# Patryk27/strolle

Measured on NVIDIA H100. Metric: Mrays/s (+ frames/s) at 1080p-per-GPU Cornell, ReSTIR DI+GI + SVGF; H100 vs CPU restatement of the reference, higher is better.
Workload: dtype f32

## Files before the change

include/strolle_b200.h:

```cpp
#ifndef STROLLE_B200_H
#define STROLLE_B200_H

#include <stddef.h>
#include <stdint.h>

#ifdef __cplusplus
extern "C" {
#endif

typedef struct st_engine st_engine;
typedef uint64_t st_handle;
typedef int32_t st_camera_handle;

enum { ST_OK = 0, ST_ERR_CUDA = -1, ST_ERR_INVALID = -2, ST_ERR_NOT_FOUND = -3, ST_ERR_LIMIT = -4 };

typedef struct st_mesh_triangle {
    float positions[3][3];
    float normals[3][3];
    float uvs[3][2];
    float tangents[3][4];
} st_mesh_triangle;

typedef struct st_material {
    float base_color[4];
// ... 52 lines not shown
int st_update_sun(st_engine* e, float azimuth, float altitude);
int st_set_environment_map(st_engine* e, const float* rgba32f, uint32_t width, uint32_t height, float intensity, float rotation);
typedef struct st_exposure { float ev, compensation, ev_min, ev_max, low, high, speed_up, speed_down; } st_exposure;
int st_set_exposure(st_engine* e, const st_exposure* exposure);
typedef struct st_bloom { float intensity, scatter, threshold, softness; int32_t levels, mode; } st_bloom;
int st_set_bloom(st_engine* e, const st_bloom* bloom);
typedef struct st_depth_of_field { float focal_distance, aperture_f_stops, sensor_height, max_radius; } st_depth_of_field;
int st_set_depth_of_field(st_engine* e, const st_depth_of_field* dof);

int st_create_camera(st_engine* e, const st_camera* camera, st_camera_handle* out);
int st_update_camera(st_engine* e, st_camera_handle camera, const st_camera* desc);
int st_delete_camera(st_engine* e, st_camera_handle camera);

int st_tick(st_engine* e);

int st_render_camera(st_engine* e, st_camera_handle camera, void* host_out, int format);
int st_copy_output(st_engine* e, st_camera_handle camera, void* host_out, int format);
int st_synchronize(st_engine* e);

int st_set_seed_base(st_engine* e, uint32_t base);
int st_set_blue_noise(st_engine* e, const uint8_t* rgba8_256x256);
int st_read_buffer(st_engine* e, st_camera_handle camera, const char* name, float* dst, size_t cap_floats, size_t* count);
int st_read_scene(st_engine* e, const char* name, float* dst, size_t cap_floats, size_t* count);
int st_bvh_depth(st_engine* e, int* depth);
uint32_t st_frame(st_engine* e);
int st_set_frame(st_engine* e, uint32_t frame);
int st_trace_closest(st_engine* e, const float* rays, size_t n, float* out, float* device_ms);
int st_trace_any(st_engine* e, const float* rays, size_t n, uint32_t* out, float* device_ms);
int st_device_math(st_engine* e, int op, const float* a, const float* b, float* out, size_t n);
#define ST_PASS_COUNT 27
int st_enable_timing(st_engine* e, int enabled);
int st_pass_times(st_engine* e, float* ms, uint32_t* launches, int reset);
const char* st_pass_name(int pass);
int st_wavelet_times(st_engine* e, float* ms5, uint32_t* launches5, int reset);
enum { ST_OPT_SVGF_FAST_MATH = 1, ST_OPT_ASYNC_OUTPUT = 2, ST_OPT_HALO_NCCL = 3, ST_OPT_WAVELET_TILED = 4, ST_OPT_WAVELET_TILE_CFG = 5, ST_OPT_FUSE_REPROJECT = 6, ST_OPT_BVH_REUSE = 7, ST_OPT_VARIANCE_TILED = 8, ST_OPT_SHADING_FAST_MATH = 9, ST_OPT_STRIP_FUSED = 10, ST_OPT_FUSED_PASSES = 11, ST_OPT_STRIP_DMA = 12, ST_OPT_WAVELET_PAIRED = 13, ST_OPT_NORMAL_MAPS = 14, ST_OPT_BVH_REFIT = 15, ST_OPT_LIGHT_GRID = 16, ST_OPT_TEXTURE_FILTER = 17, ST_OPT_TEMPORAL_AA = 18, ST_OPT_ENVIRONMENT_MAP_SAMPLING = 19, ST_OPT_TONEMAPPING = 20, ST_OPT_AUTO_EXPOSURE = 21, ST_OPT_BLOOM = 22, ST_OPT_DEPTH_OF_FIELD = 23 };
#define ST_WAVELET_PAIRED_DEFAULT 1
#define ST_STRIP_DMA_DEFAULT (-1)
#define ST_FUSED_PASSES_DEFAULT 1
#define ST_SHADING_FAST_DEFAULT 1
#define ST_VARIANCE_TILED_DEFAULT 1
#define ST_WAVELET_TILED_DEFAULT 15
#define ST_WAVELET_CFG_DEFAULT 0x01000
#define ST_FUSE_REPROJECT_DEFAULT 1
int st_set_option(st_engine* e, int option, int value);
enum { ST_STAT_WAVELET_TILED_LAUNCHES = 1, ST_STAT_WAVELET_TILED_ERRORS = 2, ST_STAT_BVH_GRAFTED_SUBTREES = 3, ST_STAT_VARIANCE_TILED_LAUNCHES = 4,
       ST_STAT_STRIP_PULLED_ROWS = 5 , ST_STAT_LAST_FRAME_FUSED_STRIPS = 6 ,
       ST_STAT_STRIP_FIRST_TIMEOUT = 7 ,
       ST_STAT_NORMAL_MAP_LAUNCHES = 8 ,
       ST_STAT_BVH_REFITS = 9 ,
       ST_STAT_LIGHT_GRID_BUILDS = 10 ,
       ST_STAT_TEXTURE_MIP_BUILDS = 11 ,
       ST_STAT_TAA_RESOLVES = 12 ,
       ST_STAT_ENVIRONMENT_MAP_LAUNCHES = 13 ,
       ST_STAT_ENVIRONMENT_MAP_DISTRIBUTION_BUILDS = 14 ,
       ST_STAT_EXPOSURE_METERINGS = 15 ,
       ST_STAT_BLOOM_PYRAMIDS = 16 ,
       ST_STAT_DEPTH_OF_FIELD_GATHERS = 17  };
int st_get_stat(st_engine* e, int stat, uint64_t* value);
typedef struct st_bvh_builder st_bvh_builder;
int st_bvh_builder_create(st_bvh_builder** out);
void st_bvh_builder_destroy(st_bvh_builder* b);
int st_bvh_builder_build(st_bvh_builder* b, const float* prims11, size_t n, int reuse, float* out, size_t cap_floats, size_t* n_floats,
                         uint32_t* grafted_subtrees, int* depth);
int st_bvh_builder_read(st_bvh_builder* b, float* out, size_t cap_floats);
int st_set_stream(st_engine* e, void* cuda_stream, int external);
int st_count_rays(st_engine* e, int enabled);
// ... 61 lines not shown
```

rust/strolle-b200-sys/src/lib.rs:

```rust
#![allow(non_camel_case_types, clippy::too_many_arguments)]

use std::os::raw::{c_char, c_int, c_void};

#[repr(C)] pub struct st_engine { _private: [u8; 0] }
#[repr(C)] pub struct st_multi { _private: [u8; 0] }
#[repr(C)] pub struct st_bvh_builder { _private: [u8; 0] }
pub type st_handle = u64;
pub type st_camera_handle = i32;

pub const ST_OK: c_int = 0;
pub const ST_ERR_CUDA: c_int = -1;
pub const ST_ERR_INVALID: c_int = -2;
pub const ST_ERR_NOT_FOUND: c_int = -3;
pub const ST_ERR_LIMIT: c_int = -4;

#[repr(C)] #[derive(Clone, Copy, Debug, Default)]
pub struct st_mesh_triangle { pub positions: [[f32; 3]; 3], pub normals: [[f32; 3]; 3], pub uvs: [[f32; 2]; 3], pub tangents: [[f32; 4]; 3] }
#[repr(C)] #[derive(Clone, Copy, Debug, Default)]
pub struct st_material { pub base_color: [f32; 4], pub emissive: [f32; 4], pub perceptual_roughness: f32, pub metallic: f32, pub reflectance: f32, pub ior: f32, pub alpha_blend: i32 }
#[repr(C)] #[derive(Clone, Copy, Debug, Default)]
pub struct st_material_textures { pub base_color: st_handle, pub emissive: st_handle, pub metallic_roughness: st_handle, pub normal_map: st_handle, pub mask: u32 }
pub const ST_LIGHT_POINT: i32 = 1;
pub const ST_LIGHT_SPOT: i32 = 2;
#[repr(C)] #[derive(Clone, Copy, Debug, Default)]
// ... 79 lines not shown
    pub fn st_remove_material(e: *mut st_engine, material: st_handle) -> c_int;
    pub fn st_insert_image(e: *mut st_engine, image: st_handle, rgba8: *const u8, width: u32, height: u32) -> c_int;
    pub fn st_remove_image(e: *mut st_engine, image: st_handle) -> c_int;
    pub fn st_set_material_textures(e: *mut st_engine, material: st_handle, textures: *const st_material_textures) -> c_int;
    pub fn st_insert_instance(e: *mut st_engine, instance: st_handle, mesh: st_handle, material: st_handle, affine: *const f32) -> c_int;
    pub fn st_remove_instance(e: *mut st_engine, instance: st_handle) -> c_int;
    pub fn st_insert_light(e: *mut st_engine, light: st_handle, l: *const st_light) -> c_int;
    pub fn st_remove_light(e: *mut st_engine, light: st_handle) -> c_int;
    pub fn st_update_sun(e: *mut st_engine, azimuth: f32, altitude: f32) -> c_int;
    pub fn st_set_environment_map(e: *mut st_engine, rgba32f: *const f32, width: u32, height: u32, intensity: f32, rotation: f32) -> c_int;
    pub fn st_set_exposure(e: *mut st_engine, exposure: *const st_exposure) -> c_int;
    pub fn st_set_bloom(e: *mut st_engine, bloom: *const st_bloom) -> c_int;
    pub fn st_set_depth_of_field(e: *mut st_engine, dof: *const st_depth_of_field) -> c_int;
    pub fn st_create_camera(e: *mut st_engine, camera: *const st_camera, out: *mut st_camera_handle) -> c_int;
    pub fn st_update_camera(e: *mut st_engine, camera: st_camera_handle, desc: *const st_camera) -> c_int;
    pub fn st_delete_camera(e: *mut st_engine, camera: st_camera_handle) -> c_int;
    pub fn st_tick(e: *mut st_engine) -> c_int;
    pub fn st_render_camera(e: *mut st_engine, camera: st_camera_handle, host_out: *mut c_void, format: c_int) -> c_int;
    pub fn st_copy_output(e: *mut st_engine, camera: st_camera_handle, host_out: *mut c_void, format: c_int) -> c_int;
    pub fn st_synchronize(e: *mut st_engine) -> c_int;
    pub fn st_set_seed_base(e: *mut st_engine, base: u32) -> c_int;
    pub fn st_set_blue_noise(e: *mut st_engine, rgba8_256x256: *const u8) -> c_int;
    pub fn st_read_buffer(e: *mut st_engine, camera: st_camera_handle, name: *const c_char, dst: *mut f32, cap_floats: usize, count: *mut usize) -> c_int;
    pub fn st_read_scene(e: *mut st_engine, name: *const c_char, dst: *mut f32, cap_floats: usize, count: *mut usize) -> c_int;
    pub fn st_bvh_depth(e: *mut st_engine, depth: *mut c_int) -> c_int;
    pub fn st_frame(e: *mut st_engine) -> u32;
    pub fn st_set_frame(e: *mut st_engine, frame: u32) -> c_int;
    pub fn st_trace_closest(e: *mut st_engine, rays: *const f32, n: usize, out: *mut f32, device_ms: *mut f32) -> c_int;
    pub fn st_trace_any(e: *mut st_engine, rays: *const f32, n: usize, out: *mut u32, device_ms: *mut f32) -> c_int;
    pub fn st_device_math(e: *mut st_engine, op: c_int, a: *const f32, b: *const f32, out: *mut f32, n: usize) -> c_int;
    pub fn st_enable_timing(e: *mut st_engine, enabled: c_int) -> c_int;
    pub fn st_pass_times(e: *mut st_engine, ms: *mut f32, launches: *mut u32, reset: c_int) -> c_int;
    pub fn st_pass_name(pass: c_int) -> *const c_char;
    pub fn st_wavelet_times(e: *mut st_engine, ms5: *mut f32, launches5: *mut u32, reset: c_int) -> c_int;
    pub fn st_set_option(e: *mut st_engine, option: c_int, value: c_int) -> c_int;
    pub fn st_get_stat(e: *mut st_engine, stat: c_int, value: *mut u64) -> c_int;
    pub fn st_bvh_builder_create(out: *mut *mut st_bvh_builder) -> c_int;
    pub fn st_bvh_builder_destroy(b: *mut st_bvh_builder);
    pub fn st_bvh_builder_build(b: *mut st_bvh_builder, prims11: *const f32, n: usize, reuse: c_int, out: *mut f32, cap_floats: usize, n_floats: *mut usize, grafted_subtrees: *mut u32, depth: *mut c_int) -> c_int;
    pub fn st_bvh_builder_read(b: *mut st_bvh_builder, out: *mut f32, cap_floats: usize) -> c_int;
    pub fn st_set_stream(e: *mut st_engine, cuda_stream: *mut c_void, external: c_int) -> c_int;
    pub fn st_count_rays(e: *mut st_engine, enabled: c_int) -> c_int;
    pub fn st_ray_count(e: *mut st_engine, rays: *mut u64, reset: c_int) -> c_int;
    pub fn st_nccl_unique_id(out128: *mut u8) -> c_int;
    pub fn st_nccl_init(e: *mut st_engine, id128: *const u8, rank: c_int, world: c_int) -> c_int;
    pub fn st_plan_frame(schedule: *const c_int, n: c_int, frame: u32, temporal_reach: c_int, out: *mut c_char, cap: usize) -> c_int;
    pub fn st_render_strips(e: *mut st_engine, camera: st_camera_handle, host_out: *mut c_void, format: c_int, temporal_reach: c_int, gather: c_int) -> c_int;
    pub fn st_plan_strip_order(schedule: *const c_int, n: c_int, dma: c_int, out: *mut c_char, cap: usize) -> c_int;
    pub fn st_strip_bounds(height: c_int, world: c_int, rows_out: *mut c_int) -> c_int;
    pub fn st_halo_bytes(e: *mut st_engine, bytes: *mut u64) -> c_int;
    pub fn st_peer_export(e: *mut st_engine, camera: st_camera_handle, out192: *mut u8) -> c_int;
    pub fn st_peer_import(e: *mut st_engine, camera: st_camera_handle, all_handles: *const u8, rank: c_int, world: c_int) -> c_int;
    pub fn st_peer_errors(e: *mut st_engine, camera: st_camera_handle, count: *mut u32) -> c_int;
    pub fn st_mark_begin(e: *mut st_engine) -> c_int;
    pub fn st_mark_end(e: *mut st_engine, ms: *mut f32) -> c_int;
    pub fn st_camera_set_strip(e: *mut st_engine, camera: st_camera_handle, y0: c_int, y1: c_int) -> c_int;
    pub fn st_buffer_device_ptr(e: *mut st_engine, camera: st_camera_handle, name: *const c_char, ptr: *mut *mut c_void, bytes: *mut usize) -> c_int;
    pub fn st_frame_schedule(e: *mut st_engine, camera: st_camera_handle, pass_ids: *mut c_int, cap: c_int, count: *mut c_int) -> c_int;
    pub fn st_render_range(e: *mut st_engine, camera: st_camera_handle, first: c_int, last: c_int) -> c_int;
    pub fn st_link_local(engines: *const *mut st_engine, cameras: *const st_camera_handle, n: c_int) -> c_int;
    pub fn st_multi_create(device_ordinals: *const c_int, n: c_int, out: *mut *mut st_multi) -> c_int;
    pub fn st_multi_destroy(m: *mut st_multi);
    pub fn st_multi_size(m: *mut st_multi) -> c_int;
    pub fn st_multi_engine(m: *mut st_multi, rank: c_int) -> *mut st_engine;
    pub fn st_multi_member_camera(m: *mut st_multi, camera: st_camera_handle, rank: c_int) -> st_camera_handle;
    pub fn st_multi_insert_mesh(m: *mut st_multi, mesh: st_handle, triangles: *const st_mesh_triangle, count: usize) -> c_int;
// ... 29 lines not shown
```

strolle_b200/csrc/engine.cu:

```cuda
#include <algorithm>
#include <cmath>
#include <cstdio>
#include <cstring>
#include <deque>
#include <functional>
#include <limits>
#include <string>
#include <unordered_map>
#include <vector>

#include <nccl.h>

#include "../../include/strolle_b200.h"
#include "kernels.h"

#include <dlfcn.h>
namespace {
struct NcclApi {
    void* lib = nullptr;
    ncclResult_t (*GetUniqueId)(ncclUniqueId*) = nullptr;
    ncclResult_t (*CommInitRank)(ncclComm_t*, int, ncclUniqueId, int) = nullptr;
    ncclResult_t (*CommDestroy)(ncclComm_t) = nullptr;
    ncclResult_t (*GroupStart)() = nullptr;
    ncclResult_t (*GroupEnd)() = nullptr;
    ncclResult_t (*Send)(const void*, size_t, ncclDataType_t, int, ncclComm_t, cudaStream_t) = nullptr;
    ncclResult_t (*Recv)(void*, size_t, ncclDataType_t, int, ncclComm_t, cudaStream_t) = nullptr;
    const char* (*GetErrorString)(ncclResult_t) = nullptr;
    bool load(std::string* err) {
        if (lib) return true;
        void* h = dlopen("libnccl.so.2", RTLD_NOW | RTLD_NOLOAD);
        if (!h) h = dlopen("libnccl.so.2", RTLD_NOW | RTLD_LOCAL);
        if (!h) { *err = std::string("cannot load libnccl.so.2: ") + dlerror(); return false; }
        auto sym = [&](const char* n) { void* p = dlsym(h, n); if (!p) *err = std::string("libnccl.so.2 lacks ") + n; return p; };
        GetUniqueId = (decltype(GetUniqueId))sym("ncclGetUniqueId"); CommInitRank = (decltype(CommInitRank))sym("ncclCommInitRank");
        CommDestroy = (decltype(CommDestroy))sym("ncclCommDestroy"); GroupStart = (decltype(GroupStart))sym("ncclGroupStart");
        GroupEnd = (decltype(GroupEnd))sym("ncclGroupEnd"); Send = (decltype(Send))sym("ncclSend"); Recv = (decltype(Recv))sym("ncclRecv");
        GetErrorString = (decltype(GetErrorString))sym("ncclGetErrorString");
        if (!GetUniqueId || !CommInitRank || !CommDestroy || !GroupStart || !GroupEnd || !Send || !Recv || !GetErrorString) return false;
        lib = h; return true;
    }
};
NcclApi g_nccl;
}


namespace st {

static thread_local std::string g_err;
static int fail(int code, const std::string& msg) { g_err = msg; return code; }
#define CK(call)                                                                                   \
    do { cudaError_t e_ = (call); if (e_ != cudaSuccess) return fail(ST_ERR_CUDA, std::string(#call) + ": " + cudaGetErrorString(e_)); } while (0)

struct H3 { float x, y, z; };
static inline H3 h3(float x, float y, float z) { H3 r = {x, y, z}; return r; }
static inline H3 operator+(H3 a, H3 b) { return h3(a.x + b.x, a.y + b.y, a.z + b.z); }
static inline H3 operator-(H3 a, H3 b) { return h3(a.x - b.x, a.y - b.y, a.z - b.z); }
static inline H3 operator*(H3 a, float s) { return h3(a.x * s, a.y * s, a.z * s); }
static inline H3 operator*(H3 a, H3 b) { return h3(a.x * b.x, a.y * b.y, a.z * b.z); }
static inline H3 operator/(H3 a, float s) { return h3(a.x / s, a.y / s, a.z / s); }
static inline float hdot(H3 a, H3 b) { return (a.x * b.x) + (a.y * b.y) + (a.z * b.z); }
static inline H3 hcross(H3 a, H3 b) { return h3(a.y * b.z - b.y * a.z, a.z * b.x - b.z * a.x, a.x * b.y - b.x * a.y); }
static inline H3 hnorm(H3 a) { return a * (1.0f / std::sqrt(hdot(a, a))); }
static inline float hmin(float a, float b) { return (a != a) ? b : ((b != b) ? a : (a < b ? a : b)); }
static inline float hmax(float a, float b) { return (a != a) ? b : ((b != b) ? a : (a > b ? a : b)); }
static inline uint32_t to_u32(float f) { if (!(f == f) || f <= 0.0f) return 0u; if (f >= 4294967296.0f) return 0xffffffffu; return (uint32_t)f; }
static inline float bits2f(uint32_t u) { float f; std::memcpy(&f, &u, 4); return f; }
static inline uint32_t f2bits(float f) { uint32_t u; std::memcpy(&u, &f, 4); return u; }
static const float FMAX = std::numeric_limits<float>::max();

struct Affine3 { H3 x, y, z, t; };
static inline H3 aff_mat(const Affine3& a, H3 v) { return (a.x * v.x + a.y * v.y) + a.z * v.z; }
static inline H3 aff_point(const Affine3& a, H3 p) { return aff_mat(a, p) + a.t; }
static Affine3 aff_inverse(const Affine3& a) {
    H3 t0 = hcross(a.y, a.z), t1 = hcross(a.z, a.x), t2 = hcross(a.x, a.y);
    float det = hdot(a.z, t2);
    float inv = 1.0f / det;
    H3 c0 = t0 * inv, c1 = t1 * inv, c2 = t2 * inv;
// ... 282 lines not shown
static const BloomDev kBloomDefaults = {0.15f, 0.7f, 0.0f, 0.0f, 7, 0};
static const st_depth_of_field kDofDefaults = {10.0f, 1.0f, 0.01866f, 16.0f};

struct CameraSlot {
    bool alive = false;
    st_camera desc;
    st_camera prev_desc;
    uint32_t frame = 0;
    CameraDev dev;
    std::vector<std::pair<std::string, float4**>> named;
    std::vector<std::pair<std::string, size_t>> sizes;
    DevMem arena;
    DevMem svgf_pairs; float4* pair[2] = {nullptr, nullptr};
    DevMem rgba8; int rgba8_slot = 0;
    DevMem taa; float4* taa_hist[2] = {nullptr, nullptr};
    DevMem expo;
    DevMem bloom;
    DevMem dof;
    cudaEvent_t ev_ready[2] = {nullptr, nullptr}, ev_copied[2] = {nullptr, nullptr};
    cudaStream_t side[2] = {nullptr, nullptr}; cudaEvent_t ev_produced = nullptr, ev_pushed[2] = {nullptr, nullptr}; bool pushed_pending[2] = {false, false};
    struct PeerLink { bool ready = false; bool ipc = false; std::vector<char*> arena, rgba8; std::vector<uint32_t*> flags; DevMem sync; uint32_t seq = 0, fseq = 0; } peer;
};

struct Step { int pass; std::function<void(cudaStream_t)> run; int sub = -1; };

}

using namespace st;

struct st_engine {
    int device = 0;
    cudaStream_t stream = nullptr; bool own_stream = true;
    cudaStream_t copy_stream = nullptr;
    std::unordered_map<st_handle, std::vector<st_mesh_triangle>> meshes;
    std::vector<st_material> materials; std::vector<st_handle> material_handles; bool materials_dirty = false;
    struct MatTex { st_handle tex[4]; uint32_t mask; };
    std::vector<MatTex> material_textures;
    struct ImageRect { st_handle handle; uint32_t x, y, w, h; };
    std::vector<ImageRect> images; uint32_t shelf_x = 0, shelf_y = 0, shelf_h = 0; bool images_dirty = false;
    DevMem d_atlas, d_srgb, d_tri_instance, d_instance_xforms;
    bool motion_dirty = true;
    bool moved_last_tick = false;
    struct Inst {
        st_handle handle, mesh, material; Affine3 xf, xf_inv, prev_xf; bool dirty;
        st_handle baked_mesh = ~(st_handle)0, baked_material = ~(st_handle)0; bool host_stale = false; Affine3 dev_xf, dev_xf_inv;
    };
    std::vector<Inst> instances; bool instances_dirty = false;
    struct Range { st_handle handle; size_t b, e; };
    std::vector<Range> tri_ranges; SlotAllocator tri_alloc;
    std::vector<float4> h_triangles; std::vector<Prim> prims; bool triangles_dirty = false;
    BvhBuild bvh; BvhOut bvh_out; bool bvh_dirty = false;
    std::vector<GpuMaterial> h_materials;
    static const st_handle kSun = ~(st_handle)0;
    std::vector<GpuLight> h_lights; std::vector<std::pair<st_handle, uint32_t>> light_slots;
    std::vector<st_handle> lights_created, lights_updated; std::vector<std::pair<st_handle, uint32_t>> lights_remapped; std::vector<uint32_t> lights_killed;
    uint32_t next_light = 1; bool lights_dirty = true;
    float sun_azimuth = 0.0f, sun_altitude = 0.35f; bool sun_dirty = true;
    GpuWorld world;
    uint32_t frame = 1, seed_base = 0xC0FFEEu;
    DevMem d_triangles, d_bvh, d_materials, d_matpacked, d_unpacklut, d_lights, d_noise, d_tlut, d_slut, d_skylut, d_scratch, d_raycount;
    bool count_rays = false;
    bool svgf_fast = true;
    bool shading_fast = ST_SHADING_FAST_DEFAULT != 0;
    bool fused_passes = ST_FUSED_PASSES_DEFAULT != 0;
    bool async_output = false;
    bool halo_nccl = false;
// ... 539 lines not shown
    const bool active = F > f;
    const double k = active ? A * f / (F - f) * (double)c.height / (double)l.sensor_height / 2.0 : 0.0;
    const double fx = -(double)c.transform[8], fy = -(double)c.transform[9], fz = -(double)c.transform[10];
    const double n = std::sqrt(fx * fx + fy * fy + fz * fz);
    DofDev p = {};
    p.active = active ? 1 : 0; p.k = (float)k; p.F = l.focal_distance; p.R = l.max_radius;
    p.fwd_x = (float)(fx / n); p.fwd_y = (float)(fy / n); p.fwd_z = (float)(fz / n);
    p.reach = (int)std::ceil((double)l.max_radius / kDofTile);
    const DofBufs b = dof_bufs(cs);
    const float fl[8] = {(float)f, (float)A, p.k, p.F, p.R, p.fwd_x, p.fwd_y, p.fwd_z};
    p.head[0] = c.width; p.head[1] = c.height; p.head[2] = (uint32_t)b.tx; p.head[3] = (uint32_t)b.ty; p.head[4] = (uint32_t)p.active;
    std::memcpy(p.head + 5, fl, sizeof fl);
    return p;
}
static bool lens_params(const st_engine* e, const CameraSlot* cs, uint32_t seed, LensDev* out) {
    const st_depth_of_field& l = e->dof_cfg;
    const st_camera& c = cs->desc;
    const double f = 0.5 * (double)l.sensor_height * (double)c.projection[5], A = f / (double)l.aperture_f_stops;
    if (!(e->dof_frame && c.mode == ST_MODE_REFERENCE && (double)l.focal_distance > f)) return false;
    double ax[3][3];
    for (int k = 0; k < 3; k++) {
        const double sg = k == 2 ? -1.0 : 1.0;
        const double x = sg * c.transform[4 * k], y = sg * c.transform[4 * k + 1], z = sg * c.transform[4 * k + 2], n = std::sqrt(x * x + y * y + z * z);
        ax[k][0] = x / n; ax[k][1] = y / n; ax[k][2] = z / n;
    }
    *out = LensDev{seed, (float)(A / 2.0), l.focal_distance, (float)ax[0][0], (float)ax[0][1], (float)ax[0][2], (float)ax[1][0], (float)ax[1][1],
                   (float)ax[1][2], (float)ax[2][0], (float)ax[2][1], (float)ax[2][2]};
    return true;
}
static CameraDev frame_source(const st_engine* e, const CameraSlot* cs, CameraDev c) {
    if (defocuses(e, cs) && cs->dof.p) c.output = dof_bufs(cs).frame;
    return c;
}
static void build_schedule(st_engine* e, CameraSlot* cs, std::vector<Step>* steps, const StripExt* ext = nullptr) {
    GpuCamera jc, jp; float4 jit;
    const bool taa = taa_cameras(e, cs, &jc, &jp, &jit);
    const CameraDev cam = [&] { CameraDev c = cs->dev; if (taa) { c.curr = jc; c.prev = jp; } return c; }();
    const StripExt no_ext; const StripExt& x = ext ? *ext : no_ext;
    const CameraDev camG = grown(cam, x.gbuffer), camV = grown(cam, x.variance);
    const int pm0 = x.preview_mirror[0], pm1 = x.preview_mirror[1];
    const SceneDev sc = e->scene();
    const uint32_t f = cs->frame;
    const int cur = (f % 2u) == 1u ? 1 : 0;
    const st_camera& d = cs->desc;
    const bool fs = e->shading_fast;
    const bool nm = e->nmap_frame;
    const bool lgon = e->lgrid_frame;
    const LightGridDev lgd = e->lgrid;
    const bool tfon = e->texf_frame;
    const TexFilterDev tfd = e->texf;
    const bool emon = e->envm_frame;
    EnvMapDev emd = e->envm;
    if (!e->envs_frame) emd.cdf = nullptr;
    const bool eson = emon && e->envs_frame;
    auto seed = [&](uint32_t k) { return dispatch_seed(e->seed_base, f, k); };
    auto add = [&](int pass, std::function<void(cudaStream_t)> fn) { steps->push_back(Step{pass, std::move(fn)}); };
    const CameraDev camO = frame_source(e, cs, cam);
    auto defocus = [&]() {
        if (!defocuses(e, cs)) return;
        const DofDev dp = dof_params(e, cs); const DofBufs db = dof_bufs(cs);
        add(P_COMPOSITION, [=](cudaStream_t s) { e->dof_gathers++; launch_depth_of_field(cam, dp, db, s); });
    };
    auto meter = [&]() {
        if (!meters(e, cs)) return;
        uint32_t* state = (uint32_t*)cs->expo.p; const ExposureDev ep = e->expo_frame; const int sms = e->sm_count;
        add(P_COMPOSITION, [=](cudaStream_t s) { e->exposure_meterings++; launch_exposure_histogram(camO, state, ep, sms, s); });
// ... 412 lines not shown
            StripPull pl; std::memset(&pl, 0, sizeof pl);
            for (int r = 0; r < N; r++) { pl.arena[r] = cs->peer.arena[r]; pl.bounds[r] = bounds[r].first; }
            pl.bounds[N] = H; pl.n_ranks = N; pl.rank = R; pl.w = (int)cs->desc.width; pl.h = H; pl.own_y0 = d.own_y0; pl.own_y1 = d.own_y1;
            pl.need_rows = (const int*)(sync + kNeedRowsWord); pl.pulled_rows = (unsigned long long*)(sync + kPulledRowsWord);
            struct { std::string name; int local; } items[] = {
                {std::string("prim_surface_map_") + prv, kSpatialReach}, {std::string("prim_gbuffer_d0_") + prv, kSpatialReach}, {std::string("prim_gbuffer_d1_") + prv, kSpatialReach},
                {"di_reservoirs_0", 0}, {"gi_reservoirs_0", 0}, {"di_diff_prev_colors", 0}, {"gi_diff_prev_colors", 0},
                {std::string("di_diff_moments_") + prv, 0}, {std::string("gi_diff_moments_") + prv, 0}};
            for (auto& it : items) {
                size_t kk = 0; float4* base = camera_buffer(cs, it.name, &kk);
                if (!base) return fail(ST_ERR_NOT_FOUND, "pull list names unknown buffer " + it.name);
                pl.items[pl.nitems++] = StripPullItem{(size_t)((char*)base - (char*)cs->arena.p), (int)kk, it.local};
            }
            e->run_timed(P_HALO_EXCHANGE, [=](cudaStream_t s) { launch_strip_pull(pl, s); });
            break;
        }
        }
    }
    d.y0 = d.own_y0; d.y1 = d.own_y1;
    if (push_rc) return push_rc;
    CK(cudaGetLastError());
    return ST_OK;
}

static CameraSlot* get_camera(st_engine* e, st_camera_handle h) { return (h >= 0 && (size_t)h < e->cameras.size() && e->cameras[h]->alive) ? e->cameras[h] : nullptr; }

}

extern "C" {

int st_copy_output(st_engine* e, st_camera_handle h, void* host_out, int format);
const char* st_last_error(void) { return g_err.c_str(); }
const char* st_pass_name(int pass) { return (pass >= 0 && pass < P_COUNT) ? kPassNames[pass] : ""; }

int st_engine_create(int device, st_engine** out) {
    if (!out) return fail(ST_ERR_INVALID, "out is null");
    int count = 0;
    cudaError_t ce = cudaGetDeviceCount(&count);
    if (ce != cudaSuccess || count == 0) return fail(ST_ERR_CUDA, "no CUDA device available: this library has no CPU fallback");
    if (device < 0 || device >= count) return fail(ST_ERR_INVALID, "bad device ordinal");
    CK(cudaSetDevice(device));
    st_engine* e = new st_engine();
    e->device = device;
    CK(cudaDeviceGetAttribute(&e->sm_count, cudaDevAttrMultiProcessorCount, device));
    CK(cudaStreamCreateWithFlags(&e->stream, cudaStreamNonBlocking));
    std::memset(&e->world, 0, sizeof e->world);
    e->h_lights.push_back(make_sun(make_float4(0, 0, 0, 25.0f), make_float4(0, 0, 0, std::numeric_limits<float>::infinity())));
    e->light_slots.push_back({st_engine::kSun, 0u});
    int rc = e->d_noise.ensure(256 * 256 * 4); if (rc) { delete e; return rc; }
    rc = e->d_unpacklut.ensure(512 * 4); if (rc) { delete e; return rc; }
    rc = e->d_tile_errors.ensure(4); if (rc) { delete e; return rc; }
    launch_unpack_lut((float*)e->d_unpacklut.p, e->stream);
    *out = e;
    return ST_OK;
}
void st_engine_destroy(st_engine* e) {
    if (!e) return;
    cudaSetDevice(e->device);
    cudaStreamSynchronize(e->stream);
    if (e->copy_stream) cudaStreamSynchronize(e->copy_stream);
    for (CameraSlot* c : e->cameras) { for (int k = 0; k < 2; k++) { if (c->side[k]) { cudaStreamSynchronize(c->side[k]); cudaStreamDestroy(c->side[k]); } if (c->ev_pushed[k]) cudaEventDestroy(c->ev_pushed[k]); } if (c->ev_produced) cudaEventDestroy(c->ev_produced);
        c->arena.release(); c->svgf_pairs.release(); c->rgba8.release(); for (int k = 0; k < 2; k++) { if (c->ev_ready[k]) cudaEventDestroy(c->ev_ready[k]); if (c->ev_copied[k]) cudaEventDestroy(c->ev_copied[k]); } delete c; }
    DevMem* all[] = {&e->d_triangles, &e->d_bvh, &e->d_materials, &e->d_lights, &e->d_noise, &e->d_tlut, &e->d_slut, &e->d_skylut, &e->d_scratch, &e->d_raycount, &e->d_matpacked, &e->d_unpacklut, &e->d_atlas, &e->d_srgb, &e->d_tri_instance, &e->d_instance_xforms, &e->d_tile_errors, &e->d_plan, &e->d_bake, &e->d_lgrid, &e->d_texf_pool, &e->d_texf_table, &e->d_texf_jobs, &e->d_envm, &e->d_envs};
    for (DevMem* d : all) d->release();
    for (auto& m : e->d_meshes) m.second.release();
    for (int k = 0; k < 2; k++) { if (e->staging[k]) cudaFreeHost(e->staging[k]); if (e->staging_ev[k]) cudaEventDestroy(e->staging_ev[k]); }
    for (auto& t : e->pending) { cudaEventDestroy(t.a); cudaEventDestroy(t.b); }
    for (cudaEvent_t ev : e->event_pool) cudaEventDestroy(ev);
    if (e->comm) g_nccl.CommDestroy(e->comm);
    if (e->own_stream) cudaStreamDestroy(e->stream);
    if (e->copy_stream) cudaStreamDestroy(e->copy_stream);
    delete e;
}

int st_insert_mesh(st_engine* e, st_handle mesh, const st_mesh_triangle* tris, size_t count) {
    if (!e || (!tris && count)) return fail(ST_ERR_INVALID, "null argument");
    rebake_host_mesh(e, mesh);
    auto dm = e->d_meshes.find(mesh);
    if (dm != e->d_meshes.end()) { cudaSetDevice(e->device); dm->second.release(); e->d_meshes.erase(dm); }
    e->meshes[mesh].assign(tris, tris + count);
    return ST_OK;
}
int st_remove_mesh(st_engine* e, st_handle mesh) {
    if (!e) return fail(ST_ERR_INVALID, "null engine");
    rebake_host_mesh(e, mesh);
    auto dm = e->d_meshes.find(mesh);
    if (dm != e->d_meshes.end()) { cudaSetDevice(e->device); dm->second.release(); e->d_meshes.erase(dm); }
    e->meshes.erase(mesh);
    return ST_OK;
}

int st_insert_material(st_engine* e, st_handle h, const st_material* m) {
    if (!e || !m) return fail(ST_ERR_INVALID, "null argument");
    auto it = std::find(e->material_handles.begin(), e->material_handles.end(), h);
    if (it != e->material_handles.end()) e->materials[it - e->material_handles.begin()] = *m;
    else { e->material_handles.push_back(h); e->materials.push_back(*m); st_engine::MatTex mt; std::memset(&mt, 0, sizeof mt); e->material_textures.push_back(mt); }
    e->materials_dirty = true;
    return ST_OK;
}
int st_has_material(st_engine* e, st_handle h) { return e && std::find(e->material_handles.begin(), e->material_handles.end(), h) != e->material_handles.end() ? 1 : 0; }
int st_remove_material(st_engine* e, st_handle h) {
    if (!e) return fail(ST_ERR_INVALID, "null engine");
    auto it = std::find(e->material_handles.begin(), e->material_handles.end(), h);
    if (it != e->material_handles.end()) *it = ~(st_handle)0 - 1;
// ... 284 lines not shown
    e->envm_frame = e->envm_set;
    if (!(e->envm_sampling && e->envm_set)) { e->d_envs.release(); e->envs_built = false; e->envm.cdf = nullptr; e->envm.total = 0.0f; }
    else if (!e->envs_built) { if ((rc = build_env_distribution(e))) return rc; }
    e->envs_frame = e->envs_built && e->envm.total > 0.0f && e->envm.total < INFINITY;
    if (e->temporal_aa != e->taa_frame) for (CameraSlot* c : e->cameras) { c->taa.release(); c->taa_hist[0] = c->taa_hist[1] = nullptr; }
    e->taa_frame = e->temporal_aa;
    if ((e->tonemapping != 0 && e->auto_exposure) != (e->tm_frame != 0 && e->ae_frame)) for (CameraSlot* c : e->cameras) c->expo.release();
    e->tm_frame = e->tonemapping; e->ae_frame = e->auto_exposure; e->expo_frame = e->exposure;
    if (e->bloom != e->bloom_frame || e->bloom_set.levels != e->bloom_cfg.levels) for (CameraSlot* c : e->cameras) c->bloom.release();
    e->bloom_frame = e->bloom; e->bloom_cfg = e->bloom_set;
    if (e->dof != e->dof_frame) for (CameraSlot* c : e->cameras) c->dof.release();
    e->dof_frame = e->dof; e->dof_cfg = e->dof_set;
    e->frame += 1;
    if (too_deep) return fail(ST_ERR_LIMIT, "BVH deeper than the 24-entry traversal stack (strolle-gpu/src/lib.rs:72-76): the scene is not drawn until it changes");
    return ST_OK;
}

int st_frame_schedule(st_engine* e, st_camera_handle h, int* pass_ids, int cap, int* count) {
    CameraSlot* cs = e ? get_camera(e, h) : nullptr;
    if (!cs || !count) return fail(ST_ERR_NOT_FOUND, "unknown camera");
    std::vector<Step> steps; build_schedule(e, cs, &steps);
    *count = (int)steps.size();
    for (int i = 0; i < cap && i < *count; i++) pass_ids[i] = steps[i].pass;
    return ST_OK;
}
static int ensure_taa_history(st_engine* e, CameraSlot* cs) {
    GpuCamera a, b; float4 j;
    if (cs->taa.p || !taa_cameras(e, cs, &a, &b, &j)) return ST_OK;
    const size_t bytes = ((size_t)cs->desc.width * cs->desc.height * 16 + 255) / 256 * 256;
    int rc = cs->taa.ensure(2 * bytes); if (rc) return rc;
    cs->taa_hist[0] = (float4*)cs->taa.p; cs->taa_hist[1] = (float4*)((char*)cs->taa.p + bytes);
    return ST_OK;
}
int st_render_range(st_engine* e, st_camera_handle h, int first, int last) {
    CameraSlot* cs = e ? get_camera(e, h) : nullptr;
    if (!cs) return fail(ST_ERR_NOT_FOUND, "unknown camera");
    if (cs->frame == 0) return fail(ST_ERR_INVALID, "st_tick must precede st_render_camera");
    CK(cudaSetDevice(e->device));
    int rc = ensure_luts(e); if (rc) return rc;
    if ((rc = ensure_taa_history(e, cs))) return rc;
    if ((rc = ensure_exposure_state(e, cs))) return rc;
    if ((rc = ensure_bloom_state(e, cs))) return rc;
    if ((rc = ensure_dof_state(e, cs))) return rc;
    std::vector<Step> steps; build_schedule(e, cs, &steps);
    if (last < 0 || last >= (int)steps.size()) last = (int)steps.size() - 1;
    for (int i = std::max(first, 0); i <= last; i++) e->run_timed(steps[i].pass, steps[i].run, steps[i].sub);
    CK(cudaGetLastError());
    return ST_OK;
}
int st_render_camera(st_engine* e, st_camera_handle h, void* host_out, int format) {
    int rc = st_render_range(e, h, 0, -1); if (rc) return rc;
    if (host_out) return st_copy_output(e, h, host_out, format);
    return ST_OK;
}
static int store_rgba8(st_engine* e, CameraSlot* cs, const CameraDev& cd, uchar4* dst8) {
    const SceneDev sc = e->scene();
    const int op = cs->desc.mode == ST_MODE_BVH_HEATMAP ? 0 : e->tm_frame;
    if (blooms(e, cs)) {
        int rc = ensure_exposure_state(e, cs); if (rc) return rc;
        if ((rc = ensure_bloom_state(e, cs))) return rc;
        const uint32_t* state = meters(e, cs) ? (const uint32_t*)cs->expo.p : nullptr; const ExposureDev ep = e->expo_frame;
        const BloomDev bp = e->bloom_cfg; const BloomLevels lv = bloom_levels(e, cs);
        e->run_timed(P_COMPOSITION, [=](cudaStream_t s) { launch_output_bloom(cd, sc, op, state, ep, bp, lv.up[0], lv.w[0], lv.h[0], dst8, s); });
        return ST_OK;
    }
    if (op == 0) { e->run_timed(P_COMPOSITION, [=](cudaStream_t s) { launch_output_rgba8(cd, sc, dst8, s); }); return ST_OK; }
    int rc = ensure_exposure_state(e, cs); if (rc) return rc;
    const uint32_t* state = meters(e, cs) ? (const uint32_t*)cs->expo.p : nullptr; const ExposureDev ep = e->expo_frame;
    e->run_timed(P_COMPOSITION, [=](cudaStream_t s) { launch_output_display(cd, sc, op, state, ep, dst8, s); });
    return ST_OK;
}
static int copy_rows_out(st_engine* e, CameraSlot* cs, void* host_out, int format, int y0, int y1) {
    const size_t W = cs->desc.width, n = W * cs->desc.height;
    const size_t first = (size_t)y0 * W, count = (size_t)(y1 - y0) * W;
    int rc2 = ensure_dof_state(e, cs); if (rc2) return rc2;
    const CameraDev src = frame_source(e, cs, cs->dev);
    if (format == ST_FORMAT_RGBA32F) CK(cudaMemcpyAsync((char*)host_out + first * 16, src.output + first, count * 16, cudaMemcpyDeviceToHost, e->stream));
    else if (format == ST_FORMAT_RGBA8_SRGB) {
        if ((rc2 = cs->rgba8.ensure(2 * n * 4))) return rc2;
        cs->rgba8_slot ^= 1;
        uchar4* dst8 = (uchar4*)cs->rgba8.p + (cs->rgba8_slot ? n : 0); CameraDev cd = src; cd.y0 = y0; cd.y1 = y1;
        const int k = cs->rgba8_slot;
        if (e->async_output) {
            if (!e->copy_stream) CK(cudaStreamCreateWithFlags(&e->copy_stream, cudaStreamNonBlocking));
            if (!cs->ev_ready[k]) { CK(cudaEventCreateWithFlags(&cs->ev_ready[k], cudaEventDisableTiming)); CK(cudaEventCreateWithFlags(&cs->ev_copied[k], cudaEventDisableTiming)); }
            else CK(cudaStreamWaitEvent(e->stream, cs->ev_copied[k], 0));
        }
        if ((rc2 = store_rgba8(e, cs, cd, dst8))) return rc2;
        if (e->async_output) {
            CK(cudaEventRecord(cs->ev_ready[k], e->stream));
            CK(cudaStreamWaitEvent(e->copy_stream, cs->ev_ready[k], 0));
            CK(cudaMemcpyAsync((char*)host_out + first * 4, dst8 + first, count * 4, cudaMemcpyDeviceToHost, e->copy_stream));
            CK(cudaEventRecord(cs->ev_copied[k], e->copy_stream));
        } else CK(cudaMemcpyAsync((char*)host_out + first * 4, dst8 + first, count * 4, cudaMemcpyDeviceToHost, e->stream));
    } else return fail(ST_ERR_INVALID, "unsupported output format");
    return ST_OK;
}
int st_copy_output(st_engine* e, st_camera_handle h, void* host_out, int format) {
    CameraSlot* cs = e ? get_camera(e, h) : nullptr;
    if (!cs || !host_out) return fail(ST_ERR_NOT_FOUND, "unknown camera");
    CK(cudaSetDevice(e->device));
    int rc = copy_rows_out(e, cs, host_out, format, 0, (int)cs->desc.height); if (rc) return rc;
    if (!e->async_output) CK(cudaStreamSynchronize(e->stream));
    return ST_OK;
}
int st_synchronize(st_engine* e) {
    if (!e) return fail(ST_ERR_INVALID, "null engine");
    CK(cudaSetDevice(e->device)); CK(cudaStreamSynchronize(e->stream));
    if (e->copy_stream) CK(cudaStreamSynchronize(e->copy_stream));
    for (CameraSlot* c : e->cameras) for (int k = 0; k < 2; k++) if (c->side[k]) CK(cudaStreamSynchronize(c->side[k]));
    return ST_OK;
}

int st_read_buffer(st_engine* e, st_camera_handle h, const char* name, float* dst, size_t cap, size_t* count) {
    CameraSlot* cs = e ? get_camera(e, h) : nullptr;
    if (!cs || !name || !count) return fail(ST_ERR_NOT_FOUND, "unknown camera");
    CK(cudaSetDevice(e->device));
    if (!std::strcmp(name, "curr_camera") || !std::strcmp(name, "prev_camera")) {
        GpuCamera jc, jp; float4 jit;
        const bool taa = taa_cameras(e, cs, &jc, &jp, &jit);
        const GpuCamera& c = !std::strcmp(name, "curr_camera") ? (taa ? jc : cs->dev.curr) : (taa ? jp : cs->dev.prev);
        *count = 40; if (dst) std::memcpy(dst, &c, 4 * std::min<size_t>(cap, 40)); return ST_OK;
    }
    if (!std::strcmp(name, "exposure")) {
        if (!cs->expo.p) return fail(ST_ERR_NOT_FOUND, "no exposure state: the camera does not meter (ST_OPT_TONEMAPPING and ST_OPT_AUTO_EXPOSURE)");
        *count = 5 + kExposureBins;
        if (dst) { CK(cudaStreamSynchronize(e->stream)); CK(cudaMemcpy(dst, cs->expo.p, 4 * std::min(cap, *count), cudaMemcpyDeviceToHost)); }
        return ST_OK;
    }
    if (!std::strcmp(name, "bloom")) {
        if (!blooms(e, cs) || !cs->bloom.p) return fail(ST_ERR_NOT_FOUND, "no bloom pyramid: ST_OPT_BLOOM is off or the camera does not bloom");
        BloomLevels lv; *count = bloom_layout((int)cs->desc.width, (int)cs->desc.height, e->bloom_cfg.levels, nullptr, &lv) / 4;
        if (dst) { CK(cudaStreamSynchronize(e->stream)); CK(cudaMemcpy(dst, cs->bloom.p, 4 * std::min(cap, *count), cudaMemcpyDeviceToHost)); }
        return ST_OK;
    }
    if (!std::strcmp(name, "depth_of_field")) {
        if (!defocuses(e, cs) || !cs->dof.p) return fail(ST_ERR_NOT_FOUND, "no depth of field: ST_OPT_DEPTH_OF_FIELD is off or the camera is not defocused");
        const DofBufs b = dof_bufs(cs); *count = b.words_count;
        if (dst) { CK(cudaStreamSynchronize(e->stream)); CK(cudaMemcpy(dst, b.words, 4 * std::min(cap, *count), cudaMemcpyDeviceToHost)); }
        return ST_OK;
    }
    if (!std::strcmp(name, "taa_history_a") || !std::strcmp(name, "taa_history_b")) {
// ... 779 lines not shown
```

strolle_b200/csrc/kernels.cu:

```cuda
#include <algorithm>
#include <cstdio>
#include <cuda_fp16.h>
#include <cuda.h>
#include <map>
#include <mutex>
#include <tuple>
#include <vector>
#include "st_device.cuh"
#include "kernels.h"
#if ST_BLOOM_TAIL_KIND == 2
#include <cooperative_groups.h>
#endif

#if defined(ST_FAST) && ST_FAST
#define ST_EXACT_ONLY 0
#else
#define ST_EXACT_ONLY 1
#endif

namespace ST_NS {

#define TILE_W 16
#define TILE_H 8

struct Px { u32 x, y; bool in; };
ST_DEV u32 row_tile(const CameraDev& cam) {
    if (cam.mirror_dn == 0) return blockIdx.y;
    const u32 lead = (u32)(ST_REACH_SPATIAL / TILE_H);
    return gridDim.y > lead ? (blockIdx.y + gridDim.y - lead) % gridDim.y : blockIdx.y;
}
ST_DEV Px pixel_full(const CameraDev& cam) {
    Px p; p.x = blockIdx.x * TILE_W + (threadIdx.x % TILE_W); p.y = (u32)cam.y0 + row_tile(cam) * TILE_H + (threadIdx.x / TILE_W);
    p.in = p.x < (u32)cam.w && p.y < (u32)cam.y1;
    return p;
}
ST_DEV int half_grid_w(int w) { return 8 * (((w + 7) / 8) / 2); }
ST_DEV Px pixel_half(const CameraDev& cam) {
    Px p; p.x = blockIdx.x * TILE_W + (threadIdx.x % TILE_W); p.y = (u32)cam.y0 + row_tile(cam) * TILE_H + (threadIdx.x / TILE_W);
    p.in = p.x < (u32)half_grid_w(cam.w) && p.y < (u32)cam.y1;
    return p;
}
ST_DEV size_t pix(const CameraDev& cam, u32 x, u32 y) { return (size_t)y * (size_t)cam.w + x; }
ST_DEV size_t screen_idx(const CameraDev& cam, u32 x, u32 y) { return (size_t)(y * to_u32_sat(cam.curr.screen.x) + x); }
ST_DEV bool in_tex(const CameraDev& cam, u32 x, u32 y) { return x < (u32)cam.w && y < (u32)cam.h; }
ST_DEV float4 tex_or_zero(const float4* __restrict__ t, const CameraDev& cam, u32 x, u32 y) { return in_tex(cam, x, y) ? t[pix(cam, x, y)] : f4zero(); }
ST_DEV void tex_store(float4* __restrict__ t, const CameraDev& cam, u32 x, u32 y, float4 v) { if (in_tex(cam, x, y)) t[pix(cam, x, y)] = v; }
ST_DEV Hit load_hit(const GpuCamera& c, const float4* __restrict__ d0, const float4* __restrict__ d1, const CameraDev& cam, u32 x, u32 y) {
    return hit_make(cam_ray(c, x, y), gbuf_unpack(tex_or_zero(d0, cam, x, y), tex_or_zero(d1, cam, x, y)));
}
ST_DEV Hit load_hit_lut(const SceneDev& sc, const GpuCamera& c, const float4* __restrict__ d0, const float4* __restrict__ d1, const CameraDev& cam, u32 x, u32 y) {
    return hit_make(cam_ray(c, x, y), gbuf_unpack(sc, tex_or_zero(d0, cam, x, y), tex_or_zero(d1, cam, x, y)));
}
#define ST_TRACE_STACK()                                          \
// ... 45 lines not shown
#ifndef ST_MINB_GI_SAMPLING_A
#define ST_MINB_GI_SAMPLING_A 0
#endif
#define ST_LB_GI_SAMPLING_A ST_LB_PICK(ST_MINB_GI_SAMPLING_A)
#ifndef ST_MINB_GI_SAMPLING_B
#define ST_MINB_GI_SAMPLING_B 0
#endif
#define ST_LB_GI_SAMPLING_B ST_LB_PICK(ST_MINB_GI_SAMPLING_B)
#ifndef ST_MINB_GI_TEMPORAL
#define ST_MINB_GI_TEMPORAL 0
#endif
#define ST_LB_GI_TEMPORAL ST_LB_PICK(ST_MINB_GI_TEMPORAL)
#ifndef ST_MINB_GI_SPATIAL_PICK
#define ST_MINB_GI_SPATIAL_PICK 0
#endif
#define ST_LB_GI_SPATIAL_PICK ST_LB_PICK(ST_MINB_GI_SPATIAL_PICK)
#ifndef ST_MINB_GI_SPATIAL_SAMPLE
#define ST_MINB_GI_SPATIAL_SAMPLE 0
#endif
#define ST_LB_GI_SPATIAL_SAMPLE ST_LB_PICK(ST_MINB_GI_SPATIAL_SAMPLE)
#ifndef ST_MINB_GI_PREVIEW
#define ST_MINB_GI_PREVIEW 0
#endif
#define ST_LB_GI_PREVIEW ST_LB_PICK(ST_MINB_GI_PREVIEW)
#ifndef ST_MINB_GI_RESOLVING
#define ST_MINB_GI_RESOLVING 0
#endif
#define ST_LB_GI_RESOLVING ST_LB_PICK(ST_MINB_GI_RESOLVING)

#if ST_EXACT_ONLY
ST_DEV float4 frame_reprojection_px(const CameraDev& cam, int cur, Px p, float4 surface_texel, float4 vel);
template <bool NMAP, bool TEXF>
__global__ void ST_LB_PRIM_GBUFFER k_prim_gbuffer(KPARAMS, int cur, int with_reprojection, const __grid_constant__ TexFilterDev tf) {
    ST_TRACE_STACK();
    Px p = pixel_full(cam);
    if (!p.in) return;
    Ray ray = cam_ray(cam.curr, p.x, p.y);
    TriHit th = trace_closest(ray, sc, stk);
    if ((int)p.y < cam.own_y0 || (int)p.y >= cam.own_y1) uncount_ray(sc);
    float4 g0 = f4zero(), g1 = f4zero(), surf = f4zero(), vel = f4zero(), tid = f4(bitsf(0xffffffffu), 0.f, 0.f, 0.f), nd = f4zero();
    if (trihit_some(th)) {
        const GpuMaterial m = sc.materials[th.material_id];
        if (NMAP) th.normal = nmap_normal(sc, th, m.normal_map_texture);
        GBuf g;
        float2 mr;
        if (TEXF) {
            TexFoot ft; ft.tri = th.triangle_id; ft.dir = ray.d; ft.w = texf_cone_width(cam.curr, p.x, p.y, th.t, true);
            const float4 t = texf_sample(sc, tf, th.material_id, 2u, m.metallic_roughness_texture, f4(1.0f, m.roughness, m.metallic, 1.0f), th.uv, ft);
            mr = f2(t.z, t.y);
            g.base_color = texf_sample(sc, tf, th.material_id, 0u, m.base_color_texture, m.base_color, th.uv, ft);
            g.emissive = xyz(texf_sample(sc, tf, th.material_id, 1u, m.emissive_texture, m.emissive, th.uv, ft));
        } else {
            mr = mat_metallic_roughness(sc, m, th.uv);
            g.base_color = mat_base_color(sc, m, th.uv); g.emissive = mat_emissive(sc, m, th.uv);
        }
        g.normal = th.normal; g.metallic = mr.x;
        g.roughness = mr.y; g.reflectance = m.reflectance; g.depth = dist(ray.o, th.point);
        gbuf_pack_pre(g, all_zero(m.base_color_texture) ? __ldg(sc.material_packed + th.material_id) : gbuf_pack_color(g.base_color), &g0, &g1);
        float2 n = oct_encode(th.normal);
        surf = f4(n.x, n.y, g.depth, m.roughness);
        nd = f4(oct_decode(n), g.depth);
        const float4* xf = sc.instance_xforms + 6u * (size_t)__ldg(sc.tri_instance + th.triangle_id);
        float4 c0 = ldg4(xf), c1 = ldg4(xf + 1), c2 = ldg4(xf + 2), q0 = ldg4(xf + 3), q1 = ldg4(xf + 4), q2 = ldg4(xf + 5);
        float3 local = ((xyz(c0) * th.point.x + xyz(c1) * th.point.y) + xyz(c2) * th.point.z) + f3(c0.w, c1.w, c2.w);
        float3 prev_point = ((xyz(q0) * local.x + xyz(q1) * local.y) + xyz(q2) * local.z) + f3(q0.w, q1.w, q2.w);
        float2 v = cam_world_to_screen(cam.curr, th.point) - cam_world_to_screen(cam.prev, prev_point);
// ... 6 lines not shown
            if (hi >= cam.own_y1) atomicMax(cam.need_rows + 1, hi);
        }
    }
    size_t i = pix(cam, p.x, p.y);
    cam.prim_gbuffer_d0[cur][i] = g0; cam.prim_gbuffer_d1[cur][i] = g1; cam.prim_surface_map[cur][i] = surf;
    cam.velocity_map[i] = vel; cam.prim_triangle_ids[i] = tid; cam.surface_nd[i] = nd;
    if (with_reprojection && (int)p.y >= cam.own_y0 && (int)p.y < cam.own_y1) cam.reprojection_map[i] = frame_reprojection_px(cam, cur, p, surf, vel);
}

ST_DEV float4 frame_reprojection_px(const CameraDev& cam, int cur, Px p, float4 surface_texel, float4 vel) {
    const float4* sp_ = cam.prim_surface_map[cur ^ 1];
    Reproj rp; rp.px = 0.f; rp.py = 0.f; rp.confidence = 0.f; rp.validity = 0u;
    Surf surface = surf_decode(surface_texel);
    if (surface.depth == 0.0f) return reproj_encode(rp);
    float2 prev = f2((float)p.x, (float)p.y) - f2(vel.x, vel.y);
    float2 pr = f2(roundf(prev.x), roundf(prev.y));
    if (cam_contains_f(cam.prev, pr)) {
        Surf ps = surf_decode(tex_or_zero(sp_, cam, to_u32_sat(pr.x), to_u32_sat(pr.y)));
        float conf = surf_similarity(ps, surface);
        if (conf > 0.0f) { rp.px = prev.x; rp.py = prev.y; rp.confidence = conf; rp.validity = 0u; }
    }
    if (reproj_some(rp)) {
        int x0 = to_i32_sat(floorf(rp.px)), x1 = to_i32_sat(ceilf(rp.px)), y0 = to_i32_sat(floorf(rp.py)), y1 = to_i32_sat(ceilf(rp.py));
        int xs[4] = {x0, x1, x0, x1}, ys[4] = {y0, y0, y1, y1};
#pragma unroll
        for (int k = 0; k < 4; k++) {
            if (!cam_contains_i(cam.curr, xs[k], ys[k])) continue;
            if (surf_similarity(surf_decode(sp_[pix(cam, (u32)xs[k], (u32)ys[k])]), surface) >= 0.25f) rp.validity |= (1u << k);
        }
    }
    return reproj_encode(rp);
}
__global__ void __launch_bounds__(ST_BLOCK) k_frame_reprojection(KPARAMS, int cur) {
    Px p = pixel_full(cam);
    if (!p.in) return;
    size_t i = pix(cam, p.x, p.y);
    cam.reprojection_map[i] = frame_reprojection_px(cam, cur, p, cam.prim_surface_map[cur][i], cam.velocity_map[i]);
}
#endif

template <bool LGRID>
ST_DEV DiRes di_sampling_px(const CameraDev& cam, const SceneDev& sc, const TraceStack& stk, const Hit& hit, u32 seed, u32 frame, Px p, const LightGridDev& lg) {
    Rng rng = rng_make(seed, p.x, p.y);
    EphRes res = LGRID ? ephemeral_build_list(rng, sc, hit, lgrid_list(lg, hit.point)) : ephemeral_build(rng, sc, hit);
    DiRes out = di_zero();
    if (res.m > 0.0f) {
        float4 bn = blue_noise(sc, p.x, p.y, frame);
        Ray ray = light_ray_bnoise(light_load(sc, res.light_id), f2(bn.x, bn.y), hit.point);
        bool occ = trace_any(ray, sc, stk);
        if (occ) res.w = 0.0f;
        out.pdf = 0.f; out.confidence = 0.f; out.light_id = res.light_id; out.light_point = ray.o; out.occluded = occ; out.m = 1.0f; out.w = res.w;
    }
    return out;
}
template <bool LGRID>
__global__ void ST_LB_DI_SAMPLING k_di_sampling(KPARAMS, int cur, u32 seed, u32 frame, const __grid_constant__ LightGridDev lg) {
    ST_TRACE_STACK();
    Px p = pixel_full(cam);
    if (!p.in) return;
    Hit hit = load_hit_lut(sc, cam.curr, cam.prim_gbuffer_d0[cur], cam.prim_gbuffer_d1[cur], cam, p.x, p.y);
    if (!hit_some(hit)) return;
    di_store(di_sampling_px<LGRID>(cam, sc, stk, hit, seed, frame, p, lg), cam.di_reservoirs[1], screen_idx(cam, p.x, p.y));
}

ST_DEV DiRes di_temporal_px(const CameraDev& cam, const SceneDev& sc, int cur, u32 seed, Px p, const Hit& lhs_hit, DiRes lhs) {
    size_t npx = (size_t)cam.w * cam.h;
    Rng rng = rng_make(seed, p.x, p.y);
    if (lhs.m != 0.0f) lhs.pdf = di_pdf_with(lhs, light_load(sc, lhs.light_id), lhs_hit);
    DiRes rhs = di_zero();
    Hit rhs_hit = hit_zero();
    bool killed = false;
    Reproj rp = reproj_decode(cam.reprojection_map[pix(cam, p.x, p.y)]);
    if (reproj_some(rp)) {
        uint2 rpos = reproj_round(rp);
        size_t ridx = screen_idx(cam, rpos.x, rpos.y);
        if (ridx < npx) rhs = di_load(cam.di_reservoirs[0], ridx);
        rhs.m = rmin(rhs.m, 64.0f);
        if (rhs.m != 0.0f) {
            GpuLight rl = light_load(sc, rhs.light_id);
            u32 slot = fbits(rl.d3.x);
            if (slot == 0xcafebabeu) { rhs.w = 0.0f; killed = true; }
            else if (slot > 0u) rhs.light_id = slot - 1u;
            rhs_hit = load_hit_lut(sc, cam.prev, cam.prim_gbuffer_d0[cur ^ 1], cam.prim_gbuffer_d1[cur ^ 1], cam, rpos.x, rpos.y);
        }
    }
    MisIn mi;
    mi.lhs_m = lhs.m; mi.rhs_m = rhs.m; mi.rhs_jacobian = 1.0f; mi.lhs_lhs_pdf = lhs.pdf; mi.rhs_rhs_pdf = rhs.pdf;
    mi.lhs_rhs_pdf = ((lhs.m > 0.0f) & hit_some(rhs_hit)) ? di_pdf_with(lhs, light_prev(light_load(sc, lhs.light_id)), rhs_hit) : 0.0f;
    mi.rhs_lhs_pdf = ((rhs.m > 0.0f) & !killed) ? di_pdf_with(rhs, light_load(sc, rhs.light_id), lhs_hit) : 0.0f;
    MisOut mo = mis_eval(mi);
    DiRes main_ = di_zero();
    float main_pdf = 0.0f;
    if (di_update(main_, rng, lhs, mo.lhs_mis * mo.lhs_pdf * lhs.w)) main_pdf = mo.lhs_pdf;
    if (di_update(main_, rng, rhs, mo.rhs_mis * mo.rhs_pdf * rhs.w)) main_pdf = mo.rhs_pdf;
    main_.m = lhs.m + mo.m;
    main_.pdf = main_pdf;
    main_.confidence = killed ? 0.0f : 1.0f;
    main_.w = res_norm(main_.w, main_pdf, 1.0f, 1.0f);
    return main_;
}
__global__ void ST_LB_DI_TEMPORAL k_di_temporal(KPARAMS, int cur, u32 seed) {
    Px p = pixel_full(cam);
    if (!p.in) return;
    size_t lhs_idx = screen_idx(cam, p.x, p.y);
    Hit lhs_hit = load_hit_lut(sc, cam.curr, cam.prim_gbuffer_d0[cur], cam.prim_gbuffer_d1[cur], cam, p.x, p.y);
    if (!hit_some(lhs_hit)) return;
    di_store_m(cam, di_temporal_px(cam, sc, cur, seed, p, lhs_hit, di_load(cam.di_reservoirs[1], lhs_idx)), cam.di_reservoirs[1], lhs_idx, p.y, cam.di_mirror_reach);
}
template <bool LGRID>
__global__ void ST_LB_DI_SAMPLING k_di_sample_temporal(KPARAMS, int cur, u32 seed_sampling, u32 seed_temporal, u32 frame, const __grid_constant__ LightGridDev lg) {
    ST_TRACE_STACK();
    Px p = pixel_full(cam);
    if (!p.in) return;
    Hit hit = load_hit_lut(sc, cam.curr, cam.prim_gbuffer_d0[cur], cam.prim_gbuffer_d1[cur], cam, p.x, p.y);
    if (!hit_some(hit)) return;
    DiRes fresh = di_sampling_px<LGRID>(cam, sc, stk, hit, seed_sampling, frame, p, lg);
    di_store_m(cam, di_temporal_px(cam, sc, cur, seed_temporal, p, hit, fresh), cam.di_reservoirs[1], screen_idx(cam, p.x, p.y), p.y, cam.di_mirror_reach);
}

struct PairTexels { float4 a0, a1, b0, b1; int state; };

ST_DEV PairTexels di_spatial_pick_pair(const CameraDev& cam, const SceneDev& sc, int cur, u32 seed, u32 frame, Px g) {
    PairTexels o; o.a0 = o.a1 = o.b0 = o.b1 = f4zero(); o.state = 0;
    uint2 lp = checker(g.x, g.y, frame / 2u + 1u);
    if (!cam_contains_u(cam.curr, lp.x, lp.y)) return o;
    o.state = 1;
    size_t lhs_idx = screen_idx(cam, lp.x, lp.y);
    Rng rng = rng_make(seed, lp.x, lp.y);
    const float4* gd0 = cam.prim_gbuffer_d0[cur]; const float4* gd1 = cam.prim_gbuffer_d1[cur];
    Hit lhs_hit = load_hit_lut(sc, cam.curr, gd0, gd1, cam, lp.x, lp.y);
    if (!hit_some(lhs_hit)) return o;
    DiRes lhs = di_load(cam.di_reservoirs[1], lhs_idx);
    DiRes rhs = di_zero();
    size_t rhs_idx = 0;
    Hit rhs_hit = hit_zero();
    float max_radius = 128.0f;
    for (u32 nth = 0u; nth < 8u; nth++) {
        float2 off = rng_disk(rng) * max_radius;
        float2 fp = f2((float)lp.x, (float)lp.y) + off;
        uint2 rpos = cam_contain(cam.curr, to_i32_sat(fp.x), to_i32_sat(fp.y));
        if (rpos.x == lp.x && rpos.y == lp.y) continue;
        float4 nd = tex_or_zero(cam.surface_nd, cam, rpos.x, rpos.y);
        if (nd.w == 0.0f) { max_radius = rmax(max_radius * 0.5f, 5.0f); continue; }
        if (fabs_(nd.w - lhs_hit.g.depth) > 0.33f * lhs_hit.g.depth) { max_radius = rmax(max_radius * 0.5f, 5.0f); continue; }
        if (dot(xyz(nd), lhs_hit.g.normal) < 0.33f) { max_radius = rmax(max_radius * 0.5f, 5.0f); continue; }
        rhs_idx = screen_idx(cam, rpos.x, rpos.y);
        rhs = di_load(cam.di_reservoirs[1], rhs_idx);
        if (rhs.m != 0.0f) { rhs_hit = load_hit_lut(sc, cam.curr, gd0, gd1, cam, rpos.x, rpos.y); break; }
    }
    if (rhs.m == 0.0f) return o;
    float lhs_rhs_pdf = di_pdf_with(lhs, light_load(sc, lhs.light_id), rhs_hit);
    float rhs_lhs_pdf = di_pdf_with(rhs, light_load(sc, rhs.light_id), lhs_hit);
    Ray ra = (lhs_rhs_pdf > 0.0f) ? di_ray(lhs, rhs_hit.point) : ray_zero();
    Ray rb = (rhs_lhs_pdf > 0.0f) ? di_ray(rhs, lhs_hit.point) : ray_zero();
    float2 na = oct_encode(ra.d), nb = oct_encode(rb.d);
    o.a0 = f4(ra.o, ra.len); o.a1 = f4(na.x, na.y, bitsf((u32)rhs_idx + 1u), 0.0f);
    o.b0 = f4(rb.o, rb.len); o.b1 = f4(nb.x, nb.y, lhs_rhs_pdf, rhs_lhs_pdf);
    o.state = 2;
    return o;
}
ST_DEV void store_pair_texels(const CameraDev& cam, const PairTexels& o, float4* buf_d0, float4* buf_d1, Px g) {
    if (o.state == 0) return;
    u32 ax = g.x * 2u, bx = g.x * 2u + 1u;
    if (o.state == 2) { tex_store(buf_d0, cam, ax, g.y, o.a0); tex_store(buf_d0, cam, bx, g.y, o.b0); }
    tex_store(buf_d1, cam, ax, g.y, o.a1); tex_store(buf_d1, cam, bx, g.y, o.b1);
}
__global__ void ST_LB_DI_SPATIAL_PICK k_di_spatial_pick(KPARAMS, int cur, u32 seed, u32 frame) {
    Px g = pixel_half(cam);
    if (!g.in) return;
    store_pair_texels(cam, di_spatial_pick_pair(cam, sc, cur, seed, frame, g), cam.di_diff_samples, cam.di_diff_curr_colors, g);
}

ST_DEV float4 spatial_trace_texel(const SceneDev& sc, const TraceStack& stk, float4 d0, float4 d1) {
    if (all_zero(d1)) return f4zero();
    Ray ray = ray_make(xyz(d0), oct_decode(f2(d1.x, d1.y)), d0.w);
    bool occ = trace_any(ray, sc, stk);
    return f4(occ ? 0.0f : 1.0f, d1.z, d1.w, 0.0f);
}
__global__ void ST_LB_SPATIAL_TRACE k_spatial_trace(KPARAMS, const float4* __restrict__ buf_d0, const float4* __restrict__ buf_d1, float4* __restrict__ buf_d2) {
    ST_TRACE_STACK();
    Px p = pixel_full(cam);
    if (!p.in) return;
    size_t i = pix(cam, p.x, p.y);
    buf_d2[i] = spatial_trace_texel(sc, stk, buf_d0[i], buf_d1[i]);
}
ST_DEV void trace_pair_texels(const CameraDev& cam, const SceneDev& sc, const TraceStack& stk, const PairTexels& o, Px g, float4* d2a, float4* d2b) {
    u32 ax = g.x * 2u, bx = g.x * 2u + 1u;
    *d2a = (o.state == 2 && in_tex(cam, ax, g.y)) ? spatial_trace_texel(sc, stk, o.a0, o.a1) : f4zero();
    *d2b = (o.state == 2 && in_tex(cam, bx, g.y)) ? spatial_trace_texel(sc, stk, o.b0, o.b1) : f4zero();
}

ST_DEV void di_spatial_sample_pair(const CameraDev& cam, u32 seed, u32 frame, Px g, float4 d0, float4 d1) {
    uint2 lp = checker(g.x, g.y, frame / 2u + 1u);
    if (!cam_contains_u(cam.curr, lp.x, lp.y)) return;
    size_t npx = (size_t)cam.w * cam.h;
    size_t lhs_idx = screen_idx(cam, lp.x, lp.y);
    Rng rng = rng_make(seed, lp.x, lp.y);
    const float4* in = cam.di_reservoirs[1]; float4* out = cam.di_reservoirs[2];
    float lhs_rhs_vis = d0.x; u32 rhs_idx = fbits(d0.y);
    float rhs_lhs_vis = d1.x, lhs_rhs_pdf = d1.y, rhs_lhs_pdf = d1.z;
    DiRes lhs = di_load(in, lhs_idx);
    if (rhs_idx > 0u && (size_t)rhs_idx - 1 < npx) {
        DiRes rhs = di_load(in, (size_t)rhs_idx - 1);
        MisIn mi;
        mi.lhs_m = lhs.m; mi.rhs_m = rhs.m; mi.rhs_jacobian = 1.0f; mi.lhs_lhs_pdf = lhs.pdf;
        mi.lhs_rhs_pdf = lhs_rhs_pdf * lhs_rhs_vis; mi.rhs_lhs_pdf = rhs_lhs_pdf * rhs_lhs_vis; mi.rhs_rhs_pdf = rhs.pdf;
        MisOut mo = mis_eval(mi);
        DiRes main_ = di_zero();
        float main_pdf = 0.0f;
        if (di_update(main_, rng, lhs, mo.lhs_mis * mo.lhs_pdf * lhs.w)) main_pdf = mo.lhs_pdf;
        if (di_update(main_, rng, rhs, mo.rhs_mis * mo.rhs_pdf * rhs.w)) { main_pdf = mo.rhs_pdf; main_.occluded = lhs_rhs_vis == 0.0f; }
        main_.m = lhs.m + mo.m;
        main_.pdf = main_pdf;
        main_.w = res_norm(main_.w, main_pdf, 1.0f, 1.0f);
        di_store(main_, out, lhs_idx);
    } else di_store(lhs, out, lhs_idx);
    uint2 op = checker(g.x, g.y, frame / 2u);
    if (cam_contains_u(cam.curr, op.x, op.y)) { size_t oi = screen_idx(cam, op.x, op.y); di_store(di_load(in, oi), out, oi); }
}
__global__ void __launch_bounds__(ST_BLOCK) k_di_spatial_sample(KPARAMS, u32 seed, u32 frame) {
    Px g = pixel_half(cam);
    if (!g.in) return;
    di_spatial_sample_pair(cam, seed, frame, g, tex_or_zero(cam.di_diff_stash, cam, g.x * 2u, g.y), tex_or_zero(cam.di_diff_stash, cam, g.x * 2u + 1u, g.y));
}
__global__ void ST_LB_DI_SPATIAL_PICK k_di_spatial_fused(KPARAMS, int cur, u32 seed_pick, u32 seed_sample, u32 frame) {
    ST_TRACE_STACK();
    Px g = pixel_half(cam);
    if (!g.in) return;
    PairTexels o = di_spatial_pick_pair(cam, sc, cur, seed_pick, frame, g);
    if (o.state == 0) return;
    float4 d2a, d2b; trace_pair_texels(cam, sc, stk, o, g, &d2a, &d2b);
    di_spatial_sample_pair(cam, seed_sample, frame, g, d2a, d2b);
}

template <bool ENVM>
__global__ void ST_LB_DI_RESOLVING k_di_resolving(KPARAMS, int cur, const __grid_constant__ EnvMapDev em) {
    ST_TRACE_STACK();
    Px p = pixel_full(cam);
    if (!p.in) return;
    size_t idx = screen_idx(cam, p.x, p.y);
    Hit hit = load_hit_lut(sc, cam.curr, cam.prim_gbuffer_d0[cur], cam.prim_gbuffer_d1[cur], cam, p.x, p.y);
    DiRes res = di_load(cam.di_reservoirs[2], idx);
    float confidence;
    LightRad rad;
    if (hit_some(hit)) {
        bool occ = trace_any(di_ray(res, hit.point), sc, stk);
        confidence = (res.occluded == occ) ? res.confidence : 0.0f;
        res.confidence = 1.0f;
        res.occluded = occ;
        if (occ) rad = lightrad_zero();
        else { rad = light_radiance(light_load(sc, res.light_id), hit); rad.radiance = rad.radiance * res.w; }
    } else {
        confidence = 1.0f;
        rad.radiance = sky_radiance<ENVM>(sc, em, world_sun_dir(sc.world), hit.dir);
        rad.diff = f3s(1.0f); rad.spec = f3s(0.0f);
    }
    float diff_brdf = (1.0f - hit.g.metallic) / kPi;
    size_t i = pix(cam, p.x, p.y);
    cam.di_diff_samples[i] = f4(rad.radiance * diff_brdf, confidence);
    cam.di_spec_samples[i] = f4(rad.radiance * rad.spec, confidence);
    di_store(res, cam.di_reservoirs[0], idx);
}

ST_DEV GiRes gi_reprojection_px(const CameraDev& cam, const Hit& hit, const Reproj& rp) {
    size_t npx = (size_t)cam.w * cam.h;
    GiRes res = gi_zero();
    if (reproj_some(rp)) {
        uint2 rpos = reproj_round(rp);
        size_t ridx = screen_idx(cam, rpos.x, rpos.y);
        if (ridx < npx) res = gi_load(cam.gi_reservoirs[0], ridx);
    }
    res.confidence = 1.0f;
    res.v1 = hit.point;
    return res;
}
__global__ void __launch_bounds__(ST_BLOCK) k_gi_reprojection(KPARAMS, int cur) {
    Px p = pixel_full(cam);
    if (!p.in) return;
    Hit hit = load_hit_lut(sc, cam.curr, cam.prim_gbuffer_d0[cur], cam.prim_gbuffer_d1[cur], cam, p.x, p.y);
    if (!hit_some(hit)) return;
    gi_store_m(cam, gi_reprojection_px(cam, hit, reproj_decode(cam.reprojection_map[pix(cam, p.x, p.y)])), cam.gi_reservoirs[2], screen_idx(cam, p.x, p.y), p.y,
               (int)p.x >= 2 * half_grid_w(cam.w) ? cam.gi_mirror_reach : 0);
}

template <bool NMAP, bool TEXF, int ENVM>
ST_DEV bool gi_sampling_a_pair(const CameraDev& cam, const SceneDev& sc, const TraceStack& stk, int cur, u32 seed, u32 frame, Px g, float4* t0, float4* t1, float4* t2,
                               const TexFilterDev& tf, const EnvMapDev& em) {
    bool tracing = gi_tracing_frame(frame);
    uint2 sp = tracing ? checker(g.x, g.y, frame / 2u) : checker(g.x, g.y, frame);
    if (!cam_contains_u(cam.curr, sp.x, sp.y)) return false;
    size_t idx = screen_idx(cam, sp.x, sp.y);
    Ray gi_r; float gi_pdf_;
    if (tracing) {
        Rng rng = rng_make(seed, sp.x, sp.y);
        Hit hit = load_hit_lut(sc, cam.curr, cam.prim_gbuffer_d0[cur], cam.prim_gbuffer_d1[cur], cam, sp.x, sp.y);
        if (!hit_some(hit)) return false;
        if (ENVM == ENV_SAMPLED) {
            float3 dir;
            if (rng_f(rng) < 0.5f) { const float xi1 = rng_f(rng), xi2 = rng_f(rng); dir = env_draw(em, xi1, xi2); }
            else dir = brdf_layered_sample(hit.g, rng, -hit.dir).dir;
            gi_r = ray_make(hit.point, dir);
            gi_pdf_ = env_mixture_pdf(em, hit.g, -hit.dir, dir);
        } else {
            BrdfS s = brdf_layered_sample(hit.g, rng, -hit.dir);
            gi_r = ray_make(hit.point, s.dir);
            gi_pdf_ = s.pdf;
        }
    } else {
        GiRes res = gi_load(cam.gi_reservoirs[2], idx);
        if (res.m == 0.0f) return false;
        gi_r = ray_make(res.v1, gi_dir(res, res.v1));
        gi_pdf_ = 1.0f;
    }
    TriHit gh = trace_closest(gi_r, sc, stk);
    GBuf gg = gbuf_zero();
    u32 gi_color_bits = 0u;
    if (trihit_some(gh)) {
        GpuMaterial m = sc.materials[gh.material_id];
        m.roughness = rmax(m.roughness, 0.75f * 0.75f);
        if (TEXF) {
            TexFoot ft; ft.tri = gh.triangle_id; ft.dir = gi_r.d; ft.w = texf_cone_width(cam.curr, sp.x, sp.y, gh.t, false);
            gg.base_color = texf_sample(sc, tf, gh.material_id, 0u, m.base_color_texture, m.base_color, gh.uv, ft);
            gg.emissive = xyz(texf_sample(sc, tf, gh.material_id, 1u, m.emissive_texture, m.emissive, gh.uv, ft));
            gg.normal = NMAP ? nmap_normal(sc, gh, m.normal_map_texture) : gh.normal; gg.metallic = m.metallic;
        } else {
            gg.base_color = mat_base_color(sc, m, gh.uv); gg.normal = NMAP ? nmap_normal(sc, gh, m.normal_map_texture) : gh.normal; gg.metallic = m.metallic; gg.emissive = mat_emissive(sc, m, gh.uv);
        }
        gi_color_bits = all_zero(m.base_color_texture) ? __ldg(sc.material_packed + gh.material_id) : gbuf_pack_color(gg.base_color);
        gg.roughness = m.roughness; gg.reflectance = m.reflectance; gg.depth = dist(gi_r.o, gh.point);
    }
    gbuf_pack_pre(gg, gi_color_bits, t1, t2);
    *t0 = f4(gi_r.d, gi_pdf_);
    return true;
}
template <bool NMAP, bool TEXF, int ENVM>
__global__ void ST_LB_GI_SAMPLING_A k_gi_sampling_a(KPARAMS, int cur, u32 seed, u32 frame, const __grid_constant__ TexFilterDev tf, const __grid_constant__ EnvMapDev em) {
    ST_TRACE_STACK();
    Px g = pixel_half(cam);
    if (!g.in) return;
    float4 t0, t1, t2;
    if (!gi_sampling_a_pair<NMAP, TEXF, ENVM>(cam, sc, stk, cur, seed, frame, g, &t0, &t1, &t2, tf, em)) return;
    size_t gi = pix(cam, g.x, g.y);
    cam.gi_d0[gi] = t0; cam.gi_d1[gi] = t1; cam.gi_d2[gi] = t2;
}

template <bool LGRID, int ENVM>
ST_DEV void gi_sampling_b_pair(const CameraDev& cam, const SceneDev& sc, const TraceStack& stk, int cur, u32 seed, u32 frame, Px g, float4 d0, float4 d1, float4 d2, const LightGridDev& lg,
                               const EnvMapDev& em) {
    bool tracing = gi_tracing_frame(frame);
    uint2 sp = tracing ? checker(g.x, g.y, frame / 2u) : checker(g.x, g.y, frame);
    if (!cam_contains_u(cam.curr, sp.x, sp.y)) return;
    size_t idx = screen_idx(cam, sp.x, sp.y);
    Hit prim = load_hit_lut(sc, cam.curr, cam.prim_gbuffer_d0[cur], cam.prim_gbuffer_d1[cur], cam, sp.x, sp.y);
    if (!hit_some(prim)) return;
    Rng rng; Hit gh; float gi_pdf_;
    if (tracing) {
        rng = rng_make(seed, sp.x, sp.y);
        gh = hit_make(ray_make(prim.point, xyz(d0)), gbuf_unpack(sc, d1, d2));
        gi_pdf_ = d0.w;
    } else {
        GiRes res = gi_load(cam.gi_reservoirs[2], idx);
        if (res.m == 0.0f) return;
        rng.s = res.rng;
        gh = hit_make(ray_make(res.v1, xyz(d0)), gbuf_unpack(sc, d1, d2));
        gi_pdf_ = 1.0f;
    }
    u32 rng_state = rng.s;
    const u32 SKY = 0xffffffffu;
    float3 sun_dir = world_sun_dir(sc.world);
// ... 17 lines not shown
            }
        } else {
            EphRes er = LGRID ? ephemeral_build_list(rng, sc, gh, lgrid_list(lg, gh.point)) : ephemeral_build(rng, sc, gh);
            if (er.w > 0.0f) { light_id = er.light_id; light_pdf = (1.0f / er.w) * (1.0f - atm_pdf); light_rad = er.rad.radiance * (f3s(1.0f) + er.rad.spec); }
            else { light_id = 0u; light_pdf = 1.0f; light_rad = f3s(0.f); }
        }
    }
    float3 radiance;
    if (light_pdf > 0.0f) {
        float vis;
        if (hit_some(gh)) {
            if (ENVM == ENV_SAMPLED && sky_below) vis = 0.0f;
            else {
                Ray r = (light_id == SKY) ? ray_make(gh.point, light_dir) : light_ray_wnoise(light_load(sc, light_id), rng, gh.point);
                vis = trace_any(r, sc, stk) ? 0.0f : 1.0f;
            }
        } else vis = 1.0f;
        radiance = light_rad * vis / light_pdf;
    } else radiance = f3s(0.f);
    if (hit_some(gh)) { radiance = radiance * (xyz(gh.g.base_color) / kPi); radiance = radiance + gh.g.emissive; }
    GiRes res = gi_zero();
    if (gi_pdf_ > 0.0f) {
        res.rng = rng_state; res.radiance = radiance; res.v1 = prim.point;
        if (hit_some(gh)) { res.v2 = gh.point; res.v2n = gh.g.normal; }
        else { res.v2 = prim.point + gh.dir * 1000.0f; res.v2n = -gh.dir; }
        res.m = 1.0f; res.w = 1.0f / gi_pdf_;
        res.pdf = 0.0f;
        res.pdf = gi_pdf(res, prim);
    }
    gi_store(res, cam.gi_reservoirs[1], idx);
}
template <bool LGRID, int ENVM>
__global__ void ST_LB_GI_SAMPLING_B k_gi_sampling_b(KPARAMS, int cur, u32 seed, u32 frame, const __grid_constant__ LightGridDev lg, const __grid_constant__ EnvMapDev em) {
    ST_TRACE_STACK();
    Px g = pixel_half(cam);
    if (!g.in) return;
    size_t gi = pix(cam, g.x, g.y);
    gi_sampling_b_pair<LGRID, ENVM>(cam, sc, stk, cur, seed, frame, g, cam.gi_d0[gi], cam.gi_d1[gi], cam.gi_d2[gi], lg, em);
}
template <bool NMAP, bool LGRID, bool TEXF, int ENVM>
__global__ void ST_LB_GI_SAMPLING_B k_gi_sampling_fused(KPARAMS, int cur, u32 seed_a, u32 seed_b, u32 frame, const __grid_constant__ LightGridDev lg,
                                                        const __grid_constant__ TexFilterDev tf, const __grid_constant__ EnvMapDev em) {
    ST_TRACE_STACK();
    Px g = pixel_half(cam);
    if (!g.in) return;
    float4 t0, t1, t2;
    if (!gi_sampling_a_pair<NMAP, TEXF, ENVM == ENV_SAMPLED ? ENV_SAMPLED : ENV_NONE>(cam, sc, stk, cur, seed_a, frame, g, &t0, &t1, &t2, tf, em)) return;
    gi_sampling_b_pair<LGRID, ENVM>(cam, sc, stk, cur, seed_b, frame, g, t0, t1, t2, lg, em);
}

__global__ void ST_LB_GI_TEMPORAL k_gi_temporal(KPARAMS, int cur, u32 seed, u32 frame, int inline_reprojection) {
    Px p = pixel_full(cam);
    if (!p.in) return;
    bool tracing = gi_tracing_frame(frame);
    size_t lhs_idx = screen_idx(cam, p.x, p.y);
    Rng rng = rng_make(seed, p.x, p.y);
    Hit lhs_hit = load_hit_lut(sc, cam.curr, cam.prim_gbuffer_d0[cur], cam.prim_gbuffer_d1[cur], cam, p.x, p.y);
    float4* curr = cam.gi_reservoirs[1];
    if (!hit_some(lhs_hit)) { gi_store_m(cam, gi_zero(), curr, lhs_idx, p.y, cam.gi_mirror_reach); return; }
    bool got = tracing ? (frame % 2u == 0u && checker_at(p.x, p.y, frame / 2u)) : checker_at(p.x, p.y, frame);
    GiRes lhs = got ? gi_load(curr, lhs_idx) : gi_zero();
    GiRes rhs = gi_zero();
    Hit rhs_hit = hit_zero();
    Reproj rp = reproj_decode(cam.reprojection_map[pix(cam, p.x, p.y)]);
    if (inline_reprojection) {
        GiRes r11 = gi_reprojection_px(cam, lhs_hit, rp);
        if ((int)p.x >= 2 * half_grid_w(cam.w)) gi_store_m(cam, r11, cam.gi_reservoirs[2], lhs_idx, p.y, cam.gi_mirror_reach);
        if (reproj_some(rp)) { rhs = r11; rhs.v2n = oct_decode(oct_encode(r11.v2n)); }
    } else if (reproj_some(rp)) rhs = gi_load(cam.gi_reservoirs[2], lhs_idx);
    if (reproj_some(rp)) {
        rhs.confidence = 1.0f;
        rhs.m = rmin(rhs.m, 128.0f);
        if (!tracing && lhs.m != 0.0f && rhs.m != 0.0f && gi_exists(rhs)) {
            if (dist(lhs.radiance, rhs.radiance) > 0.33f) rhs.confidence = 0.0f;
            rhs.radiance = lhs.radiance; rhs.v2 = lhs.v2; rhs.v2n = lhs.v2n;
        }
        if (rhs.m != 0.0f) {
            uint2 rpos = reproj_round(rp);
            rhs_hit = load_hit_lut(sc, cam.prev, cam.prim_gbuffer_d0[cur ^ 1], cam.prim_gbuffer_d1[cur ^ 1], cam, rpos.x, rpos.y);
        }
    }
    GiRes main_ = gi_zero();
    float main_pdf = 0.0f;
    if (tracing) {
// ... 35 lines not shown
    Hit rhs_hit = hit_zero();
    float rhs_jac = 0.0f;
    float max_radius = 128.0f;
    for (u32 nth = 0u; nth < 8u; nth++) {
        float2 off = rng_disk(rng) * max_radius;
        float2 fp = f2((float)lp.x, (float)lp.y) + off;
        uint2 rpos = cam_contain(cam.curr, to_i32_sat(fp.x), to_i32_sat(fp.y));
        if (rpos.x == lp.x && rpos.y == lp.y) continue;
        float4 nd = tex_or_zero(cam.surface_nd, cam, rpos.x, rpos.y);
        if (nd.w == 0.0f) { max_radius = rmax(max_radius * 0.5f, 5.0f); continue; }
        if (fabs_(nd.w - lhs_hit.g.depth) > 0.33f * lhs_hit.g.depth) { max_radius = rmax(max_radius * 0.5f, 5.0f); continue; }
        if (dot(xyz(nd), lhs_hit.g.normal) < 0.33f) { max_radius = rmax(max_radius * 0.5f, 5.0f); continue; }
        rhs_idx = screen_idx(cam, rpos.x, rpos.y);
        rhs = gi_load(reservoirs, rhs_idx);
        if (rhs.m == 0.0f) continue;
        rhs_jac = gi_jacobian(rhs, lhs_hit.point);
        if (rhs_jac < 1.0f / 10.0f || rhs_jac > 10.0f) { rhs.m = 0.0f; continue; }
        rhs_jac = rclamp(rhs_jac, 1.0f / 3.0f, 3.0f);
        rhs_hit = load_hit_lut(sc, cam.curr, gd0, gd1, cam, rpos.x, rpos.y);
        break;
    }
    if (rhs.m == 0.0f || !hit_some(rhs_hit)) return o;
    float lhs_rhs_pdf = gi_pdf(lhs, rhs_hit);
    float rhs_lhs_pdf = gi_pdf(rhs, lhs_hit);
    Ray ra = (lhs_rhs_pdf > 0.0f) ? gi_ray(lhs, rhs_hit.point) : ray_zero();
    Ray rb = (rhs_lhs_pdf > 0.0f) ? gi_ray(rhs, lhs_hit.point) : ray_zero();
    float2 na = oct_encode(ra.d), nb = oct_encode(rb.d);
    o.a0 = f4(ra.o, ra.len); o.a1 = f4(na.x, na.y, bitsf((u32)rhs_idx + 1u), rhs_jac);
    o.b0 = f4(rb.o, rb.len); o.b1 = f4(nb.x, nb.y, lhs_rhs_pdf, rhs_lhs_pdf);
    o.state = 2;
    return o;
}
__global__ void ST_LB_GI_SPATIAL_PICK k_gi_spatial_pick(KPARAMS, int cur, u32 seed, u32 frame) {
    Px g = pixel_half(cam);
    if (!g.in) return;
    store_pair_texels(cam, gi_spatial_pick_pair(cam, sc, cur, seed, frame, g), cam.gi_d0, cam.gi_d1, g);
}

ST_DEV void gi_spatial_sample_pair(const CameraDev& cam, u32 seed, u32 frame, Px g, float4 d0, float4 d1) {
    uint2 sp = checker(g.x, g.y, frame / 2u + 1u);
    if (!cam_contains_u(cam.curr, sp.x, sp.y)) return;
    size_t npx = (size_t)cam.w * cam.h;
    size_t idx = screen_idx(cam, sp.x, sp.y);
    Rng rng = rng_make(seed, sp.x, sp.y);
    const float4* in = cam.gi_reservoirs[1]; float4* out = cam.gi_reservoirs[2];
    float lhs_rhs_vis = d0.x; u32 rhs_idx = fbits(d0.y); float rhs_jac = d0.z;
    float rhs_lhs_vis = d1.x, lhs_rhs_pdf = d1.y, rhs_lhs_pdf = d1.z;
    GiRes lhs = gi_load(in, idx);
    if (rhs_idx > 0u && (size_t)rhs_idx - 1 < npx) {
        GiRes rhs = gi_load(in, (size_t)rhs_idx - 1);
        MisIn mi;
        mi.lhs_m = lhs.m; mi.rhs_m = rhs.m; mi.rhs_jacobian = rhs_jac; mi.lhs_lhs_pdf = lhs.pdf;
        mi.lhs_rhs_pdf = lhs_rhs_pdf * lhs_rhs_vis; mi.rhs_lhs_pdf = rhs_lhs_pdf * rhs_lhs_vis; mi.rhs_rhs_pdf = rhs.pdf;
        MisOut mo = mis_eval(mi);
        GiRes main_ = gi_zero();
        float main_pdf = 0.0f;
        if (gi_update(main_, rng, lhs, mo.lhs_mis * mo.lhs_pdf * lhs.w)) main_pdf = mo.lhs_pdf;
        if (gi_update(main_, rng, rhs, mo.rhs_mis * mo.rhs_pdf * rhs.w * rhs_jac)) main_pdf = mo.rhs_pdf;
        main_.m = lhs.m + mo.m;
        main_.confidence = 1.0f;
        main_.pdf = main_pdf;
        main_.v1 = lhs.v1;
        main_.w = res_norm(main_.w, main_pdf, 1.0f, 1.0f);
        main_.w = rmin(main_.w, 5.0f);
        gi_store_m(cam, main_, out, idx, sp.y, cam.gi_mirror_reach);
    } else gi_store_m(cam, lhs, out, idx, sp.y, cam.gi_mirror_reach);
    uint2 op = checker(g.x, g.y, frame / 2u);
    if (cam_contains_u(cam.curr, op.x, op.y)) { size_t oi = screen_idx(cam, op.x, op.y); gi_store_m(cam, gi_load(in, oi), out, oi, op.y, cam.gi_mirror_reach); }
}
__global__ void ST_LB_GI_SPATIAL_SAMPLE k_gi_spatial_sample(KPARAMS, u32 seed, u32 frame) {
    Px g = pixel_half(cam);
    if (!g.in) return;
    gi_spatial_sample_pair(cam, seed, frame, g, tex_or_zero(cam.gi_d2, cam, g.x * 2u, g.y), tex_or_zero(cam.gi_d2, cam, g.x * 2u + 1u, g.y));
}
__global__ void ST_LB_GI_SPATIAL_PICK k_gi_spatial_fused(KPARAMS, int cur, u32 seed_pick, u32 seed_sample, u32 frame) {
    ST_TRACE_STACK();
    Px g = pixel_half(cam);
    if (!g.in) return;
    PairTexels o = gi_spatial_pick_pair(cam, sc, cur, seed_pick, frame, g);
    if (o.state == 0) return;
    float4 d2a, d2b; trace_pair_texels(cam, sc, stk, o, g, &d2a, &d2b);
    gi_spatial_sample_pair(cam, seed_sample, frame, g, d2a, d2b);
}

ST_DEV bool gi_preview_px(const CameraDev& cam, const SceneDev& sc, const Hit& chit, u32 seed, u32 nth, const float4* __restrict__ in, Px p, GiRes* result) {
    size_t cidx = screen_idx(cam, p.x, p.y);
    Rng rng = rng_make(seed, p.x, p.y);
    if (!hit_some(chit)) { *result = gi_zero(); return true; }
    GiRes main_ = gi_zero();
    float main_pdf = 0.0f;
    GiRes center = gi_load(in, cidx);
    if (gi_merge(main_, rng, center, center.pdf)) main_pdf = center.pdf;
    u32 max_samples = to_u32_sat(lerpc(8.0f, 0.0f, main_.m / 8.0f));
    float max_radius = (nth == 0u) ? 128.0f : 64.0f;
    const float4* __restrict__ surf = cam.surface_nd;
    for (u32 k = 0u; k < max_samples; k++) {
        float2 off = rng_disk(rng) * max_radius;
        float2 fp = f2((float)p.x, (float)p.y) + off;
        uint2 sp = cam_contain(cam.curr, to_i32_sat(fp.x), to_i32_sat(fp.y));
        if (sp.x == p.x && sp.y == p.y) return false;
        if (!cam_contains_u(cam.curr, sp.x, sp.y)) continue;
        float4 nd = surf[pix(cam, sp.x, sp.y)];
        if (nd.w == 0.0f) continue;
        if (fabs_(nd.w - chit.g.depth) > 0.25f * chit.g.depth) continue;
        if (dot(xyz(nd), chit.g.normal) < 0.5f) continue;
        GiRes s = gi_load(in, screen_idx(cam, sp.x, sp.y));
        if (s.m == 0.0f) continue;
        float s_pdf = gi_pdf(s, chit);
        float s_jac = gi_jacobian(s, chit.point);
        if (s_jac < 1.0f / 10.0f || s_jac > 10.0f) continue;
        s_jac = rclamp(s_jac, 1.0f / 3.0f, 3.0f);
        if (gi_merge(main_, rng, s, s_pdf * s_jac)) main_pdf = s_pdf;
    }
    main_.confidence = center.confidence;
    main_.pdf = main_pdf;
    main_.v1 = center.v1;
    main_.w = res_norm(main_.w, main_pdf, 1.0f, main_.m);
    main_.w = rmin(main_.w, 5.0f);
    *result = main_;
    return true;
}
__global__ void ST_LB_GI_PREVIEW k_gi_preview(KPARAMS, int cur, u32 seed, u32 nth, const float4* __restrict__ in, float4* __restrict__ out, int reach) {
    Px p = pixel_full(cam);
    if (!p.in) return;
    Hit chit = load_hit_lut(sc, cam.curr, cam.prim_gbuffer_d0[cur], cam.prim_gbuffer_d1[cur], cam, p.x, p.y);
    GiRes r;
    if (gi_preview_px(cam, sc, chit, seed, nth, in, p, &r)) gi_store_m(cam, r, out, screen_idx(cam, p.x, p.y), p.y, reach);
}

ST_DEV void gi_resolving_px(const CameraDev& cam, const Hit& hit, const GiRes& res, const float4* __restrict__ in, Px p) {
    size_t idx = screen_idx(cam, p.x, p.y);
    float confidence; float3 radiance;
    if (hit_some(hit)) { confidence = res.confidence; radiance = res.w * gi_cosine(res, hit) * res.radiance; }
    else { confidence = 1.0f; radiance = f3s(0.f); }
    float diff_brdf = (1.0f - hit.g.metallic) / kPi;
    float3 spec = gi_spec(res, hit);
    size_t i = pix(cam, p.x, p.y);
    cam.gi_diff_samples[i] = f4(radiance * diff_brdf, confidence);
    cam.gi_spec_samples[i] = f4(radiance * spec, confidence);
    gi_store(gi_load(in, idx), cam.gi_reservoirs[0], idx);
}
__global__ void ST_LB_GI_RESOLVING k_gi_resolving(KPARAMS, int cur, const float4* __restrict__ in) {
    Px p = pixel_full(cam);
    if (!p.in) return;
    Hit hit = load_hit_lut(sc, cam.curr, cam.prim_gbuffer_d0[cur], cam.prim_gbuffer_d1[cur], cam, p.x, p.y);
    gi_resolving_px(cam, hit, gi_load(cam.gi_reservoirs[0], screen_idx(cam, p.x, p.y)), in, p);
}
__global__ void ST_LB_GI_PREVIEW k_gi_preview_resolve(KPARAMS, int cur, u32 seed, const float4* __restrict__ in, const float4* __restrict__ source) {
    Px p = pixel_full(cam);
    if (!p.in) return;
    Hit chit = load_hit_lut(sc, cam.curr, cam.prim_gbuffer_d0[cur], cam.prim_gbuffer_d1[cur], cam, p.x, p.y);
    GiRes r;
    if (!gi_preview_px(cam, sc, chit, seed, 1u, in, p, &r)) r = gi_load(cam.gi_reservoirs[0], screen_idx(cam, p.x, p.y));
    gi_resolving_px(cam, chit, r, source, p);
}

#if ST_EXACT_ONLY
__global__ void __launch_bounds__(ST_BLOCK) k_denoise_reproject(KPARAMS, int cur, const float4* __restrict__ prev_colors, const float4* __restrict__ prev_moments,
                                                                const float4* __restrict__ samples, float4* __restrict__ colors, float4* __restrict__ moments) {
    Px p = pixel_full(cam);
    if (!p.in) return;
    size_t i = pix(cam, p.x, p.y);
    float4 sample = samples[i];
    if (cam.prim_surface_map[cur][i].z == 0.0f) { store4m(cam, colors + i, sample, p.y, ST_REACH_SVGF); return; }
    float sl = luma(xyz(sample));
    Reproj rp = reproj_decode(cam.reprojection_map[i]);
    float3 color, moment;
    if (reproj_some(rp) && sample.w > 0.0f) {
        float4 pc = history_fetch(rp, prev_colors, cam.w, cam.h);
        float4 pm = history_fetch(rp, prev_moments, cam.w, cam.h);
        float hist = rmin(pm.x + 1.0f, 16.0f);
        float alpha = 1.0f / hist;
        color = lerpc(xyz(pc), xyz(sample), alpha);
        moment = f3(hist, lerpc(pm.y, sl, alpha), lerpc(pm.z, sl * sl, alpha));
    } else { color = xyz(sample); moment = f3(1.0f, sl, sl * sl); }
    store4m(cam, colors + i, f4(color, 0.0f), p.y, ST_REACH_SVGF);
    store4m(cam, moments + i, f4(moment, 0.0f), p.y, ST_REACH_SVGF);
}

struct ReprojectSignal { const float4* prev_colors; const float4* prev_moments; const float4* samples; float4* colors; float4* moments; };
ST_DEV void denoise_reproject_signal(const CameraDev& cam, size_t i, u32 y, float4 sample, const Reproj& rp, bool has_rp, const ReprojectSignal& g) {
    float sl = luma(xyz(sample));
    float3 color, moment;
    if (has_rp && sample.w > 0.0f) {
        float4 pc = history_fetch(rp, g.prev_colors, cam.w, cam.h);
        float4 pm = history_fetch(rp, g.prev_moments, cam.w, cam.h);
        float hist = rmin(pm.x + 1.0f, 16.0f);
        float alpha = 1.0f / hist;
        color = lerpc(xyz(pc), xyz(sample), alpha);
        moment = f3(hist, lerpc(pm.y, sl, alpha), lerpc(pm.z, sl * sl, alpha));
    } else { color = xyz(sample); moment = f3(1.0f, sl, sl * sl); }
    store4m(cam, g.colors + i, f4(color, 0.0f), y, ST_REACH_SVGF);
    store4m(cam, g.moments + i, f4(moment, 0.0f), y, ST_REACH_SVGF);
}
__global__ void __launch_bounds__(ST_BLOCK) k_denoise_reproject_pair(KPARAMS, int cur, const __grid_constant__ ReprojectSignal di, const __grid_constant__ ReprojectSignal gi) {
    Px p = pixel_full(cam);
    if (!p.in) return;
    size_t i = pix(cam, p.x, p.y);
    float4 sd = di.samples[i], sg = gi.samples[i];
    if (cam.prim_surface_map[cur][i].z == 0.0f) { store4m(cam, di.colors + i, sd, p.y, ST_REACH_SVGF); store4m(cam, gi.colors + i, sg, p.y, ST_REACH_SVGF); return; }
    Reproj rp = reproj_decode(cam.reprojection_map[i]);
    bool has_rp = reproj_some(rp);
    denoise_reproject_signal(cam, i, p.y, sd, rp, has_rp, di);
    denoise_reproject_signal(cam, i, p.y, sg, rp, has_rp, gi);
}

ST_DEV float sfu_ex2(float x) { float r; asm("ex2.approx.ftz.f32 %0, %1;" : "=f"(r) : "f"(x)); return r; }
ST_DEV float sfu_sqrt(float x) { float r; asm("sqrt.approx.ftz.f32 %0, %1;" : "=f"(r) : "f"(x)); return r; }
ST_DEV float sfu_rcp(float x) { float r; asm("rcp.approx.ftz.f32 %0, %1;" : "=f"(r) : "f"(x)); return r; }
template <bool FAST> ST_DEV float sv_sqrt(float x) { return FAST ? sfu_sqrt(x) : sqrtf(x); }
template <bool FAST> ST_DEV float sv_luma(float3 c) { return FAST ? __fmaf_rn(c.z, 0.0722f, __fmaf_rn(c.y, 0.7152f, c.x * 0.2126f)) : luma(c); }
template <bool FAST> ST_DEV float svgf_depth_weight(float c_depth, float s_depth, float depth_sigma) {
    float leeway = c_depth * depth_sigma;
    float diff = fabs_(s_depth - c_depth);
    if (diff >= leeway) return 0.0f;
    return FAST ? __fmaf_rn(-diff, sfu_rcp(leeway), 1.0f) : 1.0f - diff / leeway;
}
template <bool FAST> ST_DEV float svgf_normal_weight(float3 c_normal, float3 s_normal) {
    float d = FAST ? __fmaf_rn(s_normal.z, c_normal.z, __fmaf_rn(s_normal.y, c_normal.y, s_normal.x * c_normal.x)) : dot(s_normal, c_normal);
    return pow_det(rmax(d, 0.0f), 64.0f);
}
template <bool FAST> ST_DEV float svgf_luma_weight(float sqrt_center_luma, float sample_luma, float luma_sigma) {
    float lw = fabs_(sqrt_center_luma - sv_sqrt<FAST>(sample_luma)) * luma_sigma;
    return FAST ? sfu_ex2(lw * -1.44269504088896341f) : exp_det(-lw);
}

template <bool FAST>
__global__ void __launch_bounds__(ST_BLOCK) k_denoise_variance(KPARAMS, int cur) {
    Px p = pixel_full(cam);
    if (!p.in) return;
    size_t i = pix(cam, p.x, p.y);
    const float4* __restrict__ snd = cam.surface_nd;
    const float4* __restrict__ di_colors = cam.di_diff_curr_colors; const float4* __restrict__ gi_colors = cam.gi_diff_curr_colors;
    float4 cnd = snd[i];
    float4 cdi = di_colors[i], cgi = gi_colors[i];
    if (cnd.w == 0.0f) { cam.di_diff_stash[i] = cdi; cam.gi_diff_stash[i] = cgi; return; }
    float4 mdi = cam.di_diff_moments[cur][i], mgi = cam.gi_diff_moments[cur][i];
    float di_var, gi_var;
    if (mdi.x >= 4.0f) { di_var = mdi.z - sq(mdi.y); gi_var = mgi.z - sq(mgi.y); }
    else {
        float3 cn = xyz(cnd);
        float scdl = sv_sqrt<FAST>(sv_luma<FAST>(xyz(cdi))), scgl = sv_sqrt<FAST>(sv_luma<FAST>(xyz(cgi)));
        float3 sdi = f3s(0.f), sgi = f3s(0.f);
        int ox = -2, oy = -2;
        for (;;) {
            int sx = (int)p.x + ox, sy = (int)p.y + oy;
            if (cam_contains_i(cam.curr, sx, sy)) {
                size_t si = pix(cam, (u32)sx, (u32)sy);
                float4 nds = snd[si];
                if (nds.w != 0.0f) {
                    float common = svgf_depth_weight<FAST>(cnd.w, nds.w, 0.2f);
                    float nw = svgf_normal_weight<FAST>(cn, xyz(nds));
                    float sl = sv_luma<FAST>(xyz(di_colors[si]));
                    float w = svgf_luma_weight<FAST>(scdl, sl, 1.0f) * common * nw;
                    sdi = sdi + f3(sl, sl * sl, 1.0f) * f3s(w);
                    float gl = sv_luma<FAST>(xyz(gi_colors[si]));
                    float wg = svgf_luma_weight<FAST>(scgl, gl, 1.0f) * common * nw;
                    sgi = sgi + f3(gl, gl * gl, 1.0f) * f3s(wg);
                }
            }
            ox += 1;
            if (ox == 3) { ox = -3; oy += 1; if (oy == 3) break; }
        }
        { float m1 = sdi.x / sdi.z, m2 = sdi.y / sdi.z; di_var = fabs_(m2 - m1 * m1) * 4.0f; }
        { float m1 = sgi.x / sgi.z, m2 = sgi.y / sgi.z; gi_var = fabs_(m2 - m1 * m1) * 4.0f; }
    }
    di_var = rmax(di_var, 0.0f); gi_var = rmax(gi_var, 0.0f);
    cam.di_diff_stash[i] = f4(xyz(cdi), di_var);
    cam.gi_diff_stash[i] = f4(xyz(cgi), gi_var);
}

#ifndef ST_WAVELET_MIN_BLOCKS
#define ST_WAVELET_MIN_BLOCKS 10
#endif
template <bool FAST, bool PAIR_IN>
__global__ void __launch_bounds__(ST_BLOCK, ST_WAVELET_MIN_BLOCKS) k_denoise_wavelet(KPARAMS, int cur, u32 frame, u32 stride, float strength,
                                                              const float4* __restrict__ di_in, float4* __restrict__ di_out,
                                                              const float4* __restrict__ gi_in, float4* __restrict__ gi_out,
                                                              const float4* __restrict__ pair_in, float4* __restrict__ pair_out) {
    Px p = pixel_full(cam);
    if (!p.in) return;
    size_t i = pix(cam, p.x, p.y);
    const float4* __restrict__ snd = cam.surface_nd;
    float4 cnd = snd[i];
    float4 cdi, cgi;
    if (PAIR_IN) { F8 c = ld8(pair_in + 2 * i); cdi = c.a; cgi = c.b; } else cdi = di_in[i];
    float3 cdc = xyz(cdi); float cdv = cdi.w;
    if (cnd.w == 0.0f) { if (pair_out) pair_out[2 * i] = f4(cdc, cdv); else di_out[i] = f4(cdc, cdv); return; }
    float4 bn = blue_noise(sc, p.x, p.y, frame);
    if (!PAIR_IN) cgi = gi_in[i];
    float3 cgc = xyz(cgi); float cgv = cgi.w;
    float3 cn = xyz(cnd);
    float scdl = sv_sqrt<FAST>(sv_luma<FAST>(cdc)), scgl = sv_sqrt<FAST>(sv_luma<FAST>(cgc));
    float ls_di = lerpc(2.5f, 0.5f, sv_sqrt<FAST>(cdv));
    float ls_gi = lerpc(1.0f, 0.0f, sv_sqrt<FAST>(cgv));
    float depth_sigma = 0.33f / strength;
    float2 jf = (f2(bn.z, bn.w) - f2(0.5f, 0.5f)) * ((float)stride - 1.0f) * 0.5f;
    int jx = to_i32_sat(jf.x), jy = to_i32_sat(jf.y);
    float sdw = 1.0f; float3 sdc = cdc; float sdv = cdv;
    float sgw = 1.0f; float3 sgc = cgc; float sgv = cgv;
#pragma unroll
    for (int oy = -1; oy <= 1; oy++) {
#pragma unroll
        for (int ox = -1; ox <= 1; ox++) {
            if (ox == 0 && oy == 0) continue;
            int sx = (int)p.x + jx + ox * (int)stride, sy = (int)p.y + jy + oy * (int)stride;
            if (!cam_contains_i(cam.curr, sx, sy)) continue;
            size_t si = pix(cam, (u32)sx, (u32)sy);
            float4 nds = snd[si];
            if (nds.w == 0.0f) continue;
            float dw = svgf_depth_weight<FAST>(cnd.w, nds.w, depth_sigma);
            float nw = svgf_normal_weight<FAST>(cn, xyz(nds));
// ... 73 lines not shown
        }
    }
    ST_DEV void store(float4* __restrict__ di_out, float4* __restrict__ gi_out, float4* __restrict__ pair_out, size_t i) const {
        float4 odi, ogi;
        if (FAST) {
            float rd = sfu_rcp(sdw), rg = sfu_rcp(sgw);
            odi = f4(sdc * rd, sdv * (rd * rd));
            ogi = f4(sgc * rg, sgv * (rg * rg));
        } else {
            odi = f4(sdc / sdw, sdv / (sdw * sdw));
            ogi = f4(sgc / sgw, sgv / (sgw * sgw));
        }
        if (pair_out) st8(pair_out + 2 * i, odi, ogi);
        else { di_out[i] = odi; gi_out[i] = ogi; }
    }
};

template <int S, int J, int TW, int TH> struct WaveletTile {
    static constexpr int HL = S + J, BW = TW + 2 * HL, BH = TH + 2 * HL;
    static constexpr u32 BOX_BYTES = (u32)(BW * BH * 16);
    static constexpr u32 PLANE = (BOX_BYTES + 127u) & ~127u;
    static constexpr u32 SMEM = 3u * PLANE + 128u;
};

#ifndef ST_WAVELET_TILED_MINB
#define ST_WAVELET_TILED_MINB 1
#endif
template <bool FAST, int S, int J, int TW, int TH>
__global__ void __launch_bounds__(TW * TH, (TW * TH <= 256 && S <= 8) ? ST_WAVELET_TILED_MINB : 1) k_denoise_wavelet_tiled(KPARAMS, u32 frame, float strength,
                                                                   const __grid_constant__ CUtensorMap tm_nd, const __grid_constant__ CUtensorMap tm_di,
                                                                   const __grid_constant__ CUtensorMap tm_gi,
                                                                   float4* __restrict__ di_out, float4* __restrict__ gi_out, float4* __restrict__ pair_out,
                                                                   u32* __restrict__ errors) {
    typedef WaveletTile<S, J, TW, TH> T;
    extern __shared__ unsigned char s_raw[];
    __shared__ __align__(8) unsigned long long s_bar;
    const int tx = (int)threadIdx.x % TW, ty = (int)threadIdx.x / TW;
    const int x0 = (int)blockIdx.x * TW, y0 = cam.y0 + (int)blockIdx.y * TH;
    const u32 bar = smem_addr(&s_bar);
    const u32 raw = smem_addr(s_raw);
    const u32 base = (raw + 127u) & ~127u;
    if (threadIdx.x == 0) { mbar_init(bar, 1u); mbar_fence_init(); }
    __syncthreads();
    if (threadIdx.x == 0) {
        mbar_expect_tx(bar, 3u * T::BOX_BYTES);
        tma_load_2d(base, &tm_nd, (x0 - T::HL) * 2, y0 - T::HL, bar);
        tma_load_2d(base + T::PLANE, &tm_di, (x0 - T::HL) * 2, y0 - T::HL, bar);
        tma_load_2d(base + 2u * T::PLANE, &tm_gi, (x0 - T::HL) * 2, y0 - T::HL, bar);
    }
    const u32 px = (u32)(x0 + tx), py = (u32)(y0 + ty);
    const bool in = px < (u32)cam.w && py < (u32)cam.y1;
    int jo = 0;
    if (J > 0 && in) {
        float4 bn = blue_noise(sc, px, py, frame);
        float2 jf = (f2(bn.z, bn.w) - f2(0.5f, 0.5f)) * ((float)S - 1.0f) * 0.5f;
        jo = to_i32_sat(jf.y) * T::BW + to_i32_sat(jf.x);
    }
    {
        bool done = false;
        for (u32 spin = 0; spin < (1u << 20) && !done; spin++) done = mbar_try_wait(bar, 0u);
        if (!done) { if (threadIdx.x == 0) atomicAdd(errors, 1u); return; }
    }
    if (!in) return;
    const float4* __restrict__ t_nd = reinterpret_cast<const float4*>(s_raw + (base - raw));
    const float4* __restrict__ t_di = reinterpret_cast<const float4*>(s_raw + (base - raw) + T::PLANE);
    const float4* __restrict__ t_gi = reinterpret_cast<const float4*>(s_raw + (base - raw) + 2u * T::PLANE);
// ... 8 lines not shown
#pragma unroll
    for (int oy = -1; oy <= 1; oy++) {
#pragma unroll
        for (int ox = -1; ox <= 1; ox++) {
            if (ox == 0 && oy == 0) continue;
            const int k = cj + oy * S * T::BW + ox * S;
            float4 nds = t_nd[k];
            if (nds.w == 0.0f) continue;
            float dw, nw;
            if (!ctr.geometry(nds, &dw, &nw)) continue;
            ctr.add(dw, nw, t_di[k], t_gi[k]);
        }
    }
    ctr.store(di_out, gi_out, pair_out, i);
}

ST_DEV float3 compose_px(const CameraDev& cam, const SceneDev& sc, int cur, u32 mode, const float4* __restrict__ di_diff, const float4* __restrict__ gi_diff, size_t i) {
    float3 color;
    if (mode == 0u) {
        GBuf g = gbuf_unpack(sc, cam.prim_gbuffer_d0[cur][i], cam.prim_gbuffer_d1[cur][i]);
        float3 dd = xyz(di_diff[i]), ds = xyz(cam.di_spec_samples[i]), gd = xyz(gi_diff[i]), gs = xyz(cam.gi_spec_samples[i]);
        if (g.depth != 0.0f) color = g.emissive + (dd + gd) * xyz(g.base_color) + ds + gs;
        else color = dd;
    } else if (mode == 1u) color = xyz(di_diff[i]);
    else if (mode == 2u) color = xyz(cam.di_spec_samples[i]);
    else if (mode == 3u) color = xyz(gi_diff[i]);
    else if (mode == 4u) color = xyz(cam.gi_spec_samples[i]);
    else if (mode == 5u) color = xyz(cam.ref_colors[i]);
    else if (mode == 6u) { float4 c = cam.ref_colors[i]; color = xyz(c) / c.w; }
    else color = f3s(0.f);
    return color;
}
__global__ void __launch_bounds__(ST_BLOCK) k_composition(KPARAMS, int cur, u32 mode, const float4* __restrict__ di_diff, const float4* __restrict__ gi_diff) {
    Px p = pixel_full(cam);
    if (!p.in) return;
    size_t i = pix(cam, p.x, p.y);
    cam.output[i] = f4(compose_px(cam, sc, cur, mode, di_diff, gi_diff, i), 1.0f);
}

#define TAA_TW 32
#define TAA_TH 8
static const float kTaaClipEps = 1e-8f;
ST_DEV float taa_max(float a, float b) { return a > b ? a : b; }
ST_DEV float taa_min(float a, float b) { return a < b ? a : b; }
ST_DEV float3 taa_tonemap(float3 c) { const float d = 1.0f + taa_max(taa_max(c.x, c.y), c.z); return f3(c.x / d, c.y / d, c.z / d); }
ST_DEV float3 taa_untonemap(float3 t) { const float d = 1.0f - taa_max(taa_max(t.x, t.y), t.z); return f3(t.x / d, t.y / d, t.z / d); }
ST_DEV float3 taa_ycocg(float3 c) { return f3((0.25f * c.x + 0.5f * c.y) + 0.25f * c.z, 0.5f * c.x - 0.5f * c.z, (-0.25f * c.x + 0.5f * c.y) - 0.25f * c.z); }
ST_DEV float3 taa_rgb(float3 v) { const float t = v.x - v.z; return f3(t + v.y, v.x + v.z, t - v.y); }
ST_DEV void taa_cr_weights(float f, float w[4]) {
    w[0] = f * (-0.5f + f * (1.0f - 0.5f * f));
    w[1] = 1.0f + (f * f) * (-2.5f + 1.5f * f);
    w[2] = f * (0.5f + f * (2.0f - 1.5f * f));
    w[3] = (f * f) * (-0.5f + 0.5f * f);
}
__global__ void __launch_bounds__(TAA_TW * TAA_TH) k_taa_resolve(KPARAMS, int cur, u32 mode, const float4* __restrict__ di_diff, const float4* __restrict__ gi_diff,
                                                                 const float4* __restrict__ hist_in, float4* __restrict__ hist_out, float4 jit) {
    const int HW = TAA_TW + 2, HH = TAA_TH + 2;
    __shared__ float4 s_t[HW * HH];
    const int bx = (int)blockIdx.x * TAA_TW - 1, by = (int)blockIdx.y * TAA_TH - 1;
    for (int k = threadIdx.x; k < HW * HH; k += TAA_TW * TAA_TH) {
        const int x = min(max(bx + k % HW, 0), cam.w - 1), y = min(max(by + k / HW, 0), cam.h - 1);
        s_t[k] = f4(taa_tonemap(compose_px(cam, sc, cur, mode, di_diff, gi_diff, pix(cam, (u32)x, (u32)y))), 0.0f);
    }
    __syncthreads();
    const int tx = threadIdx.x % TAA_TW, ty = threadIdx.x / TAA_TW;
    const u32 px = blockIdx.x * TAA_TW + tx, py = blockIdx.y * TAA_TH + ty;
// ... 926 lines not shown
        float nt = ((i + 0.3f) / 32.0f) * t_max;
        float dt = nt - t; t = nt;
        float3 np = vp + t * rd;
        float3 rs, ext; float ms; atm_scattering(np, &rs, &ms, &ext);
        float3 st_ = exp3(-dt * ext);
        float3 sun_t = atm_lut(tl, 256, 64, np, sun_dir);
        float3 psi = atm_lut(sl, 32, 32, np, sun_dir);
        float3 ri = rs * (rp * sun_t + psi);
        float3 mi = ms * (mp * sun_t + psi);
        float3 ins = ri + mi;
        float3 si = (ins - ins * st_) / ext;
        lum = lum + si * tr;
        tr = tr * st_;
    }
    out[y * 256 + x] = f4(round_f16(lum.x), round_f16(lum.y), round_f16(lum.z), 1.0f);
}

#endif

__global__ void k_math_shading(int op, const float* __restrict__ a, const float* __restrict__ b, float* __restrict__ out, long n) {
    long i = (long)blockIdx.x * blockDim.x + threadIdx.x;
    if (i >= n) return;
    float r = 0.f, x = a[i], y = b[i];
    switch (op) {
        case 0: r = sin_det(x); break; case 1: r = cos_det(x); break; case 2: r = exp_det(x); break;
        case 3: r = pow_det(x, y); break; case 4: r = sqrtf(x); break; case 5: r = x / y; break;
        case 6: r = acos_det(x); break; case 7: r = atan2_det(x, y); break;
    }
    out[i] = r;
}

static dim3 grid_full(const CameraDev& cam) { return dim3((cam.w + TILE_W - 1) / TILE_W, (cam.y1 - cam.y0 + TILE_H - 1) / TILE_H); }
static dim3 grid_half(const CameraDev& cam) { int hw = 8 * (((cam.w + 7) / 8) / 2); return dim3((hw + TILE_W - 1) / TILE_W, (cam.y1 - cam.y0 + TILE_H - 1) / TILE_H); }
#define HALF_LAUNCH(kernel, c, st, ...) do { dim3 g_ = grid_half(c); if (g_.x > 0 && g_.y > 0) kernel<<<g_, ST_BLOCK, 0, st>>>(__VA_ARGS__); } while (0)

void launch_di_sampling(const CameraDev& c, const SceneDev& s, int cur, u32 seed, u32 frame, const LightGridDev* lg, cudaStream_t st) {
    if (lg) k_di_sampling<true><<<grid_full(c), ST_BLOCK, 0, st>>>(c, s, cur, seed, frame, *lg); else k_di_sampling<false><<<grid_full(c), ST_BLOCK, 0, st>>>(c, s, cur, seed, frame, LightGridDev{});
}
void launch_di_temporal(const CameraDev& c, const SceneDev& s, int cur, u32 seed, cudaStream_t st) { k_di_temporal<<<grid_full(c), ST_BLOCK, 0, st>>>(c, s, cur, seed); }
void launch_di_spatial_pick(const CameraDev& c, const SceneDev& s, int cur, u32 seed, u32 frame, cudaStream_t st) { HALF_LAUNCH(k_di_spatial_pick, c, st, c, s, cur, seed, frame); }
void launch_spatial_trace(const CameraDev& c, const SceneDev& s, const float4* d0, const float4* d1, float4* d2, cudaStream_t st) { k_spatial_trace<<<grid_full(c), ST_BLOCK, 0, st>>>(c, s, d0, d1, d2); }
void launch_di_spatial_sample(const CameraDev& c, const SceneDev& s, u32 seed, u32 frame, cudaStream_t st) { HALF_LAUNCH(k_di_spatial_sample, c, st, c, s, seed, frame); }
void launch_di_resolving(const CameraDev& c, const SceneDev& s, int cur, const EnvMapDev* em, cudaStream_t st) {
    if (em) k_di_resolving<true><<<grid_full(c), ST_BLOCK, 0, st>>>(c, s, cur, *em); else k_di_resolving<false><<<grid_full(c), ST_BLOCK, 0, st>>>(c, s, cur, EnvMapDev{});
}
void launch_gi_reprojection(const CameraDev& c, const SceneDev& s, int cur, cudaStream_t st) { k_gi_reprojection<<<grid_full(c), ST_BLOCK, 0, st>>>(c, s, cur); }
void launch_gi_sampling_a(const CameraDev& c, const SceneDev& s, int cur, u32 seed, u32 frame, bool nmap, const TexFilterDev* tf, const EnvMapDev* em,
                          cudaStream_t st) {
    const TexFilterDev tnone{};
    const TexFilterDev& t = tf ? *tf : tnone;
    const EnvMapDev enone{};
    const EnvMapDev& m = em ? *em : enone;
#define ST_GSA(N_, T_, E_) HALF_LAUNCH((k_gi_sampling_a<N_, T_, E_>), c, st, c, s, cur, seed, frame, t, m)
#define ST_GSA_E(N_, T_) do { if (em && em->cdf) ST_GSA(N_, T_, ENV_SAMPLED); else ST_GSA(N_, T_, ENV_NONE); } while (0)
    if (tf) { if (nmap) ST_GSA_E(true, true); else ST_GSA_E(false, true); }
    else { if (nmap) ST_GSA_E(true, false); else ST_GSA_E(false, false); }
#undef ST_GSA_E
#undef ST_GSA
}
void launch_gi_sampling_b(const CameraDev& c, const SceneDev& s, int cur, u32 seed, u32 frame, const LightGridDev* lg, const EnvMapDev* em, cudaStream_t st) {
    const LightGridDev none{};
    const LightGridDev& g = lg ? *lg : none;
    const EnvMapDev enone{};
    const EnvMapDev& m = em ? *em : enone;
#define ST_GSB(L_, E_) HALF_LAUNCH((k_gi_sampling_b<L_, E_>), c, st, c, s, cur, seed, frame, g, m)
#define ST_GSB_E(L_) do { if (!em) ST_GSB(L_, ENV_NONE); else if (em->cdf) ST_GSB(L_, ENV_SAMPLED); else ST_GSB(L_, ENV_MAP); } while (0)
    if (lg) ST_GSB_E(true); else ST_GSB_E(false);
#undef ST_GSB_E
#undef ST_GSB
}
void launch_gi_temporal(const CameraDev& c, const SceneDev& s, int cur, u32 seed, u32 frame, int inline_reprojection, cudaStream_t st) { k_gi_temporal<<<grid_full(c), ST_BLOCK, 0, st>>>(c, s, cur, seed, frame, inline_reprojection); }
void launch_gi_spatial_pick(const CameraDev& c, const SceneDev& s, int cur, u32 seed, u32 frame, cudaStream_t st) { HALF_LAUNCH(k_gi_spatial_pick, c, st, c, s, cur, seed, frame); }
void launch_gi_spatial_sample(const CameraDev& c, const SceneDev& s, u32 seed, u32 frame, cudaStream_t st) { HALF_LAUNCH(k_gi_spatial_sample, c, st, c, s, seed, frame); }
void launch_gi_preview(const CameraDev& c, const SceneDev& s, int cur, u32 seed, u32 nth, const float4* in, float4* out, int mirror_reach, cudaStream_t st) { k_gi_preview<<<grid_full(c), ST_BLOCK, 0, st>>>(c, s, cur, seed, nth, in, out, mirror_reach); }
void launch_gi_resolving(const CameraDev& c, const SceneDev& s, int cur, const float4* in, cudaStream_t st) { k_gi_resolving<<<grid_full(c), ST_BLOCK, 0, st>>>(c, s, cur, in); }
void launch_di_sample_temporal(const CameraDev& c, const SceneDev& s, int cur, u32 seed_sampling, u32 seed_temporal, u32 frame, const LightGridDev* lg, cudaStream_t st) {
    if (lg) k_di_sample_temporal<true><<<grid_full(c), ST_BLOCK, 0, st>>>(c, s, cur, seed_sampling, seed_temporal, frame, *lg);
    else k_di_sample_temporal<false><<<grid_full(c), ST_BLOCK, 0, st>>>(c, s, cur, seed_sampling, seed_temporal, frame, LightGridDev{});
}
void launch_di_spatial_fused(const CameraDev& c, const SceneDev& s, int cur, u32 seed_pick, u32 seed_sample, u32 frame, cudaStream_t st) { HALF_LAUNCH(k_di_spatial_fused, c, st, c, s, cur, seed_pick, seed_sample, frame); }
void launch_gi_sampling_fused(const CameraDev& c, const SceneDev& s, int cur, u32 seed_a, u32 seed_b, u32 frame, bool nmap, const LightGridDev* lg, const TexFilterDev* tf,
                              const EnvMapDev* em, cudaStream_t st) {
    const LightGridDev none{};
    const LightGridDev& g = lg ? *lg : none;
    const TexFilterDev tnone{};
    const TexFilterDev& t = tf ? *tf : tnone;
    const EnvMapDev enone{};
    const EnvMapDev& m = em ? *em : enone;
#define ST_GSF(N_, L_, T_, E_) HALF_LAUNCH((k_gi_sampling_fused<N_, L_, T_, E_>), c, st, c, s, cur, seed_a, seed_b, frame, g, t, m)
#define ST_GSF_E(N_, L_, T_) do { if (!em) ST_GSF(N_, L_, T_, ENV_NONE); else if (em->cdf) ST_GSF(N_, L_, T_, ENV_SAMPLED); else ST_GSF(N_, L_, T_, ENV_MAP); } while (0)
    if (tf) {
        if (lg) { if (nmap) ST_GSF_E(true, true, true); else ST_GSF_E(false, true, true); }
        else { if (nmap) ST_GSF_E(true, false, true); else ST_GSF_E(false, false, true); }
    } else {
        if (lg) { if (nmap) ST_GSF_E(true, true, false); else ST_GSF_E(false, true, false); }
        else { if (nmap) ST_GSF_E(true, false, false); else ST_GSF_E(false, false, false); }
    }
#undef ST_GSF_E
#undef ST_GSF
}
void launch_gi_spatial_fused(const CameraDev& c, const SceneDev& s, int cur, u32 seed_pick, u32 seed_sample, u32 frame, cudaStream_t st) { HALF_LAUNCH(k_gi_spatial_fused, c, st, c, s, cur, seed_pick, seed_sample, frame); }
void launch_gi_preview_resolve(const CameraDev& c, const SceneDev& s, int cur, u32 seed, const float4* in, const float4* source, cudaStream_t st) { k_gi_preview_resolve<<<grid_full(c), ST_BLOCK, 0, st>>>(c, s, cur, seed, in, source); }
void launch_math_shading(int op, const float* a, const float* b, float* out, long n, cudaStream_t st) { k_math_shading<<<(unsigned)((n + 255) / 256), 256, 0, st>>>(op, a, b, out, n); }
#if ST_EXACT_ONLY
void launch_prim_gbuffer(const CameraDev& c, const SceneDev& s, int cur, int with_reprojection, bool nmap, const TexFilterDev* tf, cudaStream_t st) {
    const TexFilterDev none{};
    const TexFilterDev& t = tf ? *tf : none;
#define ST_PG(N_, T_) k_prim_gbuffer<N_, T_><<<grid_full(c), ST_BLOCK, 0, st>>>(c, s, cur, with_reprojection, t)
    if (tf) { if (nmap) ST_PG(true, true); else ST_PG(false, true); }
    else { if (nmap) ST_PG(true, false); else ST_PG(false, false); }
#undef ST_PG
}
void launch_frame_reprojection(const CameraDev& c, const SceneDev& s, int cur, cudaStream_t st) { k_frame_reprojection<<<grid_full(c), ST_BLOCK, 0, st>>>(c, s, cur); }
void launch_denoise_reproject(const CameraDev& c, const SceneDev& s, int cur, const float4* pc, const float4* pm, const float4* smp, float4* col, float4* mom, cudaStream_t st) { k_denoise_reproject<<<grid_full(c), ST_BLOCK, 0, st>>>(c, s, cur, pc, pm, smp, col, mom); }
void launch_denoise_reproject_pair(const CameraDev& c, const SceneDev& s, int cur, cudaStream_t st) {
    ReprojectSignal di{c.di_diff_prev_colors, c.di_diff_moments[cur ^ 1], c.di_diff_samples, c.di_diff_curr_colors, c.di_diff_moments[cur]};
    ReprojectSignal gi{c.gi_diff_prev_colors, c.gi_diff_moments[cur ^ 1], c.gi_diff_samples, c.gi_diff_curr_colors, c.gi_diff_moments[cur]};
    k_denoise_reproject_pair<<<grid_full(c), ST_BLOCK, 0, st>>>(c, s, cur, di, gi);
}
void launch_denoise_variance(const CameraDev& c, const SceneDev& s, int cur, bool fast, cudaStream_t st) {
    if (fast) k_denoise_variance<true><<<grid_full(c), ST_BLOCK, 0, st>>>(c, s, cur); else k_denoise_variance<false><<<grid_full(c), ST_BLOCK, 0, st>>>(c, s, cur);
}
void launch_denoise_wavelet(const CameraDev& c, const SceneDev& s, int cur, u32 frame, u32 stride, float strength, const float4* di_in, float4* di_out, const float4* gi_in, float4* gi_out,
                            const float4* pair_in, float4* pair_out, bool fast, cudaStream_t st) {
#define ST_WG(F_, P_) k_denoise_wavelet<F_, P_><<<grid_full(c), ST_BLOCK, 0, st>>>(c, s, cur, frame, stride, strength, di_in, di_out, gi_in, gi_out, pair_in, pair_out)
    if (pair_in) { if (fast) ST_WG(true, true); else ST_WG(false, true); }
    else { if (fast) ST_WG(true, false); else ST_WG(false, false); }
#undef ST_WG
}
template <int TW, int TH> struct VarianceTile {
    static constexpr int HX = 3, HY = 2, BW = TW + 2 * HX, BH = TH + 2 * HY;
    static constexpr u32 BOX_BYTES = (u32)(BW * BH * 16);
    static constexpr u32 PLANE = (BOX_BYTES + 127u) & ~127u;
    static constexpr u32 SMEM = 3u * PLANE + 128u;
};
template <bool FAST, int TW, int TH>
__global__ void __launch_bounds__(TW * TH) k_denoise_variance_tiled(KPARAMS, int cur, const __grid_constant__ CUtensorMap tm_nd, const __grid_constant__ CUtensorMap tm_di,
                                                                    const __grid_constant__ CUtensorMap tm_gi, u32* __restrict__ errors) {
    typedef VarianceTile<TW, TH> T;
    extern __shared__ unsigned char s_raw[];
    __shared__ __align__(8) unsigned long long s_bar;
    const int tx = (int)threadIdx.x % TW, ty = (int)threadIdx.x / TW;
    const int x0 = (int)blockIdx.x * TW, y0 = cam.y0 + (int)blockIdx.y * TH;
    const u32 bar = smem_addr(&s_bar);
    const u32 raw = smem_addr(s_raw);
    const u32 base = (raw + 127u) & ~127u;
    if (threadIdx.x == 0) { mbar_init(bar, 1u); mbar_fence_init(); }
    __syncthreads();
    if (threadIdx.x == 0) {
        mbar_expect_tx(bar, 3u * T::BOX_BYTES);
        tma_load_2d(base, &tm_nd, (x0 - T::HX) * 2, y0 - T::HY, bar);
        tma_load_2d(base + T::PLANE, &tm_di, (x0 - T::HX) * 2, y0 - T::HY, bar);
        tma_load_2d(base + 2u * T::PLANE, &tm_gi, (x0 - T::HX) * 2, y0 - T::HY, bar);
    }
    const u32 px = (u32)(x0 + tx), py = (u32)(y0 + ty);
    const bool in = px < (u32)cam.w && py < (u32)cam.y1;
    const size_t i = in ? pix(cam, px, py) : 0;
    float4 mdi = f4zero(), mgi = f4zero();
    if (in) { mdi = cam.di_diff_moments[cur][i]; mgi = cam.gi_diff_moments[cur][i]; }
    {
        bool done = false;
        for (u32 spin = 0; spin < (1u << 20) && !done; spin++) done = mbar_try_wait(bar, 0u);
        if (!done) { if (threadIdx.x == 0) atomicAdd(errors, 1u); return; }
    }
    if (!in) return;
    const float4* __restrict__ t_nd = reinterpret_cast<const float4*>(s_raw + (base - raw));
    const float4* __restrict__ t_di = reinterpret_cast<const float4*>(s_raw + (base - raw) + T::PLANE);
    const float4* __restrict__ t_gi = reinterpret_cast<const float4*>(s_raw + (base - raw) + 2u * T::PLANE);
    const int c = (ty + T::HY) * T::BW + (tx + T::HX);
    float4 cnd = t_nd[c];
    float4 cdi = t_di[c], cgi = t_gi[c];
// ... 48 lines not shown
    Key key(plane, w, h, bw, bh);
    auto it = cache.find(key);
    if (it != cache.end()) { *out = it->second; return true; }
    TensorMapEncodeFn enc = tensor_map_encoder();
    if (!enc) {
        static bool warned = false;
        if (!warned) { warned = true; std::fprintf(stderr, "strolle_b200: cuTensorMapEncodeTiled is not available from this driver; the tile-staged SVGF kernels are off\n"); }
        return false;
    }
    cuuint64_t dims[2] = {(cuuint64_t)w * 2u, (cuuint64_t)h};
    cuuint64_t strides[1] = {(cuuint64_t)w * 16u};
    cuuint32_t box[2] = {(cuuint32_t)bw * 2u, (cuuint32_t)bh};
    cuuint32_t estr[2] = {1u, 1u};
    CUtensorMap tm;
    if (enc(&tm, CU_TENSOR_MAP_DATA_TYPE_UINT64, 2, const_cast<float4*>(plane), dims, strides, box, estr, CU_TENSOR_MAP_INTERLEAVE_NONE,
            CU_TENSOR_MAP_SWIZZLE_NONE, CU_TENSOR_MAP_L2_PROMOTION_L2_256B, CU_TENSOR_MAP_FLOAT_OOB_FILL_NONE) != CUDA_SUCCESS) return false;
    if (cache.size() > 4096) cache.clear();
    cache[key] = tm; *out = tm;
    return true;
}
template <bool FAST, int S, int J, int TW, int TH>
static bool wavelet_tiled_go(const CameraDev& c, const SceneDev& s, u32 frame, float strength, const float4* di_in, float4* di_out, const float4* gi_in, float4* gi_out,
                             float4* pair_out, u32* errors, cudaStream_t st) {
    typedef WaveletTile<S, J, TW, TH> T;
    if (T::BW * 2 > 256 || T::BH > 256) return false;
    CUtensorMap tn, td, tg;
    if (!wavelet_tensor_map(c.surface_nd, c.w, c.h, T::BW, T::BH, &tn) || !wavelet_tensor_map(di_in, c.w, c.h, T::BW, T::BH, &td) ||
        !wavelet_tensor_map(gi_in, c.w, c.h, T::BW, T::BH, &tg)) return false;
    auto kern = k_denoise_wavelet_tiled<FAST, S, J, TW, TH>;
    static bool attr_set[64] = {};
    int dev = 0; cudaGetDevice(&dev); dev &= 63;
    if (!attr_set[dev]) { if (cudaFuncSetAttribute(kern, cudaFuncAttributeMaxDynamicSharedMemorySize, (int)T::SMEM) != cudaSuccess) { cudaGetLastError(); return false; } attr_set[dev] = true; }
    dim3 grid((c.w + TW - 1) / TW, (c.y1 - c.y0 + TH - 1) / TH);
    kern<<<grid, TW * TH, T::SMEM, st>>>(c, s, frame, strength, tn, td, tg, di_out, gi_out, pair_out, errors);
    return true;
}
template <bool FAST, int S, int J>
static bool wavelet_tiled_cfg(int cfg, const CameraDev& c, const SceneDev& s, u32 frame, float strength, const float4* di_in, float4* di_out, const float4* gi_in, float4* gi_out,
                              float4* pair_out, u32* errors, cudaStream_t st) {
    switch (cfg) {
    case 0: return wavelet_tiled_go<FAST, S, J, 32, 8>(c, s, frame, strength, di_in, di_out, gi_in, gi_out, pair_out, errors, st);
    case 1: return wavelet_tiled_go<FAST, S, J, 32, 16>(c, s, frame, strength, di_in, di_out, gi_in, gi_out, pair_out, errors, st);
    case 2: return wavelet_tiled_go<FAST, S, J, 64, 4>(c, s, frame, strength, di_in, di_out, gi_in, gi_out, pair_out, errors, st);
    case 3: return wavelet_tiled_go<FAST, S, J, 64, 8>(c, s, frame, strength, di_in, di_out, gi_in, gi_out, pair_out, errors, st);
    default: return false;
    }
}
bool launch_denoise_wavelet_tiled(const CameraDev& c, const SceneDev& s, u32 frame, u32 stride, float strength, const float4* di_in, float4* di_out, const float4* gi_in,
                                  float4* gi_out, float4* pair_out, bool fast, int cfg, u32* errors, cudaStream_t st) {
    if (c.curr.screen.x != (float)c.w || c.curr.screen.y != (float)c.h) return false;
#define ST_WT(S_, J_) (fast ? wavelet_tiled_cfg<true, S_, J_>(cfg, c, s, frame, strength, di_in, di_out, gi_in, gi_out, pair_out, errors, st) \
                            : wavelet_tiled_cfg<false, S_, J_>(cfg, c, s, frame, strength, di_in, di_out, gi_in, gi_out, pair_out, errors, st))
    switch (stride) {
    case 1: return ST_WT(1, 0);
    case 2: return ST_WT(2, 0);
    case 4: return ST_WT(4, 0);
    case 8: return ST_WT(8, 1);
    case 16: return ST_WT(16, 3);
    default: return false;
    }
#undef ST_WT
}
template <bool FAST>
static bool variance_tiled_go(const CameraDev& c, const SceneDev& s, int cur, u32* errors, cudaStream_t st) {
    typedef VarianceTile<32, 8> T;
    CUtensorMap tn, td, tg;
    if (!wavelet_tensor_map(c.surface_nd, c.w, c.h, T::BW, T::BH, &tn) || !wavelet_tensor_map(c.di_diff_curr_colors, c.w, c.h, T::BW, T::BH, &td) ||
        !wavelet_tensor_map(c.gi_diff_curr_colors, c.w, c.h, T::BW, T::BH, &tg)) return false;
    auto kern = k_denoise_variance_tiled<FAST, 32, 8>;
    static bool attr_set[64] = {};
    int dev = 0; cudaGetDevice(&dev); dev &= 63;
    if (!attr_set[dev]) { if (cudaFuncSetAttribute(kern, cudaFuncAttributeMaxDynamicSharedMemorySize, (int)T::SMEM) != cudaSuccess) { cudaGetLastError(); return false; } attr_set[dev] = true; }
    dim3 grid((c.w + 31) / 32, (c.y1 - c.y0 + 7) / 8);
    kern<<<grid, 256, T::SMEM, st>>>(c, s, cur, tn, td, tg, errors);
    return true;
}
bool launch_denoise_variance_tiled(const CameraDev& c, const SceneDev& s, int cur, bool fast, u32* errors, cudaStream_t st) {
    if (c.curr.screen.x != (float)c.w || c.curr.screen.y != (float)c.h) return false;
    return fast ? variance_tiled_go<true>(c, s, cur, errors, st) : variance_tiled_go<false>(c, s, cur, errors, st);
}
void launch_composition(const CameraDev& c, const SceneDev& s, int cur, u32 mode, const float4* di_diff, const float4* gi_diff, cudaStream_t st) { k_composition<<<grid_full(c), ST_BLOCK, 0, st>>>(c, s, cur, mode, di_diff, gi_diff); }
void launch_taa_resolve(const CameraDev& c, const SceneDev& s, int cur, u32 mode, const float4* di_diff, const float4* gi_diff, const float4* hist_in, float4* hist_out,
                        float4 jit, cudaStream_t st) {
    const dim3 grid((c.w + TAA_TW - 1) / TAA_TW, (c.h + TAA_TH - 1) / TAA_TH);
    k_taa_resolve<<<grid, TAA_TW * TAA_TH, 0, st>>>(c, s, cur, mode, di_diff, gi_diff, hist_in, hist_out, jit);
}
void launch_output_rgba8(const CameraDev& c, const SceneDev& s, uchar4* out, cudaStream_t st) { k_output_rgba8<<<grid_full(c), ST_BLOCK, 0, st>>>(c, s, out); }
void launch_exposure_histogram(const CameraDev& c, u32* state, ExposureDev p, int sms, cudaStream_t st) {
    const u32 n = (u32)c.w * (u32)c.h;
    const u32 ctas = std::max(1u, std::min((n + EXPO_THREADS - 1) / EXPO_THREADS, (u32)ST_EXPO_CTAS_PER_SM * (u32)sms));
    k_exposure_histogram<<<ctas, EXPO_THREADS, 0, st>>>(c.output, n, state, p);
#if ST_EXPO_METER_LAUNCH
    k_exposure_meter<<<1, kExposureBins, 0, st>>>(state, p);
#endif
}
void launch_output_display(const CameraDev& c, const SceneDev& s, int op, const u32* state, ExposureDev p, uchar4* out, cudaStream_t st) {
    switch (op) {
    case 1: k_output_display<1><<<grid_full(c), ST_BLOCK, 0, st>>>(c, s, out, state, p); break;
    case 2: k_output_display<2><<<grid_full(c), ST_BLOCK, 0, st>>>(c, s, out, state, p); break;
    case 3: k_output_display<3><<<grid_full(c), ST_BLOCK, 0, st>>>(c, s, out, state, p); break;
    default: k_output_display<4><<<grid_full(c), ST_BLOCK, 0, st>>>(c, s, out, state, p); break;
    }
}
static dim3 grid_of(int w, int h) { return dim3((w + TILE_W - 1) / TILE_W, (h + TILE_H - 1) / TILE_H); }
void launch_bloom_pyramid(const CameraDev& c, const BloomLevels& lv, const u32* state, ExposureDev p, int tm, BloomDev b, cudaStream_t st) {
    const int L = lv.levels;
    k_bloom_down0<<<dim3((lv.w[0] + BLOOM_TX - 1) / BLOOM_TX, (lv.h[0] + BLOOM_TY - 1) / BLOOM_TY), BLOOM_TX * BLOOM_TY, 0, st>>>(
        c.output, c.w, c.h, lv.down[0], lv.w[0], lv.h[0], state, p, tm, b);
    int tail = L;
    for (int k = 1; k < L && ST_BLOOM_TAIL_TEXELS > 0; k++) if (lv.w[k] * lv.h[k] <= ST_BLOOM_TAIL_TEXELS) { tail = k; break; }
    for (int k = 1; k < tail; k++) k_bloom_down<<<grid_of(lv.w[k], lv.h[k]), ST_BLOCK, 0, st>>>(lv.down[k - 1], lv.w[k - 1], lv.h[k - 1], lv.down[k], lv.w[k], lv.h[k]);
    if (tail < L) {
#if ST_BLOOM_TAIL_KIND == 0
        k_bloom_tail<<<1, BLOOM_TAIL_THREADS, 0, st>>>(lv, tail, b.scatter);
// ... 286 lines not shown
```

strolle_b200/csrc/kernels.h:

```cpp
#pragma once
#include <cuda_runtime.h>
#include "st_types.h"

namespace st {
typedef uint32_t u32;

void launch_prim_gbuffer(const CameraDev& c, const SceneDev& s, int cur, int with_reprojection, bool nmap, const TexFilterDev* tf, cudaStream_t st);
void launch_frame_reprojection(const CameraDev& c, const SceneDev& s, int cur, cudaStream_t st);
void launch_di_sampling(const CameraDev& c, const SceneDev& s, int cur, u32 seed, u32 frame, const LightGridDev* lg, cudaStream_t st);
void launch_di_temporal(const CameraDev& c, const SceneDev& s, int cur, u32 seed, cudaStream_t st);
void launch_di_spatial_pick(const CameraDev& c, const SceneDev& s, int cur, u32 seed, u32 frame, cudaStream_t st);
void launch_spatial_trace(const CameraDev& c, const SceneDev& s, const float4* d0, const float4* d1, float4* d2, cudaStream_t st);
void launch_di_spatial_sample(const CameraDev& c, const SceneDev& s, u32 seed, u32 frame, cudaStream_t st);
void launch_di_resolving(const CameraDev& c, const SceneDev& s, int cur, const EnvMapDev* em, cudaStream_t st);
void launch_gi_reprojection(const CameraDev& c, const SceneDev& s, int cur, cudaStream_t st);
void launch_gi_sampling_a(const CameraDev& c, const SceneDev& s, int cur, u32 seed, u32 frame, bool nmap, const TexFilterDev* tf, const EnvMapDev* em, cudaStream_t st);
void launch_gi_sampling_b(const CameraDev& c, const SceneDev& s, int cur, u32 seed, u32 frame, const LightGridDev* lg, const EnvMapDev* em, cudaStream_t st);
void launch_gi_temporal(const CameraDev& c, const SceneDev& s, int cur, u32 seed, u32 frame, int inline_reprojection, cudaStream_t st);
void launch_gi_spatial_pick(const CameraDev& c, const SceneDev& s, int cur, u32 seed, u32 frame, cudaStream_t st);
void launch_gi_spatial_sample(const CameraDev& c, const SceneDev& s, u32 seed, u32 frame, cudaStream_t st);
void launch_gi_preview(const CameraDev& c, const SceneDev& s, int cur, u32 seed, u32 nth, const float4* in, float4* out, int mirror_reach, cudaStream_t st);
void launch_gi_resolving(const CameraDev& c, const SceneDev& s, int cur, const float4* in, cudaStream_t st);
void launch_di_sample_temporal(const CameraDev& c, const SceneDev& s, int cur, u32 seed_sampling, u32 seed_temporal, u32 frame, const LightGridDev* lg, cudaStream_t st);
void launch_di_spatial_fused(const CameraDev& c, const SceneDev& s, int cur, u32 seed_pick, u32 seed_sample, u32 frame, cudaStream_t st);
void launch_gi_sampling_fused(const CameraDev& c, const SceneDev& s, int cur, u32 seed_a, u32 seed_b, u32 frame, bool nmap, const LightGridDev* lg, const TexFilterDev* tf,
                              const EnvMapDev* em, cudaStream_t st);
void launch_gi_spatial_fused(const CameraDev& c, const SceneDev& s, int cur, u32 seed_pick, u32 seed_sample, u32 frame, cudaStream_t st);
void launch_gi_preview_resolve(const CameraDev& c, const SceneDev& s, int cur, u32 seed, const float4* in, const float4* source, cudaStream_t st);
void launch_denoise_reproject(const CameraDev& c, const SceneDev& s, int cur, const float4* pc, const float4* pm, const float4* smp, float4* col, float4* mom, cudaStream_t st);
void launch_denoise_reproject_pair(const CameraDev& c, const SceneDev& s, int cur, cudaStream_t st);
void launch_denoise_variance(const CameraDev& c, const SceneDev& s, int cur, bool fast, cudaStream_t st);
void launch_denoise_wavelet(const CameraDev& c, const SceneDev& s, int cur, u32 frame, u32 stride, float strength, const float4* di_in, float4* di_out, const float4* gi_in, float4* gi_out, const float4* pair_in, float4* pair_out, bool fast, cudaStream_t st);
bool launch_denoise_wavelet_tiled(const CameraDev& c, const SceneDev& s, u32 frame, u32 stride, float strength, const float4* di_in, float4* di_out, const float4* gi_in, float4* gi_out, float4* pair_out, bool fast, int cfg, u32* errors, cudaStream_t st);
bool launch_denoise_variance_tiled(const CameraDev& c, const SceneDev& s, int cur, bool fast, u32* errors, cudaStream_t st);
void launch_composition(const CameraDev& c, const SceneDev& s, int cur, u32 mode, const float4* di_diff, const float4* gi_diff, cudaStream_t st);
// ... 132 lines not shown
```

strolle_b200/engine.py:

```python
import ctypes as C
import os

import numpy as np

_HERE = os.path.dirname(os.path.abspath(__file__))
PASS_COUNT = 27
FORMAT_RGBA32F, FORMAT_RGBA8_SRGB = 0, 1
OPT_SVGF_FAST_MATH = 1
OPT_ASYNC_OUTPUT = 2
OPT_HALO_NCCL = 3
OPT_WAVELET_TILED = 4
OPT_WAVELET_TILE_CFG = 5
OPT_FUSE_REPROJECT = 6
OPT_BVH_REUSE = 7
OPT_VARIANCE_TILED = 8
OPT_FUSED_PASSES = 11
OPT_WAVELET_PAIRED = 13
OPT_STRIP_DMA = 12
OPT_STRIP_FUSED = 10
OPT_SHADING_FAST_MATH = 9
OPT_NORMAL_MAPS = 14
OPT_BVH_REFIT = 15
OPT_LIGHT_GRID = 16
OPT_TEXTURE_FILTER = 17
# ... 146 lines not shown

def load_library():
    global _LIB
    if _LIB is not None:
        return _LIB
    path = lib_path()
    if not os.path.exists(path):
        raise StrolleError(f"{path} is missing: build it with `python -m strolle_b200.build` (no CPU fallback exists)")
    lib = C.CDLL(path)
    P, u64, i32, u32, f32p = C.c_void_p, C.c_uint64, C.c_int32, C.c_uint32, C.POINTER(C.c_float)
    sig = {
        "st_engine_create": [C.c_int, C.POINTER(P)], "st_engine_destroy": [P],
        "st_insert_mesh": [P, u64, C.POINTER(_MeshTriangle), C.c_size_t], "st_remove_mesh": [P, u64],
        "st_insert_material": [P, u64, C.POINTER(_Material)], "st_has_material": [P, u64], "st_remove_material": [P, u64],
        "st_insert_image": [P, u64, C.c_void_p, u32, u32], "st_remove_image": [P, u64], "st_set_material_textures": [P, u64, C.POINTER(_MaterialTextures)],
        "st_insert_instance": [P, u64, u64, u64, f32p], "st_remove_instance": [P, u64],
        "st_insert_light": [P, u64, C.POINTER(_Light)], "st_remove_light": [P, u64], "st_update_sun": [P, C.c_float, C.c_float],
        "st_set_environment_map": [P, C.c_void_p, u32, u32, C.c_float, C.c_float], "st_set_exposure": [P, C.c_void_p], "st_set_bloom": [P, C.c_void_p],
        "st_set_depth_of_field": [P, C.c_void_p],
        "st_create_camera": [P, C.POINTER(_Camera), C.POINTER(i32)], "st_update_camera": [P, i32, C.POINTER(_Camera)], "st_delete_camera": [P, i32],
        "st_tick": [P], "st_render_camera": [P, i32, P, C.c_int], "st_copy_output": [P, i32, P, C.c_int], "st_synchronize": [P],
        "st_set_seed_base": [P, u32], "st_set_blue_noise": [P, C.c_void_p],
        "st_read_buffer": [P, i32, C.c_char_p, C.c_void_p, C.c_size_t, C.POINTER(C.c_size_t)],
        "st_read_scene": [P, C.c_char_p, C.c_void_p, C.c_size_t, C.POINTER(C.c_size_t)],
        "st_bvh_depth": [P, C.POINTER(C.c_int)],
        "st_trace_closest": [P, C.c_void_p, C.c_size_t, C.c_void_p, f32p], "st_trace_any": [P, C.c_void_p, C.c_size_t, C.c_void_p, f32p],
        "st_device_math": [P, C.c_int, C.c_void_p, C.c_void_p, C.c_void_p, C.c_size_t],
        "st_set_stream": [P, C.c_void_p, C.c_int], "st_set_option": [P, C.c_int, C.c_int], "st_get_stat": [P, C.c_int, C.POINTER(C.c_uint64)],
        "st_count_rays": [P, C.c_int], "st_ray_count": [P, C.POINTER(C.c_uint64), C.c_int],
        "st_nccl_unique_id": [C.c_void_p], "st_nccl_init": [P, C.c_void_p, C.c_int, C.c_int],
        "st_plan_frame": [C.POINTER(C.c_int), C.c_int, u32, C.c_int, C.c_char_p, C.c_size_t],
        "st_plan_strip_order": [C.POINTER(C.c_int), C.c_int, C.c_int, C.c_char_p, C.c_size_t],
        "st_strip_bounds": [C.c_int, C.c_int, C.POINTER(C.c_int)],
        "st_render_strips": [P, i32, P, C.c_int, C.c_int, C.c_int], "st_halo_bytes": [P, C.POINTER(C.c_uint64)],
        "st_peer_export": [P, i32, C.c_void_p], "st_peer_import": [P, i32, C.c_void_p, C.c_int, C.c_int],
        "st_peer_errors": [P, i32, C.POINTER(u32)],
        "st_mark_begin": [P], "st_mark_end": [P, f32p],
        "st_enable_timing": [P, C.c_int], "st_pass_times": [P, C.c_void_p, C.c_void_p, C.c_int], "st_wavelet_times": [P, C.c_void_p, C.c_void_p, C.c_int],
        "st_camera_set_strip": [P, i32, C.c_int, C.c_int],
        "st_buffer_device_ptr": [P, i32, C.c_char_p, C.POINTER(C.c_void_p), C.POINTER(C.c_size_t)],
        "st_frame_schedule": [P, i32, C.POINTER(C.c_int), C.c_int, C.POINTER(C.c_int)], "st_render_range": [P, i32, C.c_int, C.c_int],
        "st_link_local": [C.POINTER(P), C.POINTER(i32), C.c_int],
        "st_multi_create": [C.POINTER(C.c_int), C.c_int, C.POINTER(P)],
        "st_multi_insert_mesh": [P, u64, C.POINTER(_MeshTriangle), C.c_size_t], "st_multi_remove_mesh": [P, u64],
        "st_multi_insert_material": [P, u64, C.POINTER(_Material)], "st_multi_has_material": [P, u64], "st_multi_remove_material": [P, u64],
        "st_multi_insert_image": [P, u64, C.c_void_p, u32, u32], "st_multi_remove_image": [P, u64], "st_multi_set_material_textures": [P, u64, C.POINTER(_MaterialTextures)],
        "st_multi_insert_instance": [P, u64, u64, u64, f32p], "st_multi_remove_instance": [P, u64],
        "st_multi_insert_light": [P, u64, C.POINTER(_Light)], "st_multi_remove_light": [P, u64], "st_multi_update_sun": [P, C.c_float, C.c_float],
        "st_multi_set_environment_map": [P, C.c_void_p, u32, u32, C.c_float, C.c_float], "st_multi_set_exposure": [P, C.c_void_p], "st_multi_set_bloom": [P, C.c_void_p],
        "st_multi_set_depth_of_field": [P, C.c_void_p],
        "st_multi_create_camera": [P, C.POINTER(_Camera), C.POINTER(i32)], "st_multi_update_camera": [P, i32, C.POINTER(_Camera)], "st_multi_delete_camera": [P, i32],
        "st_multi_tick": [P], "st_multi_render_camera": [P, i32, P, C.c_int], "st_multi_synchronize": [P],
        "st_multi_set_option": [P, C.c_int, C.c_int], "st_multi_set_seed_base": [P, u32], "st_multi_set_blue_noise": [P, C.c_void_p],
        "st_multi_read_buffer": [P, i32, C.c_char_p, C.c_void_p, C.c_size_t, C.POINTER(C.c_size_t)], "st_multi_peer_errors": [P, i32, C.POINTER(u32)],
        "st_multi_size": [P], "st_multi_member_camera": [P, i32, C.c_int],
        "st_bvh_builder_create": [C.POINTER(P)], "st_bvh_builder_read": [P, C.c_void_p, C.c_size_t],
        "st_bvh_builder_build": [P, C.c_void_p, C.c_size_t, C.c_int, C.c_void_p, C.c_size_t, C.POINTER(C.c_size_t), C.POINTER(u32), C.POINTER(C.c_int)],
    }
    for name, args in sig.items():
        fn = getattr(lib, name)
        fn.argtypes = args
        fn.restype = None if name == "st_engine_destroy" else C.c_int
    lib.st_bvh_builder_destroy.argtypes = [P]
    lib.st_bvh_builder_destroy.restype = None
    lib.st_multi_destroy.argtypes = [P]
    lib.st_multi_destroy.restype = None
# ... 460 lines not shown
    def set_depth_of_field(self, **fields):
        self._check(self.lib.st_multi_set_depth_of_field(self._h, _depth_of_field(fields or None)))

    def read_buffer(self, cam, name):
        n = C.c_size_t()
        self._check(self.lib.st_multi_read_buffer(self._h, cam, name.encode(), None, 0, C.byref(n)))
        out = np.empty(n.value, dtype=np.float32)
        self._check(self.lib.st_multi_read_buffer(self._h, cam, name.encode(), out.ctypes.data, n.value, C.byref(n)))
        return out

    def peer_errors(self, cam):
        n = C.c_uint32()
        self._check(self.lib.st_multi_peer_errors(self._h, cam, C.byref(n)))
        return n.value


def nccl_unique_id():
    lib = load_library()
    buf = (C.c_uint8 * 128)()
    rc = lib.st_nccl_unique_id(buf)
    if rc != 0:
        raise StrolleError(lib.st_last_error().decode())
    return bytes(buf)


def strip_bounds_native(height, world):
    lib = load_library()
    out = (C.c_int * (2 * world))()
    if lib.st_strip_bounds(int(height), int(world), out) != 0:
        raise StrolleError(lib.st_last_error().decode())
    return [(out[2 * r], out[2 * r + 1]) for r in range(world)]


def plan_strip_order(schedule, dma=True, still=False):
    lib = load_library()
    arr = (C.c_int * len(schedule))(*schedule)
    out = C.create_string_buffer(8192)
    rc = lib.st_plan_strip_order(arr, len(schedule), (int(dma) & 3) | (4 if still else 0), out, 8192)
    if rc != 0:
        raise StrolleError(lib.st_last_error().decode())
    return [x for x in out.value.decode().split(";") if x]


def plan_frame_native(schedule, frame, temporal_reach=16):
    lib = load_library()
    arr = (C.c_int * len(schedule))(*schedule)
    out = C.create_string_buffer(8192)
    rc = lib.st_plan_frame(arr, len(schedule), frame, temporal_reach, out, 8192)
    if rc != 0:
        raise StrolleError(lib.st_last_error().decode())
    items = [x for x in out.value.decode().split(";") if x]
    return [(int(a), b, int(c)) for a, b, c in (i.split(":") for i in items)]
```

Before: 3704.

## Run DI and GI ReSTIR chains on forked streams with programmatic dependent launch

Adds a per-pass read/write footprint table that tags each ReSTIR pass as belonging to the DI or GI chain. When timing is off, the frame executor forks the GI chain onto a second, low-priority stream and joins it back before the shared passes, so the two independent chains can run concurrently. Kernels are now launched through cudaLaunchKernelEx with the programmatic stream serialization attribute and begin with griddepcontrol wait/launch_dependents, which lets back-to-back kernels on the same stream overlap their launch latency. It also exposes the footprint table through the C, Rust and Python APIs, and adds event and stream overhead plus a risk of hazards if the footprints are wrong.

```diff
diff --git a/include/strolle_b200.h b/include/strolle_b200.h
--- a/include/strolle_b200.h
+++ b/include/strolle_b200.h
@@ -108,6 +108,7 @@
 int st_enable_timing(st_engine* e, int enabled);
 int st_pass_times(st_engine* e, float* ms, uint32_t* launches, int reset);
 const char* st_pass_name(int pass);
+int st_pass_footprint(int pass, int* chain, uint32_t* reads, uint32_t* writes);
 int st_wavelet_times(st_engine* e, float* ms5, uint32_t* launches5, int reset);
 enum { ST_OPT_SVGF_FAST_MATH = 1, ST_OPT_ASYNC_OUTPUT = 2, ST_OPT_HALO_NCCL = 3, ST_OPT_WAVELET_TILED = 4, ST_OPT_WAVELET_TILE_CFG = 5, ST_OPT_FUSE_REPROJECT = 6, ST_OPT_BVH_REUSE = 7, ST_OPT_VARIANCE_TILED = 8, ST_OPT_SHADING_FAST_MATH = 9, ST_OPT_STRIP_FUSED = 10, ST_OPT_FUSED_PASSES = 11, ST_OPT_STRIP_DMA = 12, ST_OPT_WAVELET_PAIRED = 13, ST_OPT_NORMAL_MAPS = 14, ST_OPT_BVH_REFIT = 15, ST_OPT_LIGHT_GRID = 16, ST_OPT_TEXTURE_FILTER = 17, ST_OPT_TEMPORAL_AA = 18, ST_OPT_ENVIRONMENT_MAP_SAMPLING = 19, ST_OPT_TONEMAPPING = 20, ST_OPT_AUTO_EXPOSURE = 21, ST_OPT_BLOOM = 22, ST_OPT_DEPTH_OF_FIELD = 23 };
 #define ST_WAVELET_PAIRED_DEFAULT 1
diff --git a/rust/strolle-b200-sys/src/lib.rs b/rust/strolle-b200-sys/src/lib.rs
--- a/rust/strolle-b200-sys/src/lib.rs
+++ b/rust/strolle-b200-sys/src/lib.rs
@@ -135,6 +135,7 @@
     pub fn st_enable_timing(e: *mut st_engine, enabled: c_int) -> c_int;
     pub fn st_pass_times(e: *mut st_engine, ms: *mut f32, launches: *mut u32, reset: c_int) -> c_int;
     pub fn st_pass_name(pass: c_int) -> *const c_char;
+    pub fn st_pass_footprint(pass: c_int, chain: *mut c_int, reads: *mut u32, writes: *mut u32) -> c_int;
     pub fn st_wavelet_times(e: *mut st_engine, ms5: *mut f32, launches5: *mut u32, reset: c_int) -> c_int;
     pub fn st_set_option(e: *mut st_engine, option: c_int, value: c_int) -> c_int;
     pub fn st_get_stat(e: *mut st_engine, stat: c_int, value: *mut u64) -> c_int;
diff --git a/strolle_b200/csrc/engine.cu b/strolle_b200/csrc/engine.cu
--- a/strolle_b200/csrc/engine.cu
+++ b/strolle_b200/csrc/engine.cu
@@ -43,6 +43,7 @@
 NcclApi g_nccl;
 }
 
+thread_local bool g_pdl_next = false;
 
 namespace st {
 
@@ -391,6 +392,7 @@
     int device = 0;
     cudaStream_t stream = nullptr; bool own_stream = true;
     cudaStream_t copy_stream = nullptr;
+    cudaStream_t gi_stream = nullptr; cudaEvent_t ev_fork = nullptr, ev_join = nullptr;
     std::unordered_map<st_handle, std::vector<st_mesh_triangle>> meshes;
     std::vector<st_material> materials; std::vector<st_handle> material_handles; bool materials_dirty = false;
     struct MatTex { st_handle tex[4]; uint32_t mask; };
@@ -996,6 +998,37 @@
     if (defocuses(e, cs) && cs->dof.p) c.output = dof_bufs(cs).frame;
     return c;
 }
+enum : uint32_t {
+    B_GBUF_CUR = 1u << 0, B_GBUF_PREV = 1u << 1, B_SURFACE_ND = 1u << 2, B_REPROJECTION_MAP = 1u << 3,
+    B_DI_RES0 = 1u << 4, B_DI_RES1 = 1u << 5, B_DI_RES2 = 1u << 6, B_DI_DIFF_SAMPLES = 1u << 7, B_DI_SPEC_SAMPLES = 1u << 8,
+    B_DI_DIFF_CURR_COLORS = 1u << 9, B_DI_DIFF_STASH = 1u << 10,
+    B_GI_RES0 = 1u << 11, B_GI_RES1 = 1u << 12, B_GI_RES2 = 1u << 13, B_GI_RES3 = 1u << 14, B_GI_D0 = 1u << 15, B_GI_D1 = 1u << 16, B_GI_D2 = 1u << 17,
+    B_GI_DIFF_SAMPLES = 1u << 18, B_GI_SPEC_SAMPLES = 1u << 19,
+};
+enum { CHAIN_NONE = 0, CHAIN_DI = 1, CHAIN_GI = 2 };
+struct PassFootprint { int pass, chain; uint32_t reads, writes; };
+static const PassFootprint kChainFootprints[] = {
+    {P_DI_SAMPLING, CHAIN_DI, B_GBUF_CUR, B_DI_RES1},
+    {P_DI_TEMPORAL, CHAIN_DI, B_GBUF_CUR | B_GBUF_PREV | B_REPROJECTION_MAP | B_DI_RES0 | B_DI_RES1, B_DI_RES1},
+    {P_DI_SPATIAL_PICK, CHAIN_DI, B_GBUF_CUR | B_SURFACE_ND | B_DI_RES1, B_DI_DIFF_SAMPLES | B_DI_DIFF_CURR_COLORS | B_DI_RES2},
+    {P_DI_SPATIAL_TRACE, CHAIN_DI, B_DI_DIFF_SAMPLES | B_DI_DIFF_CURR_COLORS, B_DI_DIFF_STASH},
+    {P_DI_SPATIAL_SAMPLE, CHAIN_DI, B_DI_DIFF_STASH | B_DI_RES1, B_DI_RES2},
+    {P_DI_RESOLVING, CHAIN_DI, B_GBUF_CUR | B_DI_RES2, B_DI_DIFF_SAMPLES | B_DI_SPEC_SAMPLES | B_DI_RES0},
+    {P_GI_REPROJECTION, CHAIN_GI, B_GBUF_CUR | B_REPROJECTION_MAP | B_GI_RES0, B_GI_RES2},
+    {P_GI_SAMPLING_A, CHAIN_GI, B_GBUF_CUR | B_GI_RES2, B_GI_D0 | B_GI_D1 | B_GI_D2},
+    {P_GI_SAMPLING_B, CHAIN_GI, B_GBUF_CUR | B_GI_RES2 | B_GI_D0 | B_GI_D1 | B_GI_D2, B_GI_RES1},
+    {P_GI_TEMPORAL, CHAIN_GI, B_GBUF_CUR | B_GBUF_PREV | B_REPROJECTION_MAP | B_GI_RES0 | B_GI_RES1 | B_GI_RES2, B_GI_RES1 | B_GI_RES2},
+    {P_GI_SPATIAL_PICK, CHAIN_GI, B_GBUF_CUR | B_SURFACE_ND | B_GI_RES1, B_GI_D0 | B_GI_D1 | B_GI_RES2},
+    {P_GI_SPATIAL_TRACE, CHAIN_GI, B_GI_D0 | B_GI_D1, B_GI_D2},
+    {P_GI_SPATIAL_SAMPLE, CHAIN_GI, B_GI_D2 | B_GI_RES1, B_GI_RES2},
+    {P_GI_PREVIEW, CHAIN_GI, B_GBUF_CUR | B_SURFACE_ND | B_GI_RES0 | B_GI_RES1 | B_GI_RES2 | B_GI_RES3, B_GI_RES3 | B_GI_RES0 | B_GI_DIFF_SAMPLES | B_GI_SPEC_SAMPLES},
+    {P_GI_RESOLVING, CHAIN_GI, B_GBUF_CUR | B_GI_RES0 | B_GI_RES1 | B_GI_RES2, B_GI_DIFF_SAMPLES | B_GI_SPEC_SAMPLES | B_GI_RES0},
+};
+static const PassFootprint* chain_footprint(int pass) {
+    for (const PassFootprint& f : kChainFootprints) if (f.pass == pass) return &f;
+    return nullptr;
+}
+static int chain_of(int pass) { const PassFootprint* f = chain_footprint(pass); return f ? f->chain : CHAIN_NONE; }
 static void build_schedule(st_engine* e, CameraSlot* cs, std::vector<Step>* steps, const StripExt* ext = nullptr) {
     GpuCamera jc, jp; float4 jit;
     const bool taa = taa_cameras(e, cs, &jc, &jp, &jit);
@@ -1474,6 +1507,12 @@
 int st_copy_output(st_engine* e, st_camera_handle h, void* host_out, int format);
 const char* st_last_error(void) { return g_err.c_str(); }
 const char* st_pass_name(int pass) { return (pass >= 0 && pass < P_COUNT) ? kPassNames[pass] : ""; }
+int st_pass_footprint(int pass, int* chain, uint32_t* reads, uint32_t* writes) {
+    if (!chain || !reads || !writes) return fail(ST_ERR_INVALID, "null argument");
+    const PassFootprint* f = chain_footprint(pass);
+    *chain = f ? f->chain : CHAIN_NONE; *reads = f ? f->reads : 0u; *writes = f ? f->writes : 0u;
+    return ST_OK;
+}
 
 int st_engine_create(int device, st_engine** out) {
     if (!out) return fail(ST_ERR_INVALID, "out is null");
@@ -1512,6 +1551,7 @@
     if (e->comm) g_nccl.CommDestroy(e->comm);
     if (e->own_stream) cudaStreamDestroy(e->stream);
     if (e->copy_stream) cudaStreamDestroy(e->copy_stream);
+    if (e->gi_stream) { cudaStreamSynchronize(e->gi_stream); cudaStreamDestroy(e->gi_stream); cudaEventDestroy(e->ev_fork); cudaEventDestroy(e->ev_join); }
     delete e;
 }
 
@@ -1862,6 +1902,45 @@
     cs->taa_hist[0] = (float4*)cs->taa.p; cs->taa_hist[1] = (float4*)((char*)cs->taa.p + bytes);
     return ST_OK;
 }
+static int run_steps(st_engine* e, const std::vector<Step>& steps, int first, int last) {
+    bool di = false, gi = false;
+    for (int i = first; i <= last; i++) { di |= chain_of(steps[i].pass) == CHAIN_DI; gi |= chain_of(steps[i].pass) == CHAIN_GI; }
+    if (e->timing) {
+        for (int i = first; i <= last; i++) e->run_timed(steps[i].pass, steps[i].run, steps[i].sub);
+        return ST_OK;
+    }
+    auto run = [&](const Step& s, cudaStream_t st, bool pdl) { g_pdl_next = pdl; s.run(st); g_pdl_next = false; e->pass_launches[s.pass]++; };
+    if (!di || !gi) {
+        for (int i = first; i <= last; i++) run(steps[i], e->stream, i > first);
+        return ST_OK;
+    }
+    if (!e->gi_stream) {
+        int least = 0, greatest = 0;
+        CK(cudaDeviceGetStreamPriorityRange(&least, &greatest));
+        CK(cudaStreamCreateWithPriority(&e->gi_stream, cudaStreamNonBlocking, least));
+        CK(cudaEventCreateWithFlags(&e->ev_fork, cudaEventDisableTiming));
+        CK(cudaEventCreateWithFlags(&e->ev_join, cudaEventDisableTiming));
+    }
+    cudaError_t err = cudaSuccess;
+    auto ck = [&](cudaError_t c) { if (err == cudaSuccess) err = c; };
+    bool forked = false, main_kernel = false, gi_kernel = false;
+    for (int i = first; i <= last; i++) {
+        const Step& s = steps[i];
+        const int chain = chain_of(s.pass);
+        if (chain != CHAIN_NONE && !forked) {
+            ck(cudaEventRecord(e->ev_fork, e->stream)); ck(cudaStreamWaitEvent(e->gi_stream, e->ev_fork, 0)); forked = true; main_kernel = gi_kernel = false;
+        }
+        if (chain == CHAIN_NONE && forked) {
+            ck(cudaEventRecord(e->ev_join, e->gi_stream)); ck(cudaStreamWaitEvent(e->stream, e->ev_join, 0)); forked = false; main_kernel = gi_kernel = false;
+        }
+        bool& prev = chain == CHAIN_GI ? gi_kernel : main_kernel;
+        run(s, chain == CHAIN_GI ? e->gi_stream : e->stream, prev);
+        prev = true;
+    }
+    if (forked) { ck(cudaEventRecord(e->ev_join, e->gi_stream)); ck(cudaStreamWaitEvent(e->stream, e->ev_join, 0)); }
+    if (err != cudaSuccess) return fail(ST_ERR_CUDA, std::string("frame fork / join: ") + cudaGetErrorString(err));
+    return ST_OK;
+}
 int st_render_range(st_engine* e, st_camera_handle h, int first, int last) {
     CameraSlot* cs = e ? get_camera(e, h) : nullptr;
     if (!cs) return fail(ST_ERR_NOT_FOUND, "unknown camera");
@@ -1874,7 +1953,7 @@
     if ((rc = ensure_dof_state(e, cs))) return rc;
     std::vector<Step> steps; build_schedule(e, cs, &steps);
     if (last < 0 || last >= (int)steps.size()) last = (int)steps.size() - 1;
-    for (int i = std::max(first, 0); i <= last; i++) e->run_timed(steps[i].pass, steps[i].run, steps[i].sub);
+    if ((rc = run_steps(e, steps, std::max(first, 0), last))) return rc;
     CK(cudaGetLastError());
     return ST_OK;
 }
@@ -1938,6 +2017,7 @@
     if (!e) return fail(ST_ERR_INVALID, "null engine");
     CK(cudaSetDevice(e->device)); CK(cudaStreamSynchronize(e->stream));
     if (e->copy_stream) CK(cudaStreamSynchronize(e->copy_stream));
+    if (e->gi_stream) CK(cudaStreamSynchronize(e->gi_stream));
     for (CameraSlot* c : e->cameras) for (int k = 0; k < 2; k++) if (c->side[k]) CK(cudaStreamSynchronize(c->side[k]));
     return ST_OK;
 }
diff --git a/strolle_b200/csrc/kernels.cu b/strolle_b200/csrc/kernels.cu
--- a/strolle_b200/csrc/kernels.cu
+++ b/strolle_b200/csrc/kernels.cu
@@ -5,6 +5,7 @@
 #include <map>
 #include <mutex>
 #include <tuple>
+#include <utility>
 #include <vector>
 #include "st_device.cuh"
 #include "kernels.h"
@@ -19,6 +20,18 @@
 #endif
 
 namespace ST_NS {
+
+#define ST_PDL_ENTER() asm volatile("griddepcontrol.wait;\n\tgriddepcontrol.launch_dependents;" ::: "memory")
+template <typename... KArgs, typename... Args>
+static void launch_k(void (*kern)(KArgs...), dim3 grid, dim3 block, size_t smem, cudaStream_t st, Args&&... args) {
+    cudaLaunchConfig_t cfg = {};
+    cfg.gridDim = grid; cfg.blockDim = block; cfg.dynamicSmemBytes = smem; cfg.stream = st;
+    cudaLaunchAttribute attr[1];
+    attr[0].id = cudaLaunchAttributeProgrammaticStreamSerialization; attr[0].val.programmaticStreamSerializationAllowed = 1;
+    cfg.attrs = attr; cfg.numAttrs = g_pdl_next ? 1 : 0;
+    g_pdl_next = false;
+    cudaLaunchKernelEx(&cfg, kern, std::forward<Args>(args)...);
+}
 
 #define TILE_W 16
 #define TILE_H 8
@@ -130,6 +143,7 @@
 ST_DEV float4 frame_reprojection_px(const CameraDev& cam, int cur, Px p, float4 surface_texel, float4 vel);
 template <bool NMAP, bool TEXF>
 __global__ void ST_LB_PRIM_GBUFFER k_prim_gbuffer(KPARAMS, int cur, int with_reprojection, const __grid_constant__ TexFilterDev tf) {
+    ST_PDL_ENTER();
     ST_TRACE_STACK();
     Px p = pixel_full(cam);
     if (!p.in) return;
@@ -202,6 +216,7 @@
     return reproj_encode(rp);
 }
 __global__ void __launch_bounds__(ST_BLOCK) k_frame_reprojection(KPARAMS, int cur) {
+    ST_PDL_ENTER();
     Px p = pixel_full(cam);
     if (!p.in) return;
     size_t i = pix(cam, p.x, p.y);
@@ -225,6 +240,7 @@
 }
 template <bool LGRID>
 __global__ void ST_LB_DI_SAMPLING k_di_sampling(KPARAMS, int cur, u32 seed, u32 frame, const __grid_constant__ LightGridDev lg) {
+    ST_PDL_ENTER();
     ST_TRACE_STACK();
     Px p = pixel_full(cam);
     if (!p.in) return;
@@ -270,6 +286,7 @@
     return main_;
 }
 __global__ void ST_LB_DI_TEMPORAL k_di_temporal(KPARAMS, int cur, u32 seed) {
+    ST_PDL_ENTER();
     Px p = pixel_full(cam);
     if (!p.in) return;
     size_t lhs_idx = screen_idx(cam, p.x, p.y);
@@ -279,6 +296,7 @@
 }
 template <bool LGRID>
 __global__ void ST_LB_DI_SAMPLING k_di_sample_temporal(KPARAMS, int cur, u32 seed_sampling, u32 seed_temporal, u32 frame, const __grid_constant__ LightGridDev lg) {
+    ST_PDL_ENTER();
     ST_TRACE_STACK();
     Px p = pixel_full(cam);
     if (!p.in) return;
@@ -336,6 +354,7 @@
     tex_store(buf_d1, cam, ax, g.y, o.a1); tex_store(buf_d1, cam, bx, g.y, o.b1);
 }
 __global__ void ST_LB_DI_SPATIAL_PICK k_di_spatial_pick(KPARAMS, int cur, u32 seed, u32 frame) {
+    ST_PDL_ENTER();
     Px g = pixel_half(cam);
     if (!g.in) return;
     store_pair_texels(cam, di_spatial_pick_pair(cam, sc, cur, seed, frame, g), cam.di_diff_samples, cam.di_diff_curr_colors, g);
@@ -348,6 +367,7 @@
     return f4(occ ? 0.0f : 1.0f, d1.z, d1.w, 0.0f);
 }
 __global__ void ST_LB_SPATIAL_TRACE k_spatial_trace(KPARAMS, const float4* __restrict__ buf_d0, const float4* __restrict__ buf_d1, float4* __restrict__ buf_d2) {
+    ST_PDL_ENTER();
     ST_TRACE_STACK();
     Px p = pixel_full(cam);
     if (!p.in) return;
@@ -389,11 +409,13 @@
     if (cam_contains_u(cam.curr, op.x, op.y)) { size_t oi = screen_idx(cam, op.x, op.y); di_store(di_load(in, oi), out, oi); }
 }
 __global__ void __launch_bounds__(ST_BLOCK) k_di_spatial_sample(KPARAMS, u32 seed, u32 frame) {
+    ST_PDL_ENTER();
     Px g = pixel_half(cam);
     if (!g.in) return;
     di_spatial_sample_pair(cam, seed, frame, g, tex_or_zero(cam.di_diff_stash, cam, g.x * 2u, g.y), tex_or_zero(cam.di_diff_stash, cam, g.x * 2u + 1u, g.y));
 }
 __global__ void ST_LB_DI_SPATIAL_PICK k_di_spatial_fused(KPARAMS, int cur, u32 seed_pick, u32 seed_sample, u32 frame) {
+    ST_PDL_ENTER();
     ST_TRACE_STACK();
     Px g = pixel_half(cam);
     if (!g.in) return;
@@ -405,6 +427,7 @@
 
 template <bool ENVM>
 __global__ void ST_LB_DI_RESOLVING k_di_resolving(KPARAMS, int cur, const __grid_constant__ EnvMapDev em) {
+    ST_PDL_ENTER();
     ST_TRACE_STACK();
     Px p = pixel_full(cam);
     if (!p.in) return;
@@ -445,6 +468,7 @@
     return res;
 }
 __global__ void __launch_bounds__(ST_BLOCK) k_gi_reprojection(KPARAMS, int cur) {
+    ST_PDL_ENTER();
     Px p = pixel_full(cam);
     if (!p.in) return;
     Hit hit = load_hit_lut(sc, cam.curr, cam.prim_gbuffer_d0[cur], cam.prim_gbuffer_d1[cur], cam, p.x, p.y);
@@ -505,6 +529,7 @@
 }
 template <bool NMAP, bool TEXF, int ENVM>
 __global__ void ST_LB_GI_SAMPLING_A k_gi_sampling_a(KPARAMS, int cur, u32 seed, u32 frame, const __grid_constant__ TexFilterDev tf, const __grid_constant__ EnvMapDev em) {
+    ST_PDL_ENTER();
     ST_TRACE_STACK();
     Px g = pixel_half(cam);
     if (!g.in) return;
@@ -588,6 +613,7 @@
 }
 template <bool LGRID, int ENVM>
 __global__ void ST_LB_GI_SAMPLING_B k_gi_sampling_b(KPARAMS, int cur, u32 seed, u32 frame, const __grid_constant__ LightGridDev lg, const __grid_constant__ EnvMapDev em) {
+    ST_PDL_ENTER();
     ST_TRACE_STACK();
     Px g = pixel_half(cam);
     if (!g.in) return;
@@ -597,6 +623,7 @@
 template <bool NMAP, bool LGRID, bool TEXF, int ENVM>
 __global__ void ST_LB_GI_SAMPLING_B k_gi_sampling_fused(KPARAMS, int cur, u32 seed_a, u32 seed_b, u32 frame, const __grid_constant__ LightGridDev lg,
                                                         const __grid_constant__ TexFilterDev tf, const __grid_constant__ EnvMapDev em) {
+    ST_PDL_ENTER();
     ST_TRACE_STACK();
     Px g = pixel_half(cam);
     if (!g.in) return;
@@ -606,6 +633,7 @@
 }
 
 __global__ void ST_LB_GI_TEMPORAL k_gi_temporal(KPARAMS, int cur, u32 seed, u32 frame, int inline_reprojection) {
+    ST_PDL_ENTER();
     Px p = pixel_full(cam);
     if (!p.in) return;
     bool tracing = gi_tracing_frame(frame);
@@ -707,6 +735,7 @@
     return o;
 }
 __global__ void ST_LB_GI_SPATIAL_PICK k_gi_spatial_pick(KPARAMS, int cur, u32 seed, u32 frame) {
+    ST_PDL_ENTER();
     Px g = pixel_half(cam);
     if (!g.in) return;
     store_pair_texels(cam, gi_spatial_pick_pair(cam, sc, cur, seed, frame, g), cam.gi_d0, cam.gi_d1, g);
@@ -744,11 +773,13 @@
     if (cam_contains_u(cam.curr, op.x, op.y)) { size_t oi = screen_idx(cam, op.x, op.y); gi_store_m(cam, gi_load(in, oi), out, oi, op.y, cam.gi_mirror_reach); }
 }
 __global__ void ST_LB_GI_SPATIAL_SAMPLE k_gi_spatial_sample(KPARAMS, u32 seed, u32 frame) {
+    ST_PDL_ENTER();
     Px g = pixel_half(cam);
     if (!g.in) return;
     gi_spatial_sample_pair(cam, seed, frame, g, tex_or_zero(cam.gi_d2, cam, g.x * 2u, g.y), tex_or_zero(cam.gi_d2, cam, g.x * 2u + 1u, g.y));
 }
 __global__ void ST_LB_GI_SPATIAL_PICK k_gi_spatial_fused(KPARAMS, int cur, u32 seed_pick, u32 seed_sample, u32 frame) {
+    ST_PDL_ENTER();
     ST_TRACE_STACK();
     Px g = pixel_half(cam);
     if (!g.in) return;
@@ -796,6 +827,7 @@
     return true;
 }
 __global__ void ST_LB_GI_PREVIEW k_gi_preview(KPARAMS, int cur, u32 seed, u32 nth, const float4* __restrict__ in, float4* __restrict__ out, int reach) {
+    ST_PDL_ENTER();
     Px p = pixel_full(cam);
     if (!p.in) return;
     Hit chit = load_hit_lut(sc, cam.curr, cam.prim_gbuffer_d0[cur], cam.prim_gbuffer_d1[cur], cam, p.x, p.y);
@@ -816,12 +848,14 @@
     gi_store(gi_load(in, idx), cam.gi_reservoirs[0], idx);
 }
 __global__ void ST_LB_GI_RESOLVING k_gi_resolving(KPARAMS, int cur, const float4* __restrict__ in) {
+    ST_PDL_ENTER();
     Px p = pixel_full(cam);
     if (!p.in) return;
     Hit hit = load_hit_lut(sc, cam.curr, cam.prim_gbuffer_d0[cur], cam.prim_gbuffer_d1[cur], cam, p.x, p.y);
     gi_resolving_px(cam, hit, gi_load(cam.gi_reservoirs[0], screen_idx(cam, p.x, p.y)), in, p);
 }
 __global__ void ST_LB_GI_PREVIEW k_gi_preview_resolve(KPARAMS, int cur, u32 seed, const float4* __restrict__ in, const float4* __restrict__ source) {
+    ST_PDL_ENTER();
     Px p = pixel_full(cam);
     if (!p.in) return;
     Hit chit = load_hit_lut(sc, cam.curr, cam.prim_gbuffer_d0[cur], cam.prim_gbuffer_d1[cur], cam, p.x, p.y);
@@ -833,6 +867,7 @@
 #if ST_EXACT_ONLY
 __global__ void __launch_bounds__(ST_BLOCK) k_denoise_reproject(KPARAMS, int cur, const float4* __restrict__ prev_colors, const float4* __restrict__ prev_moments,
                                                                 const float4* __restrict__ samples, float4* __restrict__ colors, float4* __restrict__ moments) {
+    ST_PDL_ENTER();
     Px p = pixel_full(cam);
     if (!p.in) return;
     size_t i = pix(cam, p.x, p.y);
@@ -869,6 +904,7 @@
     store4m(cam, g.moments + i, f4(moment, 0.0f), y, ST_REACH_SVGF);
 }
 __global__ void __launch_bounds__(ST_BLOCK) k_denoise_reproject_pair(KPARAMS, int cur, const __grid_constant__ ReprojectSignal di, const __grid_constant__ ReprojectSignal gi) {
+    ST_PDL_ENTER();
     Px p = pixel_full(cam);
     if (!p.in) return;
     size_t i = pix(cam, p.x, p.y);
@@ -902,6 +938,7 @@
 
 template <bool FAST>
 __global__ void __launch_bounds__(ST_BLOCK) k_denoise_variance(KPARAMS, int cur) {
+    ST_PDL_ENTER();
     Px p = pixel_full(cam);
     if (!p.in) return;
     size_t i = pix(cam, p.x, p.y);
@@ -953,6 +990,7 @@
                                                               const float4* __restrict__ di_in, float4* __restrict__ di_out,
                                                               const float4* __restrict__ gi_in, float4* __restrict__ gi_out,
                                                               const float4* __restrict__ pair_in, float4* __restrict__ pair_out) {
+    ST_PDL_ENTER();
     Px p = pixel_full(cam);
     if (!p.in) return;
     size_t i = pix(cam, p.x, p.y);
@@ -1092,6 +1130,7 @@
                                                                    const __grid_constant__ CUtensorMap tm_gi,
                                                                    float4* __restrict__ di_out, float4* __restrict__ gi_out, float4* __restrict__ pair_out,
                                                                    u32* __restrict__ errors) {
+    ST_PDL_ENTER();
     typedef WaveletTile<S, J, TW, TH> T;
     extern __shared__ unsigned char s_raw[];
     __shared__ __align__(8) unsigned long long s_bar;
@@ -1166,6 +1205,7 @@
     return color;
 }
 __global__ void __launch_bounds__(ST_BLOCK) k_composition(KPARAMS, int cur, u32 mode, const float4* __restrict__ di_diff, const float4* __restrict__ gi_diff) {
+    ST_PDL_ENTER();
     Px p = pixel_full(cam);
     if (!p.in) return;
     size_t i = pix(cam, p.x, p.y);
@@ -2158,19 +2198,19 @@
 
 static dim3 grid_full(const CameraDev& cam) { return dim3((cam.w + TILE_W - 1) / TILE_W, (cam.y1 - cam.y0 + TILE_H - 1) / TILE_H); }
 static dim3 grid_half(const CameraDev& cam) { int hw = 8 * (((cam.w + 7) / 8) / 2); return dim3((hw + TILE_W - 1) / TILE_W, (cam.y1 - cam.y0 + TILE_H - 1) / TILE_H); }
-#define HALF_LAUNCH(kernel, c, st, ...) do { dim3 g_ = grid_half(c); if (g_.x > 0 && g_.y > 0) kernel<<<g_, ST_BLOCK, 0, st>>>(__VA_ARGS__); } while (0)
+#define HALF_LAUNCH(kernel, c, st, ...) do { dim3 g_ = grid_half(c); if (g_.x > 0 && g_.y > 0) launch_k(kernel, g_, ST_BLOCK, 0, st, __VA_ARGS__); } while (0)
 
 void launch_di_sampling(const CameraDev& c, const SceneDev& s, int cur, u32 seed, u32 frame, const LightGridDev* lg, cudaStream_t st) {
-    if (lg) k_di_sampling<true><<<grid_full(c), ST_BLOCK, 0, st>>>(c, s, cur, seed, frame, *lg); else k_di_sampling<false><<<grid_full(c), ST_BLOCK, 0, st>>>(c, s, cur, seed, frame, LightGridDev{});
-}
-void launch_di_temporal(const CameraDev& c, const SceneDev& s, int cur, u32 seed, cudaStream_t st) { k_di_temporal<<<grid_full(c), ST_BLOCK, 0, st>>>(c, s, cur, seed); }
+    if (lg) launch_k(k_di_sampling<true>, grid_full(c), ST_BLOCK, 0, st, c, s, cur, seed, frame, *lg); else launch_k(k_di_sampling<false>, grid_full(c), ST_BLOCK, 0, st, c, s, cur, seed, frame, LightGridDev{});
+}
+void launch_di_temporal(const CameraDev& c, const SceneDev& s, int cur, u32 seed, cudaStream_t st) { launch_k(k_di_temporal, grid_full(c), ST_BLOCK, 0, st, c, s, cur, seed); }
 void launch_di_spatial_pick(const CameraDev& c, const SceneDev& s, int cur, u32 seed, u32 frame, cudaStream_t st) { HALF_LAUNCH(k_di_spatial_pick, c, st, c, s, cur, seed, frame); }
-void launch_spatial_trace(const CameraDev& c, const SceneDev& s, const float4* d0, const float4* d1, float4* d2, cudaStream_t st) { k_spatial_trace<<<grid_full(c), ST_BLOCK, 0, st>>>(c, s, d0, d1, d2); }
+void launch_spatial_trace(const CameraDev& c, const SceneDev& s, const float4* d0, const float4* d1, float4* d2, cudaStream_t st) { launch_k(k_spatial_trace, grid_full(c), ST_BLOCK, 0, st, c, s, d0, d1, d2); }
 void launch_di_spatial_sample(const CameraDev& c, const SceneDev& s, u32 seed, u32 frame, cudaStream_t st) { HALF_LAUNCH(k_di_spatial_sample, c, st, c, s, seed, frame); }
 void launch_di_resolving(const CameraDev& c, const SceneDev& s, int cur, const EnvMapDev* em, cudaStream_t st) {
-    if (em) k_di_resolving<true><<<grid_full(c), ST_BLOCK, 0, st>>>(c, s, cur, *em); else k_di_resolving<false><<<grid_full(c), ST_BLOCK, 0, st>>>(c, s, cur, EnvMapDev{});
-}
-void launch_gi_reprojection(const CameraDev& c, const SceneDev& s, int cur, cudaStream_t st) { k_gi_reprojection<<<grid_full(c), ST_BLOCK, 0, st>>>(c, s, cur); }
+    if (em) launch_k(k_di_resolving<true>, grid_full(c), ST_BLOCK, 0, st, c, s, cur, *em); else launch_k(k_di_resolving<false>, grid_full(c), ST_BLOCK, 0, st, c, s, cur, EnvMapDev{});
+}
+void launch_gi_reprojection(const CameraDev& c, const SceneDev& s, int cur, cudaStream_t st) { launch_k(k_gi_reprojection, grid_full(c), ST_BLOCK, 0, st, c, s, cur); }
 void launch_gi_sampling_a(const CameraDev& c, const SceneDev& s, int cur, u32 seed, u32 frame, bool nmap, const TexFilterDev* tf, const EnvMapDev* em,
                           cudaStream_t st) {
     const TexFilterDev tnone{};
@@ -2195,14 +2235,14 @@
 #undef ST_GSB_E
 #undef ST_GSB
 }
-void launch_gi_temporal(const CameraDev& c, const SceneDev& s, int cur, u32 seed, u32 frame, int inline_reprojection, cudaStream_t st) { k_gi_temporal<<<grid_full(c), ST_BLOCK, 0, st>>>(c, s, cur, seed, frame, inline_reprojection); }
+void launch_gi_temporal(const CameraDev& c, const SceneDev& s, int cur, u32 seed, u32 frame, int inline_reprojection, cudaStream_t st) { launch_k(k_gi_temporal, grid_full(c), ST_BLOCK, 0, st, c, s, cur, seed, frame, inline_reprojection); }
 void launch_gi_spatial_pick(const CameraDev& c, const SceneDev& s, int cur, u32 seed, u32 frame, cudaStream_t st) { HALF_LAUNCH(k_gi_spatial_pick, c, st, c, s, cur, seed, frame); }
 void launch_gi_spatial_sample(const CameraDev& c, const SceneDev& s, u32 seed, u32 frame, cudaStream_t st) { HALF_LAUNCH(k_gi_spatial_sample, c, st, c, s, seed, frame); }
-void launch_gi_preview(const CameraDev& c, const SceneDev& s, int cur, u32 seed, u32 nth, const float4* in, float4* out, int mirror_reach, cudaStream_t st) { k_gi_preview<<<grid_full(c), ST_BLOCK, 0, st>>>(c, s, cur, seed, nth, in, out, mirror_reach); }
-void launch_gi_resolving(const CameraDev& c, const SceneDev& s, int cur, const float4* in, cudaStream_t st) { k_gi_resolving<<<grid_full(c), ST_BLOCK, 0, st>>>(c, s, cur, in); }
+void launch_gi_preview(const CameraDev& c, const SceneDev& s, int cur, u32 seed, u32 nth, const float4* in, float4* out, int mirror_reach, cudaStream_t st) { launch_k(k_gi_preview, grid_full(c), ST_BLOCK, 0, st, c, s, cur, seed, nth, in, out, mirror_reach); }
+void launch_gi_resolving(const CameraDev& c, const SceneDev& s, int cur, const float4* in, cudaStream_t st) { launch_k(k_gi_resolving, grid_full(c), ST_BLOCK, 0, st, c, s, cur, in); }
 void launch_di_sample_temporal(const CameraDev& c, const SceneDev& s, int cur, u32 seed_sampling, u32 seed_temporal, u32 frame, const LightGridDev* lg, cudaStream_t st) {
-    if (lg) k_di_sample_temporal<true><<<grid_full(c), ST_BLOCK, 0, st>>>(c, s, cur, seed_sampling, seed_temporal, frame, *lg);
-    else k_di_sample_temporal<false><<<grid_full(c), ST_BLOCK, 0, st>>>(c, s, cur, seed_sampling, seed_temporal, frame, LightGridDev{});
+    if (lg) launch_k(k_di_sample_temporal<true>, grid_full(c), ST_BLOCK, 0, st, c, s, cur, seed_sampling, seed_temporal, frame, *lg);
+    else launch_k(k_di_sample_temporal<false>, grid_full(c), ST_BLOCK, 0, st, c, s, cur, seed_sampling, seed_temporal, frame, LightGridDev{});
 }
 void launch_di_spatial_fused(const CameraDev& c, const SceneDev& s, int cur, u32 seed_pick, u32 seed_sample, u32 frame, cudaStream_t st) { HALF_LAUNCH(k_di_spatial_fused, c, st, c, s, cur, seed_pick, seed_sample, frame); }
 void launch_gi_sampling_fused(const CameraDev& c, const SceneDev& s, int cur, u32 seed_a, u32 seed_b, u32 frame, bool nmap, const LightGridDev* lg, const TexFilterDev* tf,
@@ -2226,30 +2266,30 @@
 #undef ST_GSF
 }
 void launch_gi_spatial_fused(const CameraDev& c, const SceneDev& s, int cur, u32 seed_pick, u32 seed_sample, u32 frame, cudaStream_t st) { HALF_LAUNCH(k_gi_spatial_fused, c, st, c, s, cur, seed_pick, seed_sample, frame); }
-void launch_gi_preview_resolve(const CameraDev& c, const SceneDev& s, int cur, u32 seed, const float4* in, const float4* source, cudaStream_t st) { k_gi_preview_resolve<<<grid_full(c), ST_BLOCK, 0, st>>>(c, s, cur, seed, in, source); }
+void launch_gi_preview_resolve(const CameraDev& c, const SceneDev& s, int cur, u32 seed, const float4* in, const float4* source, cudaStream_t st) { launch_k(k_gi_preview_resolve, grid_full(c), ST_BLOCK, 0, st, c, s, cur, seed, in, source); }
 void launch_math_shading(int op, const float* a, const float* b, float* out, long n, cudaStream_t st) { k_math_shading<<<(unsigned)((n + 255) / 256), 256, 0, st>>>(op, a, b, out, n); }
 #if ST_EXACT_ONLY
 void launch_prim_gbuffer(const CameraDev& c, const SceneDev& s, int cur, int with_reprojection, bool nmap, const TexFilterDev* tf, cudaStream_t st) {
     const TexFilterDev none{};
     const TexFilterDev& t = tf ? *tf : none;
-#define ST_PG(N_, T_) k_prim_gbuffer<N_, T_><<<grid_full(c), ST_BLOCK, 0, st>>>(c, s, cur, with_reprojection, t)
+#define ST_PG(N_, T_) launch_k(k_prim_gbuffer<N_, T_>, grid_full(c), ST_BLOCK, 0, st, c, s, cur, with_reprojection, t)
     if (tf) { if (nmap) ST_PG(true, true); else ST_PG(false, true); }
     else { if (nmap) ST_PG(true, false); else ST_PG(false, false); }
 #undef ST_PG
 }
-void launch_frame_reprojection(const CameraDev& c, const SceneDev& s, int cur, cudaStream_t st) { k_frame_reprojection<<<grid_full(c), ST_BLOCK, 0, st>>>(c, s, cur); }
-void launch_denoise_reproject(const CameraDev& c, const SceneDev& s, int cur, const float4* pc, const float4* pm, const float4* smp, float4* col, float4* mom, cudaStream_t st) { k_denoise_reproject<<<grid_full(c), ST_BLOCK, 0, st>>>(c, s, cur, pc, pm, smp, col, mom); }
+void launch_frame_reprojection(const CameraDev& c, const SceneDev& s, int cur, cudaStream_t st) { launch_k(k_frame_reprojection, grid_full(c), ST_BLOCK, 0, st, c, s, cur); }
+void launch_denoise_reproject(const CameraDev& c, const SceneDev& s, int cur, const float4* pc, const float4* pm, const float4* smp, float4* col, float4* mom, cudaStream_t st) { launch_k(k_denoise_reproject, grid_full(c), ST_BLOCK, 0, st, c, s, cur, pc, pm, smp, col, mom); }
 void launch_denoise_reproject_pair(const CameraDev& c, const SceneDev& s, int cur, cudaStream_t st) {
     ReprojectSignal di{c.di_diff_prev_colors, c.di_diff_moments[cur ^ 1], c.di_diff_samples, c.di_diff_curr_colors, c.di_diff_moments[cur]};
     ReprojectSignal gi{c.gi_diff_prev_colors, c.gi_diff_moments[cur ^ 1], c.gi_diff_samples, c.gi_diff_curr_colors, c.gi_diff_moments[cur]};
-    k_denoise_reproject_pair<<<grid_full(c), ST_BLOCK, 0, st>>>(c, s, cur, di, gi);
+    launch_k(k_denoise_reproject_pair, grid_full(c), ST_BLOCK, 0, st, c, s, cur, di, gi);
 }
 void launch_denoise_variance(const CameraDev& c, const SceneDev& s, int cur, bool fast, cudaStream_t st) {
-    if (fast) k_denoise_variance<true><<<grid_full(c), ST_BLOCK, 0, st>>>(c, s, cur); else k_denoise_variance<false><<<grid_full(c), ST_BLOCK, 0, st>>>(c, s, cur);
+    if (fast) launch_k(k_denoise_variance<true>, grid_full(c), ST_BLOCK, 0, st, c, s, cur); else launch_k(k_denoise_variance<false>, grid_full(c), ST_BLOCK, 0, st, c, s, cur);
 }
 void launch_denoise_wavelet(const CameraDev& c, const SceneDev& s, int cur, u32 frame, u32 stride, float strength, const float4* di_in, float4* di_out, const float4* gi_in, float4* gi_out,
                             const float4* pair_in, float4* pair_out, bool fast, cudaStream_t st) {
-#define ST_WG(F_, P_) k_denoise_wavelet<F_, P_><<<grid_full(c), ST_BLOCK, 0, st>>>(c, s, cur, frame, stride, strength, di_in, di_out, gi_in, gi_out, pair_in, pair_out)
+#define ST_WG(F_, P_) launch_k(k_denoise_wavelet<F_, P_>, grid_full(c), ST_BLOCK, 0, st, c, s, cur, frame, stride, strength, di_in, di_out, gi_in, gi_out, pair_in, pair_out)
     if (pair_in) { if (fast) ST_WG(true, true); else ST_WG(false, true); }
     else { if (fast) ST_WG(true, false); else ST_WG(false, false); }
 #undef ST_WG
@@ -2263,6 +2303,7 @@
 template <bool FAST, int TW, int TH>
 __global__ void __launch_bounds__(TW * TH) k_denoise_variance_tiled(KPARAMS, int cur, const __grid_constant__ CUtensorMap tm_nd, const __grid_constant__ CUtensorMap tm_di,
                                                                     const __grid_constant__ CUtensorMap tm_gi, u32* __restrict__ errors) {
+    ST_PDL_ENTER();
     typedef VarianceTile<TW, TH> T;
     extern __shared__ unsigned char s_raw[];
     __shared__ __align__(8) unsigned long long s_bar;
@@ -2377,7 +2418,7 @@
     int dev = 0; cudaGetDevice(&dev); dev &= 63;
     if (!attr_set[dev]) { if (cudaFuncSetAttribute(kern, cudaFuncAttributeMaxDynamicSharedMemorySize, (int)T::SMEM) != cudaSuccess) { cudaGetLastError(); return false; } attr_set[dev] = true; }
     dim3 grid((c.w + TW - 1) / TW, (c.y1 - c.y0 + TH - 1) / TH);
-    kern<<<grid, TW * TH, T::SMEM, st>>>(c, s, frame, strength, tn, td, tg, di_out, gi_out, pair_out, errors);
+    launch_k(kern, grid, TW * TH, T::SMEM, st, c, s, frame, strength, tn, td, tg, di_out, gi_out, pair_out, errors);
     return true;
 }
 template <bool FAST, int S, int J>
@@ -2417,14 +2458,14 @@
     int dev = 0; cudaGetDevice(&dev); dev &= 63;
     if (!attr_set[dev]) { if (cudaFuncSetAttribute(kern, cudaFuncAttributeMaxDynamicSharedMemorySize, (int)T::SMEM) != cudaSuccess) { cudaGetLastError(); return false; } attr_set[dev] = true; }
     dim3 grid((c.w + 31) / 32, (c.y1 - c.y0 + 7) / 8);
-    kern<<<grid, 256, T::SMEM, st>>>(c, s, cur, tn, td, tg, errors);
+    launch_k(kern, grid, 256, T::SMEM, st, c, s, cur, tn, td, tg, errors);
     return true;
 }
 bool launch_denoise_variance_tiled(const CameraDev& c, const SceneDev& s, int cur, bool fast, u32* errors, cudaStream_t st) {
     if (c.curr.screen.x != (float)c.w || c.curr.screen.y != (float)c.h) return false;
     return fast ? variance_tiled_go<true>(c, s, cur, errors, st) : variance_tiled_go<false>(c, s, cur, errors, st);
 }
-void launch_composition(const CameraDev& c, const SceneDev& s, int cur, u32 mode, const float4* di_diff, const float4* gi_diff, cudaStream_t st) { k_composition<<<grid_full(c), ST_BLOCK, 0, st>>>(c, s, cur, mode, di_diff, gi_diff); }
+void launch_composition(const CameraDev& c, const SceneDev& s, int cur, u32 mode, const float4* di_diff, const float4* gi_diff, cudaStream_t st) { launch_k(k_composition, grid_full(c), ST_BLOCK, 0, st, c, s, cur, mode, di_diff, gi_diff); }
 void launch_taa_resolve(const CameraDev& c, const SceneDev& s, int cur, u32 mode, const float4* di_diff, const float4* gi_diff, const float4* hist_in, float4* hist_out,
                         float4 jit, cudaStream_t st) {
     const dim3 grid((c.w + TAA_TW - 1) / TAA_TW, (c.h + TAA_TH - 1) / TAA_TH);
diff --git a/strolle_b200/csrc/kernels.h b/strolle_b200/csrc/kernels.h
--- a/strolle_b200/csrc/kernels.h
+++ b/strolle_b200/csrc/kernels.h
@@ -1,6 +1,8 @@
 #pragma once
 #include <cuda_runtime.h>
 #include "st_types.h"
+
+extern thread_local bool g_pdl_next;
 
 namespace st {
 typedef uint32_t u32;
diff --git a/strolle_b200/engine.py b/strolle_b200/engine.py
--- a/strolle_b200/engine.py
+++ b/strolle_b200/engine.py
@@ -202,6 +202,7 @@
         "st_plan_frame": [C.POINTER(C.c_int), C.c_int, u32, C.c_int, C.c_char_p, C.c_size_t],
         "st_plan_strip_order": [C.POINTER(C.c_int), C.c_int, C.c_int, C.c_char_p, C.c_size_t],
         "st_strip_bounds": [C.c_int, C.c_int, C.POINTER(C.c_int)],
+        "st_pass_footprint": [C.c_int, C.POINTER(C.c_int), C.POINTER(u32), C.POINTER(u32)],
         "st_render_strips": [P, i32, P, C.c_int, C.c_int, C.c_int], "st_halo_bytes": [P, C.POINTER(C.c_uint64)],
         "st_peer_export": [P, i32, C.c_void_p], "st_peer_import": [P, i32, C.c_void_p, C.c_int, C.c_int],
         "st_peer_errors": [P, i32, C.POINTER(u32)],
@@ -728,6 +729,14 @@
     return [(out[2 * r], out[2 * r + 1]) for r in range(world)]
 
 
+def pass_footprint(pass_id):
+    lib = load_library()
+    chain, reads, writes = C.c_int(), C.c_uint32(), C.c_uint32()
+    if lib.st_pass_footprint(int(pass_id), C.byref(chain), C.byref(reads), C.byref(writes)) != 0:
+        raise StrolleError(lib.st_last_error().decode())
+    return chain.value, reads.value, writes.value
+
+
 def plan_strip_order(schedule, dma=True, still=False):
     lib = load_library()
     arr = (C.c_int * len(schedule))(*schedule)
```

After: 3826 (median of 6 runs). 1.03x the previous value.
